# datamicroscopes/common

Measured on AMD Instinct MI355X. Metric: score_value evals/sec, higher is better.
Workload: dtype f32

## Files before the change

common_amd/csrc/abi.cpp:

```cpp
#include <algorithm>
#include <atomic>
#include <cmath>
#include <memory>
#include <mutex>
#include <new>

#include "launchers.hpp"

namespace msc {

static thread_local std::string g_last_error;

void set_error(const char *fmt, ...) {
  char buf[1024];
  va_list ap;
  va_start(ap, fmt);
  vsnprintf(buf, sizeof buf, fmt, ap);
  va_end(ap);
  g_last_error = buf;
}
int fail(int code, const char *fmt, ...) {
  char buf[1024];
  va_list ap;
  va_start(ap, fmt);
  vsnprintf(buf, sizeof buf, fmt, ap);
  va_end(ap);
  g_last_error = buf;
  return code;
}

size_t primitive_size(int t) {
  static const size_t sz[MSC_TYPE_NELEMS] = {1, 1, 1, 2, 2, 4, 4, 8, 8, 4, 8};
  return (t >= 0 && t < MSC_TYPE_NELEMS) ? sz[t] : 0;
}

static bool family_ok(int f) { return f >= MSC_BB && f <= MSC_DM; }

struct Switches {
  bool tail_forced = false, no_narrow_tail = false, no_bb_fuse = false, sweep_graph = false;
  uint64_t tail_min_rows = 0;
  int loo_lds = -1, sweep_nich1 = 0, alloc_candidates = 12;
  int marginal_tile = -1;

  float alloc_accept_gbps = 6650.f;
};
static Switches read_switches() {
  Switches sw;
  if (const char *e = std::getenv("MSC_TAIL_MIN_ROWS")) sw.tail_forced = true, sw.tail_min_rows = (uint64_t)std::atoll(e);
  sw.no_narrow_tail = std::getenv("MSC_NO_NARROW_TAIL") != nullptr, sw.no_bb_fuse = std::getenv("MSC_NO_BB_FUSE") != nullptr;
  if (const char *e = std::getenv("MSC_LOO_LDS")) sw.loo_lds = std::atoi(e);
  if (const char *e = std::getenv("MSC_SWEEP_NICH1")) sw.sweep_nich1 = std::atoi(e);
  if (const char *e = std::getenv("MSC_MARGINAL_TILE")) sw.marginal_tile = std::atoi(e);
  if (const char *g = std::getenv("MSC_SWEEP_GRAPH")) sw.sweep_graph = g[0] != '0' && g[0] != 0;
  if (const char *e = std::getenv("MSC_ALLOC_CANDIDATES")) sw.alloc_candidates = std::atoi(e);
  if (const char *e = std::getenv("MSC_ALLOC_ACCEPT_GBPS")) sw.alloc_accept_gbps = (float)std::atof(e);
  return sw;
}

template <typename T>
static int alloc_zeroed(DevBuf<T> &buf, size_t count) {
  MSC_HIP(buf.alloc(count, 1));
  MSC_HIP(hipMemset(buf, 0, std::max<size_t>(count, 1) * sizeof(T)));
  return MSC_OK;
}

}

using namespace msc;

extern "C" int msc_abi_version(void) { return MSC_ABI_VERSION; }
extern "C" const char *msc_last_kernel(int which) { return msc::last_kernel(which); }
extern "C" const char *msc_last_error(void) { return g_last_error.c_str(); }
extern "C" const char *msc_build_info(void) {
  return "microscopes_hip abi " "1" " gfx950 (CDNA4) hipcc " __VERSION__;
}

static int device_error_word(int device, volatile uint32_t **host_out) {
  static std::mutex mu;
  static uint32_t *words[64] = {};
  MSC_REQUIRE(device >= 0 && device < 64, "device %d: at most 64 devices", device);
  std::lock_guard<std::mutex> lock(mu);
  if (!words[device]) {
    uint32_t *h = nullptr;
    void *d = nullptr;
    MSC_HIP(hipHostMalloc(reinterpret_cast<void **>(&h), 64, hipHostMallocMapped));
    h[0] = h[1] = 0;
    MSC_HIP(hipHostGetDevicePointer(&d, h, 0));
    uint32_t *w = static_cast<uint32_t *>(d);
    if (bind_error_word_score(w) || bind_error_word_sweep(w) || bind_error_word_state(w) || bind_error_word_seq(w) ||
        bind_error_word_query(w))
      return fail(MSC_EHIP, "binding the device error word failed: %s", hipGetErrorString(hipGetLastError()));
    words[device] = h;
  }
  *host_out = words[device];
  return MSC_OK;
}
static int device_error_check(msc_context *ctx) {
  volatile uint32_t *w = ctx ? ctx->err_host : nullptr;
  if (!w || w[0] == 0) return MSC_OK;
  std::atomic_thread_fence(std::memory_order_acquire);
  const uint32_t code = w[0], detail = w[1];
  w[0] = 0;
  std::string what;
  auto add = [&](const char *t) { if (!what.empty()) what += "; "; what += t; };
  if (code & 1u) add("a wave-subset barrier of a tile kernel timed out (detail: workgroup): rows of that launch are wrong");
  if (code & 2u) add("msc_entity_op: leave from a group the row is not in / an empty group, or join of an assigned row (detail: group)");
  if (code & 4u) add("msc_relation_slice_scores: a block offset beyond the score row (detail: cell)");
  if (code & 8u) add("msc_sweep_sequential: an order entry >= nrows (visit skipped; detail: entry), or a leave from an empty group or counter (detail: group)");
  if (code & 16u) add("msc_zmatrix_add: a label outside [0, nlabels) (that sample was skipped; detail: row of z)");
  if (code & ~31u) add("unknown device-side error");
  return fail(MSC_EDEVICE, "reported by an earlier kernel on device %d: %s [detail of the first: %u]; rebuild the affected state's tables",
              ctx->device, what.c_str(), detail);
}

extern "C" int msc_context_create(int device, void *stream, msc_context **out) {
  MSC_REQUIRE(out != nullptr, "msc_context_create: out is null");
  *out = nullptr;
  int ndev = 0;
  hipError_t e = hipGetDeviceCount(&ndev);
  if (e != hipSuccess || ndev <= 0)
    return fail(MSC_ENODEVICE, "no HIP device visible (%s); this library has no CPU path",
                e == hipSuccess ? "device count is 0" : hipGetErrorString(e));
  MSC_REQUIRE(device >= 0 && device < ndev, "device %d out of range (have %d)", device, ndev);
  hipDeviceProp_t prop;
  MSC_HIP(hipGetDeviceProperties(&prop, device));
  if (std::strncmp(prop.gcnArchName, "gfx950", 6) != 0)
    return fail(MSC_ENODEVICE, "device %d is %s; kernels are built for gfx950 only", device,
                prop.gcnArchName);
  MSC_HIP(hipSetDevice(device));
  std::unique_ptr<msc_context> ctx(new (std::nothrow) msc_context());
  if (!ctx) return fail(MSC_ENOMEM, "out of host memory");
  ctx->device = device;
  ctx->stream = static_cast<hipStream_t>(stream);
  ctx->num_cus = prop.multiProcessorCount > 0 ? prop.multiProcessorCount : 256;
  MSC_HIP(ctx->mailbox_host.alloc(192 * 1024));
  MSC_HIP(hipHostGetDevicePointer(&ctx->mailbox_dev, ctx->mailbox_host, 0));
  if (ctx->sync_word_host.alloc(16) == hipSuccess) {
    *ctx->sync_word_host = 0;
    if (hipHostGetDevicePointer(&ctx->sync_word_dev, ctx->sync_word_host, 0) != hipSuccess) ctx->sync_word_ok = false;
  } else {
    (void)hipGetLastError();
  }
  MSC_TRY(device_error_word(device, &ctx->err_host));
  *out = ctx.release();
  return MSC_OK;
}

static void vmm_free(msc_context::VmmAlloc &a);

extern "C" int msc_context_destroy(msc_context *ctx) {
  if (!ctx) return MSC_OK;
  (void)hipSetDevice(ctx->device);
  for (auto &a : ctx->vmm) vmm_free(a);
  ctx->vmm.clear();
  if (ctx->record_stream) (void)hipStreamDestroy(ctx->record_stream);
  delete ctx;
  return MSC_OK;
}

extern "C" int msc_context_set_stream(msc_context *ctx, void *stream) {
  MSC_REQUIRE(ctx, "null context");
  ctx->stream = static_cast<hipStream_t>(stream);
  return MSC_OK;
}

extern "C" int msc_context_synchronize(msc_context *ctx) {
  MSC_REQUIRE(ctx, "null context");
  if (ctx->sync_word_host && ctx->sync_word_ok) {
    const uint32_t seq = ++ctx->sync_seq;
    if (hipStreamWriteValue32(ctx->stream, ctx->sync_word_dev, seq, 0) == hipSuccess) {
      volatile uint32_t *w = ctx->sync_word_host;
      for (int spin = 0; spin < 400000; spin++)
        if (*w == seq) {
          std::atomic_thread_fence(std::memory_order_acquire);
          return device_error_check(ctx);
        }
    } else {
      (void)hipGetLastError();
      ctx->sync_word_ok = false;
    }
  }
  MSC_HIP(hipStreamSynchronize(ctx->stream));
  return device_error_check(ctx);
}

static bool vmm_alloc(int device, size_t nbytes, msc_context::VmmAlloc *out) {
  const size_t chunk = 32u << 20;
  hipMemAllocationProp prop = {};
  prop.type = hipMemAllocationTypePinned;
  prop.location.type = hipMemLocationTypeDevice;
  prop.location.id = device;
  size_t gran = 0;
  if (hipMemGetAllocationGranularity(&gran, &prop, hipMemAllocationGranularityMinimum) != hipSuccess || gran == 0 || chunk % gran != 0) {
    (void)hipGetLastError();
    return false;
  }
  msc_context::VmmAlloc a;
  const size_t n = (std::max<size_t>(nbytes, 1) + chunk - 1) / chunk;
  a.size = n * chunk;
  a.va = nullptr;
  if (hipMemAddressReserve(&a.va, a.size, 2u << 20, nullptr, 0) != hipSuccess) {
    (void)hipGetLastError();
    return false;
  }
  bool ok = true;
  size_t mapped = 0;
// ... 737 lines not shown
    d.loo_tab = nullptr;
    tf.push_back(d);
    extra_f.push_back(0u);
  }
  for (uint32_t i = 0; i < n; i++)
    if (!taken[i]) {
      tf.push_back(t[i]);
      extra_f.push_back(extra[i]);
    }
  {
    std::vector<FeatDesc> &ta = st->desc_acc_host;
    ta.clear();
    std::vector<bool> covered(n, false);
    for (size_t q = 0; q < quads.size(); q++) {
      const Fused &fq = quads[q];
      if ((size_t)st->K * 8u * fq.m * 4u > 64u * 1024u) continue;
      const std::vector<uint32_t> &mem = members[fq.radix - 2];
      FeatDesc d = tf[q];
      for (uint32_t j = 0; j < 4; j++) d.fuse_acc[j] = nullptr;
      for (uint32_t j = 0; j < fq.m; j++) {
        const uint32_t src = t_src[mem[fq.first + j]];
        d.fuse_acc[j] = st->desc_host[src].acc_i64;
        covered[src] = true;
      }
      ta.push_back(d);
    }
    for (uint32_t i = 0; i < n; i++)
      if (!covered[i]) ta.push_back(st->desc_host[i]);
  }
  const std::vector<Fused> &fused = quads;
  st->fuse_any = !fused.empty();
  st->fuse_nfeat = (uint32_t)tf.size();
  st->fuse_split = split - (n - st->fuse_nfeat);
  for (uint32_t i = st->fuse_split; i < st->fuse_nfeat; i++) {
    tf[i].blk_first -= n - st->fuse_nfeat;
    tf[i].blk_end -= n - st->fuse_nfeat;
  }
  if (st->fuse_any) facts = plan_layout(tf, st->fuse_split, extra_f, sw);
  for (FeatDesc &d : tf) d.rn_pack = nullptr, d.rn_pos = nullptr, d.rn_x = nullptr, d.rn_n2 = d.rn_n2p = 0;
  for (FeatDesc &d : t) d.rn_pack = nullptr, d.rn_pos = nullptr, d.rn_x = nullptr, d.rn_n2 = d.rn_n2p = 0;
  if (stages_nich(facts.path) && bview == nullptr) facts.path = MSC_PATH_TILE;
  if (stages_nich(facts.path)) {
    const uint32_t s0 = st->fuse_split, n2 = st->fuse_nfeat - s0, n2p = (n2 + 3u) & ~3u;
    std::vector<NichPos> pos(n2p);
    std::vector<const void *> xcols(n2);
    for (uint32_t i = 0; i < n2p; i++) {
      NichPos &q = pos[i];
      q.xlim = INFINITY, q.blk_ok = 0u;
      if (i < n2) {
        const FeatDesc &d = tf[s0 + i];
        q.blk = (d.blk_first - s0) | (d.blk_end - d.blk_first) << 16, q.seg_end = d.grp_end - s0;
        xcols[i] = d.col;
      } else q.blk = i | 1u << 16, q.seg_end = n2p;
    }
    const float *xm = nullptr;
    if (nich_x_matrix(bview, xcols, &xm)) {
      MSC_HIP(hipMemcpyAsync(st->rn_pos, pos.data(), sizeof(NichPos) * n2p, hipMemcpyHostToDevice, st->ctx->stream));
      MSC_HIP(hipStreamSynchronize(st->ctx->stream));
      FeatDesc &h = tf[s0];
      h.rn_pack = st->rn_pack, h.rn_pos = st->rn_pos, h.rn_x = xm, h.rn_n2 = n2, h.rn_n2p = n2p;
    } else facts.path = MSC_PATH_TILE;
  }
  for (FeatDesc &d : tf) d.lk_idx = nullptr, d.lk_l4 = d.lk_goff = 0;
  for (FeatDesc &d : t) d.lk_idx = nullptr, d.lk_l4 = d.lk_goff = 0;
  if (bview == nullptr && facts.path == MSC_PATH_LOOKUPS) facts.path = MSC_PATH_TILE;
  if (facts.path == MSC_PATH_TILE_ROLES || facts.path == MSC_PATH_LOOKUPS) {
    const uint32_t *im = nullptr;
    uint32_t l4 = 0;
    if (look_idx_matrix(bview, tf, st->fuse_split, &im, &l4)) tf[0].lk_idx = im, tf[0].lk_l4 = l4;
    else facts.path = MSC_PATH_TILE;
  }
  st->tile_path = facts.path;
  {
    double lookups = 0, rows = 0, nich = (double)(st->fuse_nfeat - st->fuse_split);
    for (uint32_t i = 0; i < st->fuse_split; i++) {
      if (tf[i].family == MSC_NICH) nich += 1;
      else if (tf[i].family == MSC_DM) lookups += 2.0 * (tf[i].dim + 1), rows += tf[i].grp_rows;
      else lookups += 1, rows += tf[i].grp_rows;
    }
    PlanCost pc;
    const double first = 6.0 + 0.45 * lookups + 0.012 * rows;
    pc.tile_round_us = facts.path == MSC_PATH_NICH_PACK ? 6.0 + 1.3 * nich + 3.0 * lookups : facts.path == MSC_PATH_TILE_ROLES ? first + 0.75 * nich
                       : facts.path == MSC_PATH_LOOKUPS ? 0.75 * first : first + 1.5 * nich;
    pc.sweep_round_us = pc.tile_round_us + 2.5;
    pc.tail_fixed_us = 2.0;
    pc.tail_group_us = 0.5 + 0.03 * lookups + 0.057 * nich;
    st->plan_cost = pc;
  }
  st->tile_narrow_tail_ok = facts.tail_ok;
  st->tail_masked_nich = facts.tail_masked_nich;
  st->tail_dm = facts.tail_dm;
  st->tail_max_rows = facts.tail_max_rows;
  st->tail_pack_rows = facts.tail_pack_rows;
  return MSC_OK;
}

static int upload_desc(msc_state *st) {
  MSC_TRY(plan_groups(st));
  MSC_HIP(hipMemcpyAsync(st->desc_dev, st->desc_host.data(), sizeof(FeatDesc) * st->nfeat,
                         hipMemcpyHostToDevice, st->ctx->stream));
  MSC_HIP(hipMemcpyAsync(st->desc_tile_dev, st->desc_tile_host.data(), sizeof(FeatDesc) * st->nfeat,
                         hipMemcpyHostToDevice, st->ctx->stream));
  MSC_HIP(hipMemcpyAsync(st->desc_fuse_dev, st->desc_fuse_host.data(), sizeof(FeatDesc) * st->fuse_nfeat,
                         hipMemcpyHostToDevice, st->ctx->stream));
  MSC_HIP(hipMemcpyAsync(st->desc_acc_dev, st->desc_acc_host.data(), sizeof(FeatDesc) * st->desc_acc_host.size(),
                         hipMemcpyHostToDevice, st->ctx->stream));
  MSC_HIP(hipStreamSynchronize(st->ctx->stream));
  return MSC_OK;
}

extern "C" int msc_state_create(msc_context *ctx, const msc_feature_spec *features,
                                uint32_t nfeatures, uint32_t ngroups, msc_state **out) {
  MSC_REQUIRE(ctx && features && out, "null argument");
  MSC_REQUIRE(nfeatures > 0 && nfeatures <= 65535, "a state needs 1..65535 features (got %u)", nfeatures);
  MSC_REQUIRE(ngroups > 0 && ngroups <= (1u << 20), "ngroups %u out of range", ngroups);
  *out = nullptr;
  MSC_HIP(hipSetDevice(ctx->device));
  std::unique_ptr<msc_state> st(new (std::nothrow) msc_state());
  if (!st) return fail(MSC_ENOMEM, "out of host memory");
  st->ctx = ctx;
  st->nfeat = nfeatures;
  st->K = ngroups;
  st->kpad = round_up(ngroups, kGroupTile);
  const size_t kpad = st->kpad;
  st->feats.resize(nfeatures);
  st->desc_host.resize(nfeatures);
  size_t n_i64 = kpad, n_f64 = 0;
  for (uint32_t f = 0; f < nfeatures; f++) {
    msc_feature_host &h = st->feats[f];
    h.family = features[f].family;
    h.dim = features[f].dim;
    MSC_REQUIRE(family_ok(h.family), "feature %u: unknown family %d", f, h.family);
    if (h.family == MSC_DD && (h.dim == 0 || h.dim > kMaxDDDim))
      return fail(MSC_EUNSUPPORTED, "feature %u: dd dim %u outside 1..%u (DirichletDiscrete<128>)", f,
                  h.dim, kMaxDDDim);
    if (h.family == MSC_DM && (h.dim == 0 || h.dim > kMaxDDDim))
      return fail(MSC_EUNSUPPORTED, "feature %u: dm categories %u outside 1..%u", f, h.dim, kMaxDDDim);
    if (h.family == MSC_NIW && (h.dim == 0 || h.dim > kMaxNiwDim))
      return fail(MSC_EUNSUPPORTED, "feature %u: niw dim %u outside 1..%u", f, h.dim, kMaxNiwDim);
    h.i64_off = n_i64;
    h.i64_len = acc_i64_rows(h.family, h.dim) * kpad;
    n_i64 += h.i64_len;
    h.f64_off = n_f64;
    h.f64_len = h.family == MSC_NIW ? (size_t)ngroups * (h.dim + (size_t)h.dim * h.dim)
                                    : acc_f64_rows(h.family) * kpad;
    n_f64 += h.f64_len;
  }
  st->n_i64 = n_i64;
  st->n_f64 = n_f64;
  st->nich1 = nfeatures == 1 && st->feats[0].family == MSC_NICH;
  for (const msc_feature_host &h : st->feats) st->has_dm |= h.family == MSC_DM, st->n_niw += h.family == MSC_NIW;
  MSC_TRY(alloc_zeroed(st->red_i64, n_i64));
  MSC_TRY(alloc_zeroed(st->red_f64, n_f64));
  MSC_TRY(alloc_zeroed(st->cnt_u32, kpad));
  MSC_TRY(alloc_zeroed(st->logpc, crp_floats(st->kpad)));
  MSC_TRY(alloc_zeroed(st->desc_dev, nfeatures));
  MSC_TRY(alloc_zeroed(st->desc_tile_dev, nfeatures));
  MSC_TRY(alloc_zeroed(st->desc_fuse_dev, nfeatures));
  MSC_TRY(alloc_zeroed(st->nich_info, nfeatures));
  MSC_TRY(alloc_zeroed(st->rn_pos, (size_t)((nfeatures + 3u) & ~3u)));
  {
    size_t nnich = 0;
    for (uint32_t f = 0; f < nfeatures; f++) nnich += features[f].family == MSC_NICH;
    MSC_TRY(alloc_zeroed(st->rn_pack, (1 + kNichPackRows * nnich) * (size_t)kpad));
  }
  MSC_TRY(alloc_zeroed(st->desc_acc_dev, nfeatures));
  MSC_TRY(alloc_zeroed(st->rng_dev, 2));
  MSC_TRY(alloc_zeroed(st->colmax_dev, 1));
  for (uint32_t f = 0; f < nfeatures; f++) {
    msc_feature_host &h = st->feats[f];
    default_hp(h.family, h.dim, h.hp);
    MSC_TRY(alloc_zeroed(h.hp_dev, h.hp.size()));
    MSC_TRY(alloc_zeroed(h.tab, (size_t)(tab_rows(h.family, h.dim) + 4) * kpad));
    MSC_TRY(alloc_zeroed(h.raw_u32, (size_t)raw_u32_rows(h.family, h.dim) * kpad));
    const size_t nf32 = h.family == MSC_NIW ? (size_t)ngroups * (h.dim + (size_t)h.dim * h.dim)
                                            : (size_t)raw_f32_rows(h.family) * kpad;
    MSC_TRY(alloc_zeroed(h.raw_f32, nf32));
    if (loo_rows(h.family)) MSC_TRY(alloc_zeroed(h.loo64, (size_t)loo_rows(h.family) * kpad));
    if (loo_tab_rows(h.family, h.dim)) MSC_TRY(alloc_zeroed(h.loo_tab, (size_t)loo_tab_rows(h.family, h.dim) * kpad));
    if (h.family == MSC_DM) {
      MSC_TRY(alloc_zeroed(h.dm_meta_dev, 2 * ((size_t)h.dim + 1)));
      h.dm_meta.assign(2 * ((size_t)h.dim + 1), 0u);
    }
    if (h.family == MSC_NIW) {
      if (h.dim <= (uint32_t)kNiwPad) {
        MSC_TRY(alloc_zeroed(h.niw_w, (size_t)ngroups * kNiwPad * kNiwPad));
        MSC_TRY(alloc_zeroed(h.niw_b, (size_t)ngroups * 2 * kNiwPad));
      }
      MSC_TRY(alloc_zeroed(h.niw_w64, (size_t)ngroups * niw_w_stream(h.dim)));
      MSC_TRY(alloc_zeroed(h.niw_mu64, (size_t)ngroups * niw_b_stream(h.dim)));
      MSC_TRY(alloc_zeroed(h.niw_c64, (size_t)ngroups * 8));
    }
    if (!h.hp.empty()) {
      hipError_t e = hipMemcpy(h.hp_dev, h.hp.data(), h.hp.size() * sizeof(float), hipMemcpyHostToDevice);
      if (e != hipSuccess) return fail(MSC_EHIP, "hp upload failed: %s", hipGetErrorString(e));
    }
    h.raw_valid = true;
    h.additive_valid = true;
    h.derived_valid = false;
    FeatDesc &d = st->desc_host[f];
    std::memset(&d, 0, sizeof d);
    d.family = h.family;
    d.dim = h.dim;
    d.col_type = value_type_of(h.family);
    d.hp = h.hp_dev;
    d.tab = h.tab;
    d.raw_u32 = h.raw_u32;
    d.raw_f32 = h.raw_f32;
    d.acc_i64 = st->red_i64 + h.i64_off;
    d.acc_f64 = st->red_f64 + h.f64_off;
    d.niw_w = h.niw_w;
    d.niw_b = h.niw_b;
    d.niw_w64 = h.niw_w64;
    d.niw_mu64 = h.niw_mu64;
    d.niw_c64 = h.niw_c64;
    d.vcap = 32;
    d.dm_meta = nullptr;
    d.loo64 = h.loo64;
    d.loo_tab = h.loo_tab;
    d.aux = 0.0;
    for (float a : h.hp) d.aux += h.family == MSC_DD || h.family == MSC_DM ? (double)a : 0.0;
  }
  st->cnt_additive_valid = true;
  MSC_TRY(upload_desc(st.get()));
  hipError_t e = hipStreamSynchronize(ctx->stream);
  if (e != hipSuccess) return fail(MSC_EHIP, "state init failed: %s", hipGetErrorString(e));
  *out = st.release();
  return MSC_OK;
}

extern "C" int msc_state_destroy(msc_state *st) {
  if (!st) return MSC_OK;
  (void)hipSetDevice(st->ctx->device);
  (void)hipStreamSynchronize(st->ctx->stream);
  if (st->step_graph.exec) (void)hipGraphExecDestroy(st->step_graph.exec);
  if (st->pred_upload) (void)hipEventDestroy(st->pred_upload);
  delete st;
  return MSC_OK;
}

extern "C" int msc_state_shape(const msc_state *st, uint32_t *nfeatures, uint32_t *ngroups) {
  MSC_REQUIRE(st, "null state");
  if (nfeatures) *nfeatures = st->nfeat;
  if (ngroups) *ngroups = st->K;
  return MSC_OK;
}

extern "C" int msc_state_set_hp(msc_state *st, uint32_t feature, const float *host_hp, size_t nfloats) {
  MSC_REQUIRE(st && host_hp, "null argument");
  MSC_REQUIRE(feature < st->nfeat, "feature %u out of range", feature);
  msc_feature_host &h = st->feats[feature];
  MSC_REQUIRE(nfloats == h.hp.size(), "feature %u: hp block has %zu floats, expected %zu", feature,
              nfloats, h.hp.size());
  std::copy(host_hp, host_hp + nfloats, h.hp.begin());
  if (nfloats) {
    MSC_HIP(hipMemcpyAsync(h.hp_dev, h.hp.data(), nfloats * sizeof(float), hipMemcpyHostToDevice, st->ctx->stream));
    MSC_HIP(hipStreamSynchronize(st->ctx->stream));
  }
  h.derived_valid = false;
  if (h.family == MSC_DD || h.family == MSC_DM) {
    double asum = 0;
    for (float a : h.hp) asum += (double)a;
    st->desc_host[feature].aux = asum;
    MSC_TRY(upload_desc(st));
  }
  return MSC_OK;
}

extern "C" int msc_state_get_hp(const msc_state *st, uint32_t feature, float *host_hp, size_t nfloats) {
  MSC_REQUIRE(st && host_hp, "null argument");
  MSC_REQUIRE(feature < st->nfeat, "feature %u out of range", feature);
  const msc_feature_host &h = st->feats[feature];
  MSC_REQUIRE(nfloats == h.hp.size(), "feature %u: hp block has %zu floats, expected %zu", feature,
              nfloats, h.hp.size());
  std::copy(h.hp.begin(), h.hp.end(), host_hp);
  return MSC_OK;
}

static int launch_commit_all(msc_state *st) {
  if (launch_commit(st->ctx->stream, st->desc_dev, (int)st->nfeat, st->kpad, st->red_i64, st->cnt_u32))
    return fail(MSC_EHIP, "k_commit launch failed");
  for (uint32_t f = 0; f < st->nfeat; f++)
    if (st->feats[f].family == MSC_NIW &&
        launch_niw_commit(st->ctx->stream, st->desc_dev, f, st->feats[f].dim, st->K, st->kpad, 1))
      return fail(MSC_EHIP, "k_niw_commit launch failed");
  return MSC_OK;
}

static int ensure_raw(msc_state *st) {
  bool any = false;
  for (auto &h : st->feats) any |= !h.raw_valid;
  if (!any) return MSC_OK;
  MSC_TRY(launch_commit_all(st));
  for (auto &h : st->feats) { h.raw_valid = true; h.derived_valid = false; }
  st->crp_valid = false;
  return MSC_OK;
}

static void record_layout(int family, uint32_t dim, uint32_t &nu32, uint32_t &nf32) {
  nu32 = raw_u32_rows(family, dim);
  nf32 = raw_f32_rows(family);
}

extern "C" int msc_state_set_ss(msc_state *st, uint32_t feature, uint32_t first_group,
                                uint32_t ngroups, const void *host_records, size_t nbytes) {
  MSC_REQUIRE(st && host_records, "null argument");
// ... 486 lines not shown
  r.lanes = narrow_lanes(st, sw, &r.table_rows);
  r.path = st->nich1 ? MSC_PATH_NICH1 : st->has_dm ? MSC_PATH_TILE_DM : st->tile_path;
  if (r.lanes) return r;
  if (r.path == MSC_PATH_NICH1) {
    r.shape.nich1 = nich1_shape_for(st->ctx, out, nrows, st->K);
    return r;
  }
  const int cus = st->ctx->num_cus;
  const uint32_t ktiles = st->kpad / kGroupTile, last_groups = st->K - (ktiles - 1) * kGroupTile;
  const uint64_t round = (uint64_t)cus / ktiles;
  const bool small4 = r.path != MSC_PATH_TILE_DM && (nrows + 63) / 64 <= round, small2 = small4 && (nrows + 31) / 32 <= round;
  r.shape.wave_rows = small2 ? 2 : small4 ? 4 : 8;
  r.shape.pair = !small4 && pair_path(r.path, st->K);
  if (ktiles > 1 && r.path == MSC_PATH_TILE_ROLES && !small4 && last_groups > 64 && last_groups <= 128) r.shape.last = LastTile::pair;
  if (r.shape.last == LastTile::pair || !narrow_tail_fits(st)) return r;
  const PlanCost &pc = st->plan_cost;
  const uint64_t c128 = (nrows + 127) / 128;
  const double tile_us = (r.shape.pair ? kPairTileShare : 1.0) *
                         (tile_rounds_us(c128 * ktiles, cus, false, pc) - (ktiles > 1 ? tile_rounds_us(c128 * (ktiles - 1), cus, false, pc) : 0.0));
  const bool many_rows = sw.tail_forced ? nrows >= sw.tail_min_rows
                                        : nrows >= kTailMinRows && tail_rows_us(last_groups, true, nrows, cus, pc) < tile_us;
  if (many_rows) r.shape.last = LastTile::rows;
  return r;
}

static int run_score(msc_state *st, uint64_t row0, uint64_t nrows, const int32_t *z_dev, bool crp,
                     bool niw_f32, float *out_dev, uint64_t ld_out) {
  hipStream_t s = st->ctx->stream;
  const float *prior = crp ? st->logpc : nullptr;
  if (z_dev) MSC_TRY(run_loo_own(st, row0, nrows, z_dev, crp));
  const ScoreRoute r = route_score(st, nrows, out_dev);
  if (r.lanes) {
    return launch_narrow(s, st->ctx->num_cus, r.lanes, r.table_rows, false, st->desc_dev, (int)st->nfeat, st->K, st->kpad, row0, nrows,
                         z_dev, st->own, prior, out_dev, ld_out, 0, nullptr, nullptr, ZeroSpans());
  }
  bool written = false;
  if (st->n_niw < st->nfeat || crp) {
    const bool nich1 = r.path == MSC_PATH_NICH1;
    TailPlan tail;
    if (!nich1) {
      MSC_TRY(tail_plan(st, tail));
      MSC_TRY(refresh_fused_tables(st));
    }
    MSC_TRY(launch_score(s, st->ctx->num_cus, r.path, tail, r.shape, nich1 ? st->desc_dev : st->desc_fuse_dev, (int)st->fuse_nfeat,
                         (int)st->fuse_split, st->K, st->kpad, row0, nrows, z_dev, st->own, prior, out_dev, ld_out));
    written = true;
    for (uint32_t f = 0; f < st->nfeat; f++)
      if (gp_beyond_table(st, f) &&
          launch_gp_large_fix(s, st->ctx->num_cus, st->desc_dev, (int)f, st->K, st->kpad, row0, nrows, z_dev, out_dev, ld_out))
        return fail(MSC_EHIP, "k_gp_large_fix launch failed");
  }
  for (uint32_t f = 0; f < st->nfeat; f++) {
    if (st->feats[f].family != MSC_NIW) continue;
    if (z_dev) MSC_HIP(grow_retained(st->retired, st->niw_qown, nrows));
    if (launch_niw_score(s, st->ctx->num_cus, st->desc_dev, f, st->feats[f].dim, st->K, st->kpad, row0, nrows, z_dev, written,
                         niw_f32, st->niw_qown, out_dev, ld_out))
      return fail(MSC_EHIP, "k_score_niw launch failed: %s", hipGetErrorString(hipGetLastError()));
    written = true;
  }
  return MSC_OK;
}

extern "C" int msc_score_value(msc_state *st, const msc_dataview *view, const uint32_t *cols,
                               uint64_t row0, uint64_t nrows, const int32_t *z_dev, uint32_t flags,
                               float *out_dev, uint64_t ld_out) {
  MSC_REQUIRE(st && (out_dev || nrows == 0), "null argument");
  MSC_REQUIRE(ld_out >= st->K, "ld_out %llu < ngroups %u", (unsigned long long)ld_out, st->K);
  MSC_REQUIRE((flags & ~(MSC_SCORE_CRP_PRIOR | MSC_SCORE_NIW_F32)) == 0, "unknown flags 0x%x", flags);
  MSC_HIP(hipSetDevice(st->ctx->device));
  MSC_TRY(device_error_check(st->ctx));
  MSC_TRY(bind_view(st, view, cols, row0, nrows));
  if (nrows == 0) return MSC_OK;
  MSC_TRY(ensure_derived(st));
  const bool crp = (flags & MSC_SCORE_CRP_PRIOR) != 0;
  if (crp) MSC_TRY(ensure_crp(st));
  return run_score(st, row0, nrows, z_dev, crp, (flags & MSC_SCORE_NIW_F32) != 0, out_dev, ld_out);
}

extern "C" int msc_score_tune(msc_state *st, const msc_dataview *view, const uint32_t *cols, uint64_t row0,
                              uint64_t nrows, float *out_dev, uint64_t ld_out, int *shape_out, float *ms_out) {
  MSC_REQUIRE(st && view && out_dev, "null argument");
  MSC_REQUIRE(ld_out >= st->K, "ld_out %llu < ngroups %u", (unsigned long long)ld_out, st->K);
  if (shape_out) *shape_out = -1;
  if (ms_out) *ms_out = 0.f;
  MSC_HIP(hipSetDevice(st->ctx->device));
  MSC_TRY(bind_view(st, view, cols, row0, nrows));
  const ScoreRoute r = route_score(st, nrows, out_dev);
  if (r.lanes || r.path != MSC_PATH_NICH1 || nrows == 0) return MSC_OK;
  MSC_TRY(ensure_derived(st));
  hipStream_t s = st->ctx->stream;
  hipStreamCaptureStatus cap = hipStreamCaptureStatusNone;
  if (hipStreamIsCapturing(s, &cap) == hipSuccess && cap != hipStreamCaptureStatusNone)
    return fail(MSC_EINVAL, "msc_score_tune waits for the device: not on a capturing stream");
  auto launch = [&](int code) {
    return launch_score(s, st->ctx->num_cus, MSC_PATH_NICH1, TailPlan(), ScoreShape{8, false, LastTile::tiles, code}, st->desc_dev, 1, (int)st->tile_split, st->K, st->kpad, row0,
                        nrows, nullptr, nullptr, nullptr, out_dev, ld_out);
  };
  hipEvent_t e0, e1;
  MSC_HIP(hipEventCreate(&e0));
  MSC_HIP(hipEventCreate(&e1));
  float best = 0.f;
  int shape = -1, rc = MSC_OK;
  for (int cand = 0; cand < kNich1NumShapes && rc == MSC_OK; cand++) {
    if ((rc = launch(cand)) != MSC_OK) break;
    hipError_t e = hipEventRecord(e0, s);
    for (int r = 0; r < 6 && e == hipSuccess; r++) (void)launch(cand);
    if (e == hipSuccess) e = hipEventRecord(e1, s);
    if (e == hipSuccess) e = hipEventSynchronize(e1);
    float ms = 0.f;
    if (e == hipSuccess) e = hipEventElapsedTime(&ms, e0, e1);
    if (e != hipSuccess) { rc = fail(MSC_EHIP, "timing failed: %s", hipGetErrorString(e)); break; }
    if (shape < 0 || ms < best) {
      best = ms;
      shape = cand;
    }
  }
  int plain_stores = 0;
  if (rc == MSC_OK && shape >= 0) {
    float ms_kind[2] = {0.f, 0.f};
    for (int kind = 0; kind < 2 && rc == MSC_OK; kind++) {
      const int code = shape | (kind ? 0x100 : 0);
      if ((rc = launch(code)) != MSC_OK) break;
      hipError_t e = hipEventRecord(e0, s);
      for (int r = 0; r < 6 && e == hipSuccess; r++) (void)launch(code);
      if (e == hipSuccess) e = hipEventRecord(e1, s);
      if (e == hipSuccess) e = hipEventSynchronize(e1);
      if (e == hipSuccess) e = hipEventElapsedTime(&ms_kind[kind], e0, e1);
      if (e != hipSuccess) rc = fail(MSC_EHIP, "timing failed: %s", hipGetErrorString(e));
    }
    plain_stores = ms_kind[1] < ms_kind[0] ? 1 : 0;
    best = ms_kind[plain_stores];
  }
  (void)hipEventDestroy(e0);
  (void)hipEventDestroy(e1);
  MSC_TRY(rc);
  auto &memo = st->ctx->nich1_shapes;
  for (size_t i = 0; i < memo.size();)
    if (memo[i].out == out_dev && memo[i].nrows == nrows && memo[i].K == st->K) memo.erase(memo.begin() + i);
    else i++;
  memo.insert(memo.begin(), msc_context::ShapeEntry{out_dev, nrows, st->K, shape, plain_stores});
  if (memo.size() > 16) memo.pop_back();
  if (shape_out) *shape_out = shape;
  if (ms_out) *ms_out = best / 6.f;
  return MSC_OK;
}

static int commit(msc_state *st) {
  MSC_TRY(launch_commit_all(st));
  for (auto &h : st->feats) { h.raw_valid = true; h.derived_valid = false; }
  st->crp_valid = false;
  return MSC_OK;
}

enum : uint32_t { kAccZeroed = 0x100, kAccThenPrepare = 0x200 };

static int commit_and_prepare(msc_state *st, bool bump_rng = true) {
  hipStream_t s = st->ctx->stream;
  if (launch_commit_prepare(s, st->desc_dev, (int)st->nfeat, st->K, st->kpad, st->red_i64, st->cnt_u32, st->alpha,
                            st->logpc, bump_rng ? st->rng_dev : nullptr, prepare_value_slices(st)))
    return fail(MSC_EHIP, "k_commit_prepare launch failed");
  for (uint32_t f = 0; f < st->nfeat; f++) {
    const msc_feature_host &h = st->feats[f];
    if (h.family == MSC_NIW && (launch_niw_commit(s, st->desc_dev, f, h.dim, st->K, st->kpad, 1) ||
                                launch_niw_prepare(s, st->desc_dev, f, h.dim, st->K, st->kpad)))
      return fail(MSC_EHIP, "niw commit / prepare launch failed");
    if (h.family == MSC_DM && st->desc_host[f].dm_meta != nullptr &&
        launch_dm_prepare(s, st->desc_dev, (int)f, h.dim, st->kpad, dm_value_slices(h)))
      return fail(MSC_EHIP, "k_dm_prepare launch failed");
  }
  for (auto &h : st->feats) { h.raw_valid = true; h.derived_valid = true; }
  st->crp_valid = true;
  return MSC_OK;
}

static int accumulate_impl(msc_state *st, const msc_dataview *view, const uint32_t *cols, uint64_t row0,
                           uint64_t nrows, const int32_t *z_dev, uint32_t flags) {
  MSC_TRY(bind_view(st, view, cols, row0, nrows));
  hipStream_t s = st->ctx->stream;
  if (flags & MSC_ACC_RESET) {
    if (!(flags & kAccZeroed) && launch_zero64(s, st->red_i64, st->n_i64, st->red_f64, st->n_f64))
      return fail(MSC_EHIP, "k_zero64 launch failed");
  } else {
    MSC_TRY(ensure_raw(st));
    for (uint32_t f = 0; f < st->nfeat; f++)
      if (!st->feats[f].additive_valid) {
        const int rc = st->feats[f].family == MSC_NIW
                           ? launch_niw_commit(s, st->desc_dev, f, st->feats[f].dim, st->K, st->kpad, 0)
                           : launch_lift(s, st->desc_dev + f, 1, st->kpad, st->red_i64, st->cnt_u32, 0);
        if (rc) return fail(MSC_EHIP, "k_lift launch failed");
      }
    if (!st->cnt_additive_valid)
      if (launch_lift(s, st->desc_dev, 0, st->kpad, st->red_i64, st->cnt_u32, 1))
        return fail(MSC_EHIP, "k_lift launch failed");
  }
  for (auto &h : st->feats) h.additive_valid = true;
  st->cnt_additive_valid = true;
  if (nrows > 0) {
    const int rc = launch_accumulate(s, st->ctx->num_cus, st->desc_acc_dev, st->desc_acc_host.data(), (int)st->desc_acc_host.size(),
                                     st->K, st->kpad, row0, nrows, z_dev,
                                     (flags & MSC_ACC_SUBTRACT) ? -1 : 1, st->red_i64);
    if (rc == -2) return fail(MSC_EUNSUPPORTED, "accumulate tables for %u groups exceed LDS", st->K);
    if (rc) return fail(MSC_EHIP, "k_accumulate launch failed: %s", hipGetErrorString(hipGetLastError()));
    for (uint32_t f = 0; f < st->nfeat; f++) {
      if (st->feats[f].family != MSC_NIW) continue;
      MSC_REQUIRE(nrows < (1ull << 32), "niw accumulate takes at most 2^32 - 1 rows per call");
      MSC_HIP(grow_retained(st->retired, st->niw_scratch, 2 * (size_t)st->K + 1 + (size_t)nrows));
      if (launch_niw_accumulate(s, st->ctx->num_cus, st->desc_dev, f, st->K, row0, nrows, z_dev,
                                (flags & MSC_ACC_SUBTRACT) ? -1 : 1, st->niw_scratch, st->feats[f].dim))
        return fail(MSC_EHIP, "niw accumulate launch failed");
    }
  }
  for (auto &h : st->feats) h.raw_valid = false;
  if (flags & kAccThenPrepare) return commit_and_prepare(st);
  if (!(flags & MSC_ACC_NO_COMMIT)) MSC_TRY(commit(st));
  return MSC_OK;
}

extern "C" int msc_accumulate(msc_state *st, const msc_dataview *view, const uint32_t *cols,
                              uint64_t row0, uint64_t nrows, const int32_t *z_dev, uint32_t flags) {
  MSC_REQUIRE(st && (z_dev || nrows == 0), "null argument");
  MSC_REQUIRE((flags & ~(MSC_ACC_RESET | MSC_ACC_SUBTRACT | MSC_ACC_NO_COMMIT)) == 0, "unknown flags 0x%x", flags);
  MSC_HIP(hipSetDevice(st->ctx->device));
  MSC_TRY(device_error_check(st->ctx));
  return accumulate_impl(st, view, cols, row0, nrows, z_dev, flags);
}

extern "C" int msc_entity_op(msc_state *st, const msc_dataview *view, const uint32_t *cols, uint64_t row, uint32_t group,
                             int sign, int32_t *z_dev) {
  MSC_REQUIRE(st && view, "null argument");
  MSC_REQUIRE(sign != 0, "sign must be +1 (join) or -1 (leave)");
  MSC_REQUIRE(group < st->K, "group %u outside [0,%u)", group, st->K);
  MSC_REQUIRE(!st->rng_bump_pending, "msc_entity_op between msc_sweep_step_begin and msc_state_commit_reduce: the additive "
                                     "tables hold uncommitted sums");
  MSC_TRY(device_error_check(st->ctx));
  MSC_HIP(hipSetDevice(st->ctx->device));
  MSC_TRY(bind_view(st, view, cols, row, 1));
  hipStream_t s = st->ctx->stream;
  bool scalar_only = true;
  for (const auto &h : st->feats) scalar_only &= h.family != MSC_NIW && h.family != MSC_DM;
  if (!scalar_only) {
    if (!st->one_z) MSC_TRY(alloc_zeroed(st->one_z, 1));
    if (launch_set_i32(s, st->one_z, (int32_t)group)) return fail(MSC_EHIP, "k_set_i32 launch failed");
    MSC_TRY(accumulate_impl(st, view, cols, row, 1, st->one_z, sign < 0 ? (uint32_t)MSC_ACC_SUBTRACT : 0u));
    if (z_dev && launch_set_i32(s, z_dev + row, sign > 0 ? (int32_t)group : -1)) return fail(MSC_EHIP, "k_set_i32 launch failed");
    return MSC_OK;
  }
  MSC_TRY(ensure_raw(st));
  for (uint32_t f = 0; f < st->nfeat; f++)
    if (!st->feats[f].additive_valid && launch_lift(s, st->desc_dev + f, 1, st->kpad, st->red_i64, st->cnt_u32, 0))
      return fail(MSC_EHIP, "k_lift launch failed");
  if (!st->cnt_additive_valid && launch_lift(s, st->desc_dev, 0, st->kpad, st->red_i64, st->cnt_u32, 1))
    return fail(MSC_EHIP, "k_lift launch failed");
  for (auto &h : st->feats) h.additive_valid = true;
  st->cnt_additive_valid = true;
  MSC_TRY(ensure_derived(st));
  MSC_TRY(ensure_crp(st));
  if (launch_entity_op(s, st->desc_dev, (int)st->nfeat, st->K, st->kpad, row, group, sign > 0 ? 1 : -1, st->red_i64, st->cnt_u32,
                       st->alpha, st->logpc, z_dev ? z_dev + row : nullptr))
    return fail(MSC_EHIP, "k_entity_op launch failed");
  return MSC_OK;
}

extern "C" int msc_score_data(msc_state *st, float *out_dev) {
  MSC_REQUIRE(st && out_dev, "null argument");
  MSC_HIP(hipSetDevice(st->ctx->device));
  MSC_TRY(ensure_raw(st));
  if (launch_score_data(st->ctx->stream, st->desc_dev, (int)st->nfeat, st->K, st->kpad, out_dev))
    return fail(MSC_EHIP, "k_score_data launch failed");
  if (st->n_niw) {
    MSC_TRY(ensure_derived(st));
    for (uint32_t f = 0; f < st->nfeat; f++)
      if (st->feats[f].family == MSC_NIW &&
          launch_niw_score_data(st->ctx->stream, st->desc_dev, f, st->K, st->kpad, out_dev))
        return fail(MSC_EHIP, "k_niw_score_data launch failed");
  }
  return MSC_OK;
}

static bool sweep_is_niw1(const msc_state *st) {
  return st->nfeat == 1 && st->feats[0].family == MSC_NIW && (int)st->K <= sweep_niw1_max_groups(st->feats[0].dim);
}

static bool sweep_pair_mode(const msc_state *st) {
  return view_rows(st) >= kTailMinRows && pair_path(st->tile_path, st->K);
}
static bool sweep_rows_pays(const msc_state *st, const Switches &sw, uint32_t groups) {
  const uint64_t rows = view_rows(st);
  if (sw.tail_forced) return rows >= sw.tail_min_rows;
  if (rows < kTailMinRows) return false;
  const int cus = st->ctx->num_cus;
  const uint64_t c128 = (rows + 127) / 128;
  const bool tail = groups < st->K;
  const double sample_us = [&](uint64_t floats_per_row) { return 30.0 + (double)rows * floats_per_row * 4.0 / 2.0e6; }(tail ? st->K : 128);
  double rows_us = tail_rows_us(groups, false, rows, cus, st->plan_cost), tile_us;
  if (tail) {
    rows_us *= 1.15;
    tile_us = tile_rounds_us(c128, cus, false, st->plan_cost) + sample_us;
  } else {
    if (groups > 64) rows_us += sample_us;
    PlanCost pc = st->plan_cost;
    pc.sweep_round_us = pc.tile_round_us * (sweep_pair_mode(st) ? kPairTileShare : 1.0) + 2.5;
    tile_us = tile_rounds_us(c128, cus, true, pc);
  }
  return rows_us < tile_us;
}

static bool sweep_plain(const msc_state *st) {
  for (uint32_t f = 0; f < st->nfeat; f++) if (gp_beyond_table(st, f)) return false;
  return st->n_niw == 0;
}

static bool sweep_is_fused(const msc_state *st) {
  if (sweep_is_niw1(st)) return true;
  if (!sweep_plain(st)) return false;
  return st->nich1 ? st->K <= sweep_nich1_rows_max_groups() : st->K <= 256;
}

enum class SweepKind { niw1, nich1, nich1_rows, narrow, rows, rows_sampler, mixed, roles_tail, generic };
struct SweepRoute {
  SweepKind kind = SweepKind::generic;
  int lanes = 0; uint32_t table_rows = 0;
  bool transposed = false;
  ScoreShape shape;
  uint64_t tail_ld = 0;
  bool tail_pair = false;
};
static SweepRoute route_sweep(const msc_state *st, uint64_t nrows) {
  const Switches sw = read_switches();
  const uint64_t cus = (uint64_t)st->ctx->num_cus;
  SweepRoute r;
  if (sweep_is_niw1(st)) {
    r.kind = SweepKind::niw1;
  } else if (sweep_is_fused(st)) {
    if (st->nich1) {
      r.kind = st->K > 1024 ? SweepKind::nich1_rows : SweepKind::nich1;
      r.transposed = sw.sweep_nich1 == 2 || (sw.sweep_nich1 != 1 && view_rows(st) >= cus * 64);
    } else if ((r.lanes = narrow_lanes(st, sw, &r.table_rows)) != 0) {
      r.kind = SweepKind::narrow;
    } else if (narrow_tail_fits(st) && st->K <= kTailMaxGroups && sweep_rows_pays(st, sw, st->K)) {
      r.kind = st->K <= 64 ? SweepKind::rows : SweepKind::rows_sampler;
    } else {
      r.kind = SweepKind::mixed;
      r.shape.pair = sweep_pair_mode(st);
      const bool small = (nrows + 63) / 64 <= cus, view_small = (view_rows(st) + 63) / 64 <= cus;
      const int R = small ? ((nrows + 31) / 32 > cus ? 4 : 2) : view_small ? 4 : 8;
      if (!st->has_dm && (view_small || st->tile_path == MSC_PATH_TILE)) r.shape.wave_rows = R;
    }
  } else if (!st->nich1 && !st->has_dm && st->tile_path != MSC_PATH_TILE && st->tile_narrow_tail_ok && st->K > 256 &&
             st->K <= (uint32_t)kGroupTile + kTailMaxGroups && sweep_rows_pays(st, sw, st->K - kGroupTile) && sweep_plain(st)) {
    r.tail_ld = st->K <= (uint32_t)kGroupTile + 64 ? 64 : 128;
    r.tail_pair = st->tile_path == MSC_PATH_TILE_ROLES && r.tail_ld == 128;
    if (r.tail_pair || narrow_tail_fits(st)) r.kind = SweepKind::roles_tail;
  }
  return r;
}

static int sweep_assign_impl(msc_state *st, const msc_dataview *view, const uint32_t *cols, uint64_t row0,
                             uint64_t nrows, uint64_t row_id0, int32_t *z_dev, uint64_t seed, uint64_t sweep,
                             bool *zeroed = nullptr) {
  MSC_TRY(bind_view(st, view, cols, row0, nrows));
  if (nrows == 0) return MSC_OK;
  if (!st->rng_valid || st->rng_seed != seed || st->rng_sweep != sweep) {
    if (launch_rng_set(st->ctx->stream, st->rng_dev, seed, sweep)) return fail(MSC_EHIP, "k_rng_set launch failed");
    st->rng_valid = true;
    st->rng_seed = seed;
    st->rng_sweep = sweep;
  }
  MSC_TRY(ensure_derived(st));
  MSC_TRY(ensure_crp(st));
  hipStream_t s = st->ctx->stream;
  const int cus = st->ctx->num_cus;
  ZeroSpans zero;
  if (zeroed) {
    zero.a = reinterpret_cast<unsigned long long *>(st->red_i64.get()); zero.na = st->n_i64;
    zero.b = reinterpret_cast<unsigned long long *>(st->red_f64.get()); zero.nb = st->n_f64;
  }
  const SweepRoute r = route_sweep(st, nrows);
  bool zeroes = true;
  switch (r.kind) {
    case SweepKind::niw1:
      MSC_TRY(launch_sweep_niw1(s, cus, st->feats[0].dim, st->desc_dev, st->K, st->kpad, row0, nrows, row_id0, z_dev, st->logpc, st->rng_dev, zero));
      break;
    case SweepKind::nich1_rows:
      MSC_HIP(grow_retained(st->retired, st->rows_table, sweep_nich1_rows_table_floats(st->kpad)));
      MSC_TRY(launch_sweep_nich1_rows(s, cus, st->desc_dev, st->K, st->kpad, row0, nrows, row_id0, z_dev, st->logpc, st->rng_dev, zero, st->rows_table));
      break;
    case SweepKind::nich1:
      MSC_TRY(launch_sweep_nich1(s, cus, r.transposed, st->desc_dev, st->K, st->kpad, row0, nrows, row_id0, z_dev, st->own, st->logpc, st->rng_dev, zero));
      break;
    case SweepKind::narrow:
      MSC_TRY(run_loo_own(st, row0, nrows, z_dev, true));
      MSC_TRY(launch_narrow(s, cus, r.lanes, r.table_rows, true, st->desc_dev, (int)st->nfeat, st->K, st->kpad, row0, nrows, z_dev,
                            st->own, st->logpc, nullptr, 0, row_id0, z_dev, st->rng_dev, zero));
      break;
    case SweepKind::mixed:
      MSC_TRY(run_loo_own(st, row0, nrows, z_dev, true));
      MSC_TRY(refresh_fused_tables(st));
      MSC_TRY(launch_sweep_mixed(s, cus, st->has_dm, st->tile_path, r.shape, st->desc_fuse_dev, (int)st->fuse_nfeat, (int)st->fuse_split, st->K, st->kpad, row0, nrows, row_id0, z_dev, st->own, st->logpc, st->rng_dev, zero));
      break;
    case SweepKind::rows:
    case SweepKind::rows_sampler: {
      MSC_TRY(run_loo_own(st, row0, nrows, z_dev, true));
      MSC_TRY(refresh_fused_tables(st));
      TailPlan tail;
      MSC_TRY(tail_plan(st, tail, false));
      if (r.kind == SweepKind::rows) {
        MSC_TRY(launch_sweep_rows(s, cus, tail, st->desc_fuse_dev, (int)st->fuse_nfeat, (int)st->fuse_split, st->K, st->kpad, row0, nrows, row_id0,
                                  z_dev, st->own, st->logpc, st->rng_dev, zero));
        break;
      }
      MSC_HIP(grow_retained(st->retired, st->tail_scores, ((size_t)nrows + 16) * 128));
      MSC_TRY(launch_score_tail(s, cus, tail, st->desc_fuse_dev, (int)st->fuse_nfeat, (int)st->fuse_split, st->K, st->kpad, 0, row0, nrows,
                                z_dev, st->own, st->logpc, st->tail_scores, 128));
      if (launch_sample_rows(s, cus, st->tail_scores, 128, st->K, nrows, row_id0, z_dev, st->rng_dev)) return fail(MSC_EHIP, "k_sample_rows launch failed");
      zeroes = false;
      break;
    }
    case SweepKind::roles_tail: {
      MSC_TRY(refresh_fused_tables(st));
      MSC_TRY(run_loo_own(st, row0, nrows, z_dev, true));
      MSC_HIP(grow_retained(st->retired, st->tail_scores, ((size_t)nrows + 16) * r.tail_ld));
      TailPlan tail;
      MSC_TRY(tail_plan(st, tail, false));
      MSC_TRY(r.tail_pair ? launch_score_pair_tail(s, cus, st->desc_fuse_dev, (int)st->fuse_nfeat, (int)st->fuse_split, st->K, st->kpad, row0, nrows,
                                                   z_dev, st->own, st->logpc, st->tail_scores, r.tail_ld)
                          : launch_score_tail(s, cus, tail, st->desc_fuse_dev, (int)st->fuse_nfeat, (int)st->fuse_split, st->K, st->kpad,
                                              kGroupTile, row0, nrows, z_dev, st->own, st->logpc, st->tail_scores - kGroupTile, r.tail_ld));
      MSC_TRY(launch_sweep_roles_tail(s, cus, st->tile_path, st->desc_fuse_dev, (int)st->fuse_nfeat, (int)st->fuse_split, st->K, st->kpad, row0, nrows,
                                      row_id0, z_dev, st->own, st->logpc, st->rng_dev, zero, st->tail_scores));
      break;
    }
    case SweepKind::generic: {
      const uint64_t ld = std::min<uint64_t>(st->kpad, ((uint64_t)st->K + 63) & ~63ull);
      const uint64_t chunk = std::max<uint64_t>(1, std::min<uint64_t>((4096ull << 20) / (ld * sizeof(float)), nrows));
      MSC_HIP(grow_retained(st->retired, st->scratch, chunk * ld));
      for (uint64_t at = 0; at < nrows; at += chunk) {
        const uint64_t n = std::min<uint64_t>(chunk, nrows - at);
        MSC_TRY(run_score(st, row0 + at, n, z_dev + at, true, false, st->scratch, ld));
        if (launch_sample_rows(s, cus, st->scratch, ld, st->K, n, row_id0 + at, z_dev + at, st->rng_dev))
          return fail(MSC_EHIP, "k_sample_rows launch failed");
      }
      zeroes = false;
      break;
    }
  }
  if (zeroed) {
    *zeroed = zeroes;
    return MSC_OK;
  }
  if (launch_rng_bump(s, st->rng_dev)) return fail(MSC_EHIP, "k_rng_bump launch failed");
  st->rng_sweep = sweep + 1;
  return MSC_OK;
}

extern "C" int msc_sweep_assign(msc_state *st, const msc_dataview *view, const uint32_t *cols,
                                uint64_t row0, uint64_t nrows, uint64_t row_id0, int32_t *z_dev,
                                uint64_t seed, uint64_t sweep) {
  MSC_REQUIRE(st && (z_dev || nrows == 0), "null argument");
  MSC_HIP(hipSetDevice(st->ctx->device));
  MSC_TRY(device_error_check(st->ctx));
  return sweep_assign_impl(st, view, cols, row0, nrows, row_id0, z_dev, seed, sweep);
}

static int accumulate_impl(msc_state *st, const msc_dataview *view, const uint32_t *cols, uint64_t row0,
                           uint64_t nrows, const int32_t *z_dev, uint32_t flags);

typedef std::vector<uint8_t> StepFlags;
static StepFlags save_flags(const msc_state *st) {
  StepFlags f;
  for (auto &h : st->feats) f.push_back((uint8_t)(h.raw_valid | (h.additive_valid << 1) | (h.derived_valid << 2)));
  f.push_back((uint8_t)(st->cnt_additive_valid | (st->crp_valid << 1) | (st->rng_valid << 2)));
  return f;
}
static void restore_flags(msc_state *st, const StepFlags &f) {
  for (size_t i = 0; i < st->feats.size(); i++) {
    st->feats[i].raw_valid = f[i] & 1;
    st->feats[i].additive_valid = (f[i] >> 1) & 1;
    st->feats[i].derived_valid = (f[i] >> 2) & 1;
  }
  st->cnt_additive_valid = f.back() & 1;
  st->crp_valid = (f.back() >> 1) & 1;
  st->rng_valid = (f.back() >> 2) & 1;
}

extern "C" int msc_sweep_step(msc_state *st, const msc_dataview *view, const uint32_t *cols, uint64_t row0,
                              uint64_t nrows, uint64_t row_id0, int32_t *z_dev, uint64_t seed, uint64_t sweep) {
  MSC_REQUIRE(st && view && (z_dev || nrows == 0), "null argument");
  MSC_HIP(hipSetDevice(st->ctx->device));
  MSC_TRY(device_error_check(st->ctx));
  hipStream_t s = st->ctx->stream;
  auto eager = [&]() -> int {
    st->step_graph.n_eager++;
    bool zeroed = false;
    MSC_TRY(sweep_assign_impl(st, view, cols, row0, nrows, row_id0, z_dev, seed, sweep, &zeroed));
    st->rng_valid = false;
    MSC_TRY(accumulate_impl(st, view, cols, row0, nrows, z_dev,
                            MSC_ACC_RESET | kAccThenPrepare | (zeroed ? (uint32_t)kAccZeroed : 0u)));
    st->rng_valid = true;
    st->rng_sweep = sweep + 1;
    return MSC_OK;
  };
  MSC_TRY(bind_view(st, view, cols, row0, nrows));
  msc_state::StepGraph &g = st->step_graph;
  const bool no_graph = !read_switches().sweep_graph;
  if (nrows == 0) return accumulate_impl(st, view, cols, row0, 0, z_dev, MSC_ACC_RESET);
  if (no_graph || g.disabled) return eager();
  std::vector<uint32_t> colv(st->nfeat);
  for (uint32_t f = 0; f < st->nfeat; f++) colv[f] = cols ? cols[f] : f;
  const bool same_key = g.view == view && g.view_serial == view->serial && g.row0 == row0 && g.nrows == nrows &&
                        g.row_id0 == row_id0 && g.z == z_dev && g.alpha == st->alpha && g.cols == colv;
  if (!same_key) {
    if (g.exec) { (void)hipGraphExecDestroy(g.exec); g.exec = nullptr; }
    g.view = view; g.view_serial = view->serial; g.row0 = row0; g.nrows = nrows; g.row_id0 = row_id0; g.z = z_dev;
    g.alpha = st->alpha; g.cols = colv;
    g.seen = 0;
  }
  const bool next_sweep = st->rng_valid && st->rng_seed == seed && st->rng_sweep == sweep;
  const StepFlags entry = save_flags(st);
  if (g.exec) {
    if (!next_sweep || entry != g.flags) return eager();
    MSC_HIP(hipGraphLaunch(g.exec, s));
    g.n_replayed++;
    st->rng_sweep = sweep + 1;
    return MSC_OK;
  }
  if (g.seen < 2 || !next_sweep || !sweep_is_fused(st)) {
    g.seen++;
    return eager();
  }
  msc_context *ctx = st->ctx;
  if (!ctx->record_stream && hipStreamCreateWithFlags(&ctx->record_stream, hipStreamNonBlocking) != hipSuccess)
    ctx->record_stream = nullptr;
  if (!ctx->record_stream || hipStreamBeginCapture(ctx->record_stream, hipStreamCaptureModeThreadLocal) != hipSuccess) {
    (void)hipGetLastError();
    g.disabled = true;
    return eager();
  }
  const uint64_t sweep_before = st->rng_sweep;
  ctx->stream = ctx->record_stream;
  const int rc = eager();
  ctx->stream = s;
  g.n_eager--;
  hipGraph_t graph = nullptr;
  const hipError_t ec = hipStreamEndCapture(ctx->record_stream, &graph);
  bool ok = rc == MSC_OK && ec == hipSuccess && graph != nullptr && save_flags(st) == entry;
  if (ok && hipGraphInstantiate(&g.exec, graph, nullptr, nullptr, 0) != hipSuccess) {
    g.exec = nullptr;
    ok = false;
  }
  if (graph) (void)hipGraphDestroy(graph);
  if (!ok) {
    (void)hipGetLastError();
    if (g.exec) { (void)hipGraphExecDestroy(g.exec); g.exec = nullptr; }
    g.disabled = true;
    restore_flags(st, entry);
    st->rng_sweep = sweep_before;
    return eager();
  }
  g.flags = entry;
  MSC_HIP(hipGraphLaunch(g.exec, s));
  g.n_replayed++;
  return MSC_OK;
}

extern "C" int msc_sweep_step_begin(msc_state *st, const msc_dataview *view, const uint32_t *cols, uint64_t row0,
                                    uint64_t nrows, uint64_t row_id0, int32_t *z_dev, uint64_t seed, uint64_t sweep) {
  MSC_REQUIRE(st && view && (z_dev || nrows == 0), "null argument");
  MSC_HIP(hipSetDevice(st->ctx->device));
  MSC_TRY(device_error_check(st->ctx));
  if (nrows == 0) return accumulate_impl(st, view, cols, row0, 0, z_dev, MSC_ACC_RESET | MSC_ACC_NO_COMMIT);
  bool zeroed = false;
  MSC_TRY(sweep_assign_impl(st, view, cols, row0, nrows, row_id0, z_dev, seed, sweep, &zeroed));
  st->rng_valid = false;
  st->rng_bump_pending = true;
  st->rng_next_sweep = sweep + 1;
  return accumulate_impl(st, view, cols, row0, nrows, z_dev,
                         MSC_ACC_RESET | MSC_ACC_NO_COMMIT | (zeroed ? (uint32_t)kAccZeroed : 0u));
}

extern "C" int msc_sweep_step_stats(const msc_state *st, uint64_t *eager_steps, uint64_t *graph_steps) {
  MSC_REQUIRE(st, "null argument");
  if (eager_steps) *eager_steps = st->step_graph.n_eager;
  if (graph_steps) *graph_steps = st->step_graph.n_replayed;
  return MSC_OK;
}

constexpr double kSeqLaunchUs = 20000.0;
constexpr uint64_t kSeqMaxVisitsPerLaunch = 10000;

static double seq_visit_us(const msc_state *st) {
  double rows = 0.0;
  for (uint32_t f = 0; f < st->nfeat; f++) {
    switch (st->feats[f].family) {
      case MSC_BB: rows += 4; break;
      case MSC_GP:
      case MSC_BNB: rows += 2.0 * st->desc_host[f].vcap + 4; break;
      case MSC_DD: rows += 2.0 * st->feats[f].dim + 2; break;
      case MSC_NICH: rows += 14; break;
      default: break;
    }
  }
  return 16.0 + 0.02 * 2.0 * rows + 0.007 * (double)st->K * (double)st->nfeat;
}

struct SeqRoute { int rc = MSC_OK; const char *why = ""; };
static SeqRoute route_sequential(const msc_state *st) {
  SeqRoute r;
  for (const auto &h : st->feats) {
    if (h.family == MSC_NIW || h.family == MSC_DM || h.family == MSC_BBNC) {
      r.rc = MSC_EUNSUPPORTED;
      r.why = "the sequential sweep takes bb, gp, bnb, dd, nich and noop features (the state holds niw, dm or bbnc)";
      return r;
    }
  }
  if (st->nfeat > (uint32_t)kSeqMaxFeat) {
    r.rc = MSC_EUNSUPPORTED;
    r.why = "the sequential sweep takes at most 256 features";
  } else if (st->K > kSeqMaxGroups) {
    r.rc = MSC_EUNSUPPORTED;
    r.why = "the sequential sweep takes at most 8192 groups";
  }
  return r;
}

extern "C" int msc_sweep_sequential(msc_state *st, const msc_dataview *view, const uint32_t *cols, uint64_t row0,
                                    uint64_t nrows, uint64_t row_id0, int32_t *z_dev, const uint32_t *order_dev,
                                    uint32_t nsweeps, uint64_t seed, uint64_t sweep, int32_t *trace_dev) {
  MSC_REQUIRE(st && view && (z_dev || nrows == 0), "null argument");
  MSC_REQUIRE(nrows < (1ull << 32), "the sequential sweep takes at most 2^32 - 1 rows per call");
  MSC_REQUIRE(!st->rng_bump_pending, "msc_sweep_sequential between msc_sweep_step_begin and msc_state_commit_reduce: the "
                                     "additive tables hold uncommitted sums");
  MSC_HIP(hipSetDevice(st->ctx->device));
  MSC_TRY(device_error_check(st->ctx));
  const SeqRoute route = route_sequential(st);
  if (route.rc != MSC_OK) return fail(route.rc, "%s", route.why);
  MSC_TRY(bind_view(st, view, cols, row0, nrows));
  if (nrows == 0 || nsweeps == 0) return MSC_OK;
  hipStream_t s = st->ctx->stream;
  MSC_TRY(ensure_raw(st));
  for (uint32_t f = 0; f < st->nfeat; f++)
    if (!st->feats[f].additive_valid && launch_lift(s, st->desc_dev + f, 1, st->kpad, st->red_i64, st->cnt_u32, 0))
      return fail(MSC_EHIP, "k_lift launch failed");
  if (!st->cnt_additive_valid && launch_lift(s, st->desc_dev, 0, st->kpad, st->red_i64, st->cnt_u32, 1))
    return fail(MSC_EHIP, "k_lift launch failed");
  for (auto &h : st->feats) h.additive_valid = true;
  st->cnt_additive_valid = true;
  MSC_TRY(ensure_derived(st));
  MSC_TRY(ensure_crp(st));
  const uint64_t visits = (uint64_t)nsweeps * nrows;
  const uint64_t per_launch = (uint64_t)std::max(1.0, std::min((double)kSeqMaxVisitsPerLaunch, kSeqLaunchUs / seq_visit_us(st)));
  for (uint64_t v0 = 0; v0 < visits; v0 += per_launch) {
    const uint64_t v1 = std::min(visits, v0 + per_launch);
    const int rc = launch_sweep_seq(s, st->desc_dev, (int)st->nfeat, st->K, st->kpad, row0, nrows, row_id0, z_dev, order_dev,
                                    v0, v1, seed, sweep, st->red_i64, st->cnt_u32, st->alpha, st->logpc, trace_dev);
    if (rc == -2) return fail(MSC_EUNSUPPORTED, "k_sweep_seq does not take this shape");
    if (rc) return fail(MSC_EHIP, "k_sweep_seq launch failed: %s", hipGetErrorString(hipGetLastError()));
  }
  for (auto &h : st->feats) { h.raw_valid = true; h.additive_valid = true; h.derived_valid = true; }
  st->cnt_additive_valid = true;
  st->crp_valid = true;
  return MSC_OK;
}

extern "C" int msc_state_reduce_buffers(msc_state *st, void **dev_i64, size_t *n_i64, void **dev_f64,
                                        size_t *n_f64) {
  MSC_REQUIRE(st, "null state");
  if (dev_i64) *dev_i64 = st->red_i64;
  if (n_i64) *n_i64 = st->n_i64;
  if (dev_f64) *dev_f64 = st->red_f64;
  if (n_f64) *n_f64 = st->n_f64;
  return MSC_OK;
}

extern "C" int msc_state_reduce_pack(msc_state *st, void **pack_dev, size_t *n_f64) {
  MSC_REQUIRE(st && pack_dev, "null argument");
  MSC_HIP(hipSetDevice(st->ctx->device));
  if (!st->red_pack) MSC_TRY(alloc_zeroed(st->red_pack, st->n_i64 + st->n_f64));
  if (launch_pack64(st->ctx->stream, false, st->red_i64, st->n_i64, st->red_f64, st->n_f64, st->red_pack))
    return fail(MSC_EHIP, "k_pack64 launch failed");
  *pack_dev = st->red_pack;
  if (n_f64) *n_f64 = st->n_i64 + st->n_f64;
  return MSC_OK;
}
extern "C" int msc_state_reduce_unpack(msc_state *st) {
  MSC_REQUIRE(st, "null state");
  MSC_REQUIRE(st->red_pack, "msc_state_reduce_unpack before msc_state_reduce_pack");
  MSC_HIP(hipSetDevice(st->ctx->device));
  if (launch_pack64(st->ctx->stream, true, st->red_i64, st->n_i64, st->red_f64, st->n_f64, st->red_pack))
    return fail(MSC_EHIP, "k_unpack64 launch failed");
  return MSC_OK;
}

extern "C" int msc_state_set_sweep_rows(msc_state *st, uint64_t global_rows) {
  MSC_REQUIRE(st, "null state");
  if (st->sweep_rows_hint != global_rows && st->step_graph.exec) {
    (void)hipGraphExecDestroy(st->step_graph.exec);
    st->step_graph.exec = nullptr;
    st->step_graph.seen = 0;
  }
  st->sweep_rows_hint = global_rows;
  return MSC_OK;
}

extern "C" int msc_state_col_bounds(msc_state *st, const msc_dataview *view, const uint32_t *cols, uint32_t *out, size_t n) {
  MSC_REQUIRE(st && view, "null argument");
  const size_t want = col_bounds_size(st);
  MSC_REQUIRE(n == want, "the state's features take %zu column bounds (got %zu)", want, n);
  MSC_REQUIRE(out || n == 0, "null argument");
  MSC_HIP(hipSetDevice(st->ctx->device));
  MSC_TRY(device_error_check(st->ctx));
  MSC_TRY(bind_view(st, view, cols, 0, 0));
  size_t k = 0;
  for (uint32_t f = 0; f < st->nfeat; f++) {
    const uint32_t c = st->bound_cols[f];
    if (is_count_family(st->feats[f].family)) out[k++] = (uint32_t)std::max(view->col_max[c], 0ll);
    else if (st->feats[f].family == MSC_DM)
      for (uint32_t i = 0; i <= st->feats[f].dim; i++) out[k++] = view->dm_max[c][i];
  }
  return MSC_OK;
}

extern "C" int msc_state_set_col_bounds(msc_state *st, const uint32_t *bounds, size_t n) {
  MSC_REQUIRE(st, "null state");
  const size_t want = col_bounds_size(st);
  MSC_REQUIRE(n == 0 || n == want, "the state's features take %zu column bounds (got %zu)", want, n);
  MSC_REQUIRE(bounds || n == 0, "null bounds");
  std::vector<std::vector<uint32_t>> nb;
  if (n != 0) {
    nb.resize(st->nfeat);
    for (uint32_t f = 0, k = 0; f < st->nfeat; f++) {
// ... 788 lines not shown
```

common_amd/csrc/kernels_sweep.hip:

```cpp
#include "family_math.hpp"
#include "launchers.hpp"
#include "score_block.hpp"

namespace msc {

template <int CTRL, int ROW_MASK>
MSC_DEV float dpp_f32(float identity, float v) {
  return __int_as_float(__builtin_amdgcn_update_dpp(__float_as_int(identity), __float_as_int(v), CTRL, ROW_MASK, 0xf, false));
}
#define MSC_DPP_REDUCE(op, v)                                                     \
  asm volatile("s_nop 1\n\t" op " %0, %0, %0 row_shr:1 row_mask:0xf bank_mask:0xf\n\t"      \
               "s_nop 1\n\t" op " %0, %0, %0 row_shr:2 row_mask:0xf bank_mask:0xf\n\t"      \
               "s_nop 1\n\t" op " %0, %0, %0 row_shr:4 row_mask:0xf bank_mask:0xf\n\t"      \
               "s_nop 1\n\t" op " %0, %0, %0 row_shr:8 row_mask:0xf bank_mask:0xf\n\t"      \
               "s_nop 1\n\t" op " %0, %0, %0 row_bcast:15 row_mask:0xa bank_mask:0xf\n\t"   \
               "s_nop 1\n\t" op " %0, %0, %0 row_bcast:31 row_mask:0xc bank_mask:0xf\n\t"   \
               "s_nop 1"                                                          \
               : "+v"(v))
MSC_DEV float wave_max(float v) {
  MSC_DPP_REDUCE("v_max_f32_dpp", v);
  return lane_bcast(v, 63);
}
MSC_DEV float wave_incl_scan(float v, int) {
  MSC_DPP_REDUCE("v_add_f32_dpp", v);
  return v;
}

template <int G, bool LOG2 = false, bool BOUND = false, bool SHIFTED = false>
MSC_DEV int sample_from_scores(const float (&s)[G], float u01, int lane, uint32_t K, float bound = 0.f) {
  float p[G], sum = 0.f, incl = 0.f, total = 0.f;
  bool done = false;
  if (BOUND) {
    sum = 0.f;
#pragma unroll
    for (int j = 0; j < G; j++) {
      p[j] = __builtin_amdgcn_exp2f(SHIFTED ? s[j] : LOG2 ? s[j] - bound : (s[j] - bound) * 1.44269504088896340736f);
      sum += p[j];
    }
    incl = wave_incl_scan(sum, lane);
    total = lane_bcast(incl, 63);
    done = total > 0x1p-60f && total < 0x1p100f;
  }
  if (!done) {
    float m = s[0];
#pragma unroll
    for (int j = 1; j < G; j++) m = fmaxf(m, s[j]);
    m = wave_max(m);
    sum = 0.f;
#pragma unroll
    for (int j = 0; j < G; j++) {
      p[j] = __builtin_amdgcn_exp2f(LOG2 ? s[j] - m : (s[j] - m) * 1.44269504088896340736f);
      sum += p[j];
    }
    incl = wave_incl_scan(sum, lane);
    total = lane_bcast(incl, 63);
  }
  const float dart = u01 * total;
  float c = incl - sum;
  int nmiss = 0;
  if constexpr (G <= 4) {
#pragma unroll
    for (int j = 0; j < G; j++) {
      c += p[j];
      nmiss += c < dart ? 1 : 0;
    }
  } else {
    float q[G / 4];
#pragma unroll
    for (int b = 0; b < G / 4; b++) q[b] = ((p[4 * b] + p[4 * b + 1]) + p[4 * b + 2]) + p[4 * b + 3];
    int blk = 0;
#pragma unroll
    for (int b = 0; b < G / 4; b++) {
      const float cq = c + q[b];
      const bool miss = (blk == b) && cq < dart;
      c = miss ? cq : c;
      blk += miss ? 1 : 0;
    }
    nmiss = 4 * blk;
    if (blk < G / 4) {
      float e0 = p[0], e1 = p[1], e2 = p[2];
#pragma unroll
      for (int b = 1; b < G / 4; b++) {
        e0 = blk == b ? p[4 * b] : e0;
        e1 = blk == b ? p[4 * b + 1] : e1;
        e2 = blk == b ? p[4 * b + 2] : e2;
      }
      c += e0;
      const bool m0 = c < dart;
      c += e1;
      const bool m1 = m0 && c < dart;
      c += e2;
      const bool m2 = m1 && c < dart;
      nmiss += (m0 ? 1 : 0) + (m1 ? 1 : 0) + (m2 ? 1 : 0);
    }
  }
  const unsigned long long hit = __builtin_amdgcn_ballot_w64(nmiss < G);
  if (hit == 0ull) return (int)K - 1;
  const int l = (int)__builtin_ctzll(hit);
  const int k = G * l + lane_bcast(nmiss, l);
  return k < (int)K ? k : (int)K - 1;
}

template <int TAILP>
MSC_DEV int sample_tile_and_tail(const float (&sm)[4], const float (&st)[4], float u01, int lane, uint32_t K) {
  float m = fmaxf(fmaxf(fmaxf(sm[0], sm[1]), fmaxf(sm[2], sm[3])), fmaxf(fmaxf(st[0], st[1]), fmaxf(st[2], st[3])));
  m = wave_max(m);
  float pm[4], pt[4], summ = 0.f, sumt = 0.f;
#pragma unroll
  for (int j = 0; j < 4; j++) {
    pm[j] = __builtin_amdgcn_exp2f((sm[j] - m) * 1.44269504088896340736f);
    pt[j] = __builtin_amdgcn_exp2f((st[j] - m) * 1.44269504088896340736f);
    summ += pm[j];
    sumt += pt[j];
  }
  const float inclm = wave_incl_scan(summ, lane), totm = lane_bcast(inclm, 63);
  const float inclt = wave_incl_scan(sumt, lane), tott = lane_bcast(inclt, 63);
  const float dart = u01 * (totm + tott);
  float c = inclm - summ;
  int nmiss = 0;
#pragma unroll
  for (int j = 0; j < 4; j++) {
    c += pm[j];
    nmiss += c < dart ? 1 : 0;
  }
  unsigned long long hit = __builtin_amdgcn_ballot_w64(nmiss < 4);
  if (hit != 0ull) {
    const int l = (int)__builtin_ctzll(hit);
    return 4 * l + lane_bcast(nmiss, l);
  }
  c = totm + (inclt - sumt);
  nmiss = 0;
#pragma unroll
  for (int j = 0; j < 4; j++) {
    c += pt[j];
    nmiss += c < dart ? 1 : 0;
  }
  hit = __builtin_amdgcn_ballot_w64(nmiss < 4 && lane < 16 * TAILP);
  if (hit == 0ull) return (int)K - 1;
  const int l = (int)__builtin_ctzll(hit);
  const int k = kGroupTile + 4 * l + lane_bcast(nmiss, l);
  return k < (int)K ? k : (int)K - 1;
}


template <int G>
__global__ __launch_bounds__(256, G == 16 ? 3 : 1) void k_sweep_nich1(const FeatDesc *__restrict__ feats, uint32_t K,
                                                      uint32_t kpad, uint64_t row0, uint64_t nrows,
                                                      uint64_t row_id0, int32_t *__restrict__ z,
                                                      const float *__restrict__ own,
                                                      const float *__restrict__ crp,
                                                      const uint64_t *__restrict__ rng, int chunk_rows,
                                                      ZeroSpans zero) {
  const uint64_t seed = rng[0], sweep = rng[1];
  zero_spans(zero);
  const FeatDesc fd = feats[0];
  const int lane = threadIdx.x & 63;
  const uint32_t kb = (uint32_t)(G * lane);
  float mh[G], ml[G], c0[G], c1[G], c2[G];
  bool empty[G];
#pragma unroll
  for (int j = 0; j < G; j++) {
    const uint32_t k = kb + j;
    const size_t kc = k < kpad ? k : 0;
    mh[j] = fd.tab[(size_t)NICH_MU_HI * kpad + kc];
    ml[j] = fd.tab[(size_t)NICH_MU_LO * kpad + kc];
    c0[j] = fd.tab[(size_t)NICH_C0 * kpad + kc];
    c1[j] = fd.tab[(size_t)NICH_C1 * kpad + kc];
    c2[j] = fd.tab[(size_t)NICH_C2 * kpad + kc];
    const float lcj = crp[kc];
    empty[j] = __builtin_isinf(lcj);
    c0[j] += empty[j] ? 0.f : lcj;
  }
  const float le0 = crp[2 * (size_t)kpad], le1 = crp[2 * (size_t)kpad + 1];
  constexpr float kLog2e = 1.44269504088896340736f;
  const bool any_empty = !__builtin_isinf(le0);
  const float dle = any_empty ? (le1 - le0) * kLog2e : 0.f;
  float c0s[G];
  unsigned emask = 0u;
  float bound = -INFINITY;
#pragma unroll
  for (int j = 0; j < G; j++) {
    if (empty[j] && kb + j < K) emask |= 1u << j;
    c0s[j] = (kb + j >= K) ? -INFINITY : (c0[j] + (empty[j] ? le0 : 0.f)) * kLog2e;
    if (kb + j < K) bound = fmaxf(bound, c0s[j]);
  }
  bound = wave_max(bound) + 16.f;
#pragma unroll
  for (int j = 0; j < G; j++) c0s[j] -= bound;
  const float *xcol = reinterpret_cast<const float *>(fd.col) + row0;
  const uint64_t nchunks = (nrows + chunk_rows - 1) / chunk_rows;
  const uint64_t wave_id = (uint64_t)blockIdx.x * 4 + (threadIdx.x >> 6);
  const uint64_t nwaves = (uint64_t)gridDim.x * 4;
  for (uint64_t chunk = wave_id; chunk < nchunks; chunk += nwaves) {
    const uint64_t rb = chunk * chunk_rows;
    const int nr = (int)((nrows - rb) < (uint64_t)chunk_rows ? (nrows - rb) : (uint64_t)chunk_rows);
    const bool has_row = lane < nr;
    const float xv = has_row ? xcol[rb + lane] : 0.0f;
    int gz = has_row ? z[rb + lane] : -1;
    if ((uint32_t)gz >= K) gz = -1;
    const float u01 = philox_uniform01(seed, sweep, row_id0 + rb + lane);
    const unsigned long long mbits =
        __builtin_amdgcn_ballot_w64(fd.mask != nullptr && has_row && fd.mask[row0 + rb + lane] != 0);
    float sloo = 0.f;
    bool single = false;
    if (gz >= 0) {
      const float lm1 = crp[kpad + gz];
      single = __builtin_isinf(lm1);
      double s = single ? (double)le1 + (double)crp[2 * (size_t)kpad + 3] : (double)lm1 + (double)crp[crp_lo_cntm1(kpad) + gz];
      if (!((mbits >> lane) & 1ull))
        s += nich_loo_tab(fd.hp, fd.loo64 + (size_t)gz * kNlooStride, 1, xv);
      sloo = (float)s * kLog2e - bound;
    }
    const unsigned long long singles = any_empty ? __builtin_amdgcn_ballot_w64(single) : 0ull;
    const unsigned long long odd = mbits | singles;
    int znew = gz;
    for (int r = 0; r < nr; r++) {
      const float x = lane_bcast(xv, r), sl = lane_bcast(sloo, r);
      const int g = lane_bcast(gz, r);
      float s[G];
#pragma unroll
      for (int j = 0; j < G; j++) s[j] = nich_eval_log2(x, mh[j], ml[j], c0s[j], c1[j], c2[j]);
      if ((odd >> r) & 1ull) {
        if ((mbits >> r) & 1ull) {
          const float e_raw = ((singles >> r) & 1ull) ? le1 : le0;
#pragma unroll
          for (int j = 0; j < G; j++) {
            const float lcj = crp[kb + j < kpad ? kb + j : 0];
            s[j] = (kb + j >= K) ? -INFINITY : (__builtin_isinf(lcj) ? e_raw : lcj) * kLog2e - bound;
          }
        } else {
#pragma unroll
          for (int j = 0; j < G; j++) s[j] += ((emask >> j) & 1u) ? dle : 0.f;
        }
      }
      if (g >= 0 && lane == g / G) {
#pragma unroll
        for (int j = 0; j < G; j++)
          if (j == g % G) s[j] = sl;
      }
      const int pick = sample_from_scores<G, true, true, true>(s, lane_bcast(u01, r), lane, K);
      if (lane == r) znew = pick;
    }
    if (has_row) z[rb + lane] = znew;
  }
}

constexpr int kTRows = 32;
constexpr int kTPad = 65;

template <int G>
struct NichConsts {
  float mh[G], ml[G], c0s[G], c1[G], c2[G];
  unsigned emask;
};
struct NichRowCtx {
  const float *tab, *crp;
  uint32_t K, kpad;
  float le0, le1, dle, bound, x;
  bool masked, single;
};
MSC_DEV float nich_entry_log2(const NichRowCtx &c, uint32_t k) {
  constexpr float kLog2e = 1.44269504088896340736f;
  const size_t kc = k < c.kpad ? k : 0;
  const float lc = c.crp[kc];
  const bool empty = __builtin_isinf(lc);
  float s;
  if (c.masked) {
    s = (empty ? (c.single ? c.le1 : c.le0) : lc) * kLog2e - c.bound;
  } else {
    const float c0s = (c.tab[(size_t)NICH_C0 * c.kpad + kc] + (empty ? c.le0 : lc)) * kLog2e - c.bound;
    s = nich_eval_log2(c.x, c.tab[(size_t)NICH_MU_HI * c.kpad + kc], c.tab[(size_t)NICH_MU_LO * c.kpad + kc], c0s,
                       c.tab[(size_t)NICH_C1 * c.kpad + kc], c.tab[(size_t)NICH_C2 * c.kpad + kc]);
    s += (c.single && empty) ? c.dle : 0.f;
  }
  return k < c.K ? s : -INFINITY;
}
template <int G>
MSC_DEV void nich_row_scores(float (&s)[G], const NichConsts<G> &c, float x, bool masked, bool single, float dle, int own,
                             float sl, const float *__restrict__ crp, uint32_t K, uint32_t kpad, uint32_t l, float le0,
                             float le1, float bound) {
  constexpr float kLog2e = 1.44269504088896340736f;
#pragma unroll
  for (int j = 0; j < G; j++) s[j] = nich_eval_log2(x, c.mh[j], c.ml[j], c.c0s[j], c.c1[j], c.c2[j]);
  if (masked) {
#pragma unroll
    for (int j = 0; j < G; j++) {
      const uint32_t k = (uint32_t)G * l + j;
      const float lc = crp[k < kpad ? k : 0];
      s[j] = (k >= K) ? -INFINITY : (__builtin_isinf(lc) ? (single ? le1 : le0) : lc) * kLog2e - bound;
    }
  } else if (single) {
#pragma unroll
    for (int j = 0; j < G; j++) s[j] += ((c.emask >> j) & 1u) ? dle : 0.f;
  }
#pragma unroll
  for (int j = 0; j < G; j++)
    if (j == own) s[j] = sl;
}

constexpr int kTCst = 5;
enum { TC_MH = 0, TC_ML, TC_C0, TC_C1, TC_C2 };

template <int G>
__global__ __launch_bounds__(256) void k_sweep_nich1_t(const FeatDesc *__restrict__ feats, uint32_t K, uint32_t kpad,
                                                        uint64_t row0, uint64_t nrows, uint64_t row_id0,
                                                        int32_t *z, const float *__restrict__ crp,
                                                        const uint64_t *__restrict__ rng, ZeroSpans zero) {
  constexpr int TR = kTRows;
  __shared__ float lsum[4][TR * kTPad];
  __shared__ float cst[64 * G * kTCst];
  const uint64_t seed = rng[0], sweep = rng[1];
  zero_spans(zero);
  const FeatDesc fd = feats[0];
  const int lane = threadIdx.x & 63, wave = __builtin_amdgcn_readfirstlane(threadIdx.x >> 6);
  float *mysum = lsum[wave];
  constexpr float kLog2e = 1.44269504088896340736f;
  const float le0 = crp[2 * (size_t)kpad], le1 = crp[2 * (size_t)kpad + 1];
  const bool any_empty = !__builtin_isinf(le0);
  const float dle = any_empty ? (le1 - le0) * kLog2e : 0.f;
  for (uint32_t k = threadIdx.x; k < 64u * G; k += 256u) {
    const uint32_t kc = k < kpad ? k : 0u;
    const float lc = crp[kc];
    float *c = cst + k * kTCst;
    c[TC_MH] = fd.tab[NICH_MU_HI * kpad + kc];
    c[TC_ML] = fd.tab[NICH_MU_LO * kpad + kc];
    c[TC_C0] = k < K ? (fd.tab[NICH_C0 * kpad + kc] + (__builtin_isinf(lc) ? le0 : lc)) * kLog2e : -INFINITY;
    c[TC_C1] = fd.tab[NICH_C1 * kpad + kc];
    c[TC_C2] = fd.tab[NICH_C2 * kpad + kc];
  }
  __syncthreads();
  NichConsts<G> mine;
  mine.emask = 0u;
  float bound = -INFINITY;
#pragma unroll
  for (int j = 0; j < G; j++) {
    const uint32_t k = (uint32_t)(G * lane + j);
    const float *c = cst + k * kTCst;
    mine.mh[j] = c[TC_MH], mine.ml[j] = c[TC_ML], mine.c0s[j] = c[TC_C0], mine.c1[j] = c[TC_C1], mine.c2[j] = c[TC_C2];
    if (k < K && __builtin_isinf(crp[k])) mine.emask |= 1u << j;
    bound = fmaxf(bound, mine.c0s[j]);
  }
  bound = wave_max(bound) + 16.f;
#pragma unroll
  for (int j = 0; j < G; j++) mine.c0s[j] -= bound;
  const float *xcol = reinterpret_cast<const float *>(fd.col) + row0;
  const uint64_t wave_id = (uint64_t)blockIdx.x * 4 + wave, nwaves = (uint64_t)gridDim.x * 4;
  const uint64_t per = nrows / nwaves, extra = nrows % nwaves;
  const uint64_t rbeg = wave_id * per + (wave_id < extra ? wave_id : extra), rend = rbeg + per + (wave_id < extra ? 1 : 0);
  for (uint64_t rb = rbeg; rb < rend; rb += 64) {
    const int nr = __builtin_amdgcn_readfirstlane((int)((rend - rb) < 64u ? (rend - rb) : 64u));
    const bool has_row = lane < nr;
    const float xv = has_row ? xcol[rb + lane] : 0.0f;
    int gz = has_row ? z[rb + lane] : -1;
    if ((uint32_t)gz >= K) gz = -1;
    const float u01 = philox_uniform01(seed, sweep, row_id0 + rb + lane);
    const bool my_mask = fd.mask != nullptr && has_row && fd.mask[row0 + rb + lane] != 0;
    const unsigned long long mbits = __builtin_amdgcn_ballot_w64(my_mask);
    float sloo = 0.f;
    bool single = false;
    if (gz >= 0) {
      const float lm1 = crp[kpad + gz];
      single = __builtin_isinf(lm1);
      float s = single ? le1 : lm1;
      if (!my_mask) s += nich_loo_tab_sweep(fd.hp, fd.loo64 + (size_t)gz * kNlooStride, 1, xv);
      sloo = s * kLog2e - bound;
    }
    const bool my_single = single && any_empty;
    const unsigned long long singles = __builtin_amdgcn_ballot_w64(my_single);
    const unsigned long long odd = mbits | singles;
    const bool plain = !(my_mask || my_single);
    const NichRowCtx rc = {fd.tab, crp, K, kpad, le0, le1, dle, bound, xv, my_mask, my_single};
    auto entry = [&](int k) -> float {
      const float *c = cst + k * kTCst;
      float s = nich_eval_log2_est(xv, c[TC_MH], c[TC_ML], c[TC_C0] - bound, c[TC_C1], c[TC_C2]);
      if (!plain) s = nich_entry_log2(rc, (uint32_t)k);
      return __builtin_amdgcn_exp2f(k == gz ? sloo : s);
    };
    const int own_lane = gz >= 0 ? gz / G : -1;
    float own_sum = 0.f;
    if (own_lane >= 0) {
      own_sum = entry(G * own_lane);
#pragma unroll
      for (int j = 1; j < G; j++) own_sum += entry(G * own_lane + j);
    }
    int pick = gz;
    bool redo = false;
    for (int h0 = 0; h0 < nr; h0 += TR) {
      const int h1 = h0 + TR < nr ? h0 + TR : nr;
      __builtin_amdgcn_s_waitcnt(0);
      for (int r = h0; r < h1; r++) {
        const float x = lane_bcast(xv, r);
        float s[G];
        if ((odd >> r) & 1ull) {
          nich_row_scores<G>(s, mine, x, ((mbits >> r) & 1ull) != 0, ((singles >> r) & 1ull) != 0, dle, -1, 0.f, crp, K, kpad,
                             (uint32_t)lane, le0, le1, bound);
        } else {
#pragma unroll
          for (int j = 0; j < G; j++) s[j] = nich_eval_log2_est(x, mine.mh[j], mine.ml[j], mine.c0s[j], mine.c1[j], mine.c2[j]);
        }
        float sum = __builtin_amdgcn_exp2f(s[0]);
#pragma unroll
        for (int j = 1; j < G; j++) sum += __builtin_amdgcn_exp2f(s[j]);
        mysum[(r - h0) * kTPad + lane] = sum;
      }
      __builtin_amdgcn_wave_barrier();
      if (lane >= h0 && lane < h1) {
        float *row = mysum + (lane - h0) * kTPad;
        if (own_lane >= 0) row[own_lane] = own_sum;
        float blk[8], total = 0.f;
#pragma unroll
        for (int b = 0; b < 8; b++) {
          float t = row[8 * b];
#pragma unroll
          for (int i = 1; i < 8; i++) t += row[8 * b + i];
          blk[b] = t;
          total = b == 0 ? t : total + t;
        }
        if (total > 0x1p-60f && total < 0x1p100f) {
          const float dart = u01 * total;
          float c0 = 0.f;
          int b0 = 0;
#pragma unroll
          for (int b = 0; b < 7; b++) {
            const bool miss = b0 == b && c0 + blk[b] < dart;
            c0 = miss ? c0 + blk[b] : c0;
            b0 += miss ? 1 : 0;
          }
          int hl = 8 * b0;
#pragma unroll
          for (int i = 0; i < 7; i++) {
            const float v = row[8 * b0 + i];
            const bool miss = hl == 8 * b0 + i && c0 + v < dart;
            c0 = miss ? c0 + v : c0;
            hl += miss ? 1 : 0;
          }
          int j0 = 0;
#pragma unroll
          for (int j = 0; j < G - 1; j++) {
            const float v = entry(G * hl + j);
            const bool miss = j0 == j && c0 + v < dart;
            c0 = miss ? c0 + v : c0;
            j0 += miss ? 1 : 0;
          }
          const int k = G * hl + j0;
          pick = k < (int)K ? k : (int)K - 1;
        } else {
          redo = true;
        }
      }
      __builtin_amdgcn_wave_barrier();
    }
    unsigned long long todo = __builtin_amdgcn_ballot_w64(redo);
    while (todo != 0ull) {
      const int r = (int)__builtin_ctzll(todo);
      todo &= todo - 1ull;
      const float x = lane_bcast(xv, r);
      const int g = lane_bcast(gz, r);
      float s[G];
      nich_row_scores<G>(s, mine, x, ((mbits >> r) & 1ull) != 0, ((singles >> r) & 1ull) != 0, dle,
                         (g >= 0 && lane == g / G) ? g % G : -1, lane_bcast(sloo, r), crp, K, kpad, (uint32_t)lane, le0, le1, bound);
      const int p = sample_from_scores<G, true, false>(s, lane_bcast(u01, r), lane, K);
      if (lane == r) pick = p;
    }
    if (has_row) z[rb + lane] = pick;
  }
}

#ifndef MSC_DBG_ALWAYS_REDO
#define MSC_DBG_ALWAYS_REDO 0
#endif
constexpr int kRowsNb = 16;
constexpr uint32_t kRowsMaxK = 32768;
struct RowsGeom {
  uint32_t B, nb;
};
inline RowsGeom rows_geom(uint32_t kpad) {
  RowsGeom g;
  g.B = ((kpad + kRowsNb - 1) / kRowsNb + 63) / 64 * 64;
  g.nb = (kpad + g.B - 1) / g.B;
  return g;
}
enum { RT_MH = 0, RT_ML, RT_C0, RT_C1, RT_C2, RT_PRIOR, RT_DLE, RT_PAD, RT_WORDS };

__global__ __launch_bounds__(1024) void k_nich_rows_table(const FeatDesc *__restrict__ feats, uint32_t K, uint32_t kpad,
                                                           const float *__restrict__ crp, float *__restrict__ tab, uint32_t nent) {
  __shared__ float red[16];
  const FeatDesc fd = feats[0];
  constexpr float kLog2e = 1.44269504088896340736f;
  const float le0 = crp[2 * (size_t)kpad], le1 = crp[2 * (size_t)kpad + 1];
  const bool any_empty = !__builtin_isinf(le0);
  const float dle = any_empty ? (le1 - le0) * kLog2e : 0.f;
  float mx = -INFINITY;
  for (uint32_t k = threadIdx.x; k < K; k += 1024) {
    const float lc = crp[k];
    mx = fmaxf(mx, (fd.tab[(size_t)NICH_C0 * kpad + k] + (__builtin_isinf(lc) ? le0 : lc)) * kLog2e);
  }
  mx = wave_max(mx);
  if ((threadIdx.x & 63) == 0) red[threadIdx.x >> 6] = mx;
  __syncthreads();
  float bound = red[0];
  for (int w = 1; w < 16; w++) bound = fmaxf(bound, red[w]);
  bound += 16.f;
  for (uint32_t k = threadIdx.x; k < nent; k += 1024) {
    float *e = tab + (size_t)k * RT_WORDS;
    const bool in = k < K;
    const uint32_t kc = in ? k : 0u;
    const float lc = crp[kc];
    const bool empty = __builtin_isinf(lc);
    const float pr = empty ? le0 : lc;
    e[RT_MH] = in ? fd.tab[(size_t)NICH_MU_HI * kpad + kc] : 0.f;
    e[RT_ML] = in ? fd.tab[(size_t)NICH_MU_LO * kpad + kc] : 0.f;
    e[RT_C0] = in ? (fd.tab[(size_t)NICH_C0 * kpad + kc] + pr) * kLog2e - bound : -INFINITY;
    e[RT_C1] = in ? fd.tab[(size_t)NICH_C1 * kpad + kc] : 0.f;
    e[RT_C2] = in ? fd.tab[(size_t)NICH_C2 * kpad + kc] : 0.f;
    e[RT_PRIOR] = in ? pr * kLog2e - bound : -INFINITY;
    e[RT_DLE] = in && empty ? dle : 0.f;
    e[RT_PAD] = 0.f;
  }
  if (threadIdx.x < 8 * RT_WORDS) tab[(size_t)nent * RT_WORDS + threadIdx.x] = 0.f;
  if (threadIdx.x == 0) tab[((size_t)nent + 8) * RT_WORDS] = bound;
}

typedef float f32x2 __attribute__((ext_vector_type(2)));
typedef uint32_t u32x2 __attribute__((ext_vector_type(2)));
MSC_DEV f32x2 rows_eval2(f32x2 x, f32x4 e0, float c2) {
#pragma clang fp contract(off)
  const f32x2 mh = {e0.x, e0.x}, ml = {e0.y, e0.y}, c0 = {e0.z, e0.z}, nc1 = {-e0.w, -e0.w}, sc = {c2, c2};
  const f32x2 one = {1.0f, 1.0f};
  const f32x2 a = __builtin_elementwise_fma(x, sc, -mh) - ml;
  const f32x2 u = __builtin_elementwise_fma(a, a, one);
  const u32x2 magic = {kLog2eOverU, kLog2eOverU};
  const f32x2 ru = __builtin_bit_cast(f32x2, magic - __builtin_bit_cast(u32x2, u));
  const f32x2 lg = {hw_log2(u.x), hw_log2(u.y)};
  const f32x2 s = __builtin_elementwise_fma(nc1, __builtin_elementwise_fma(__builtin_elementwise_fma(a, a, -(u - one)), ru, lg), c0);
  return f32x2{__builtin_amdgcn_exp2f(s.x), __builtin_amdgcn_exp2f(s.y)};
}
MSC_DEV float rows_entry(float x, f32x4 e0, f32x4 e1, bool masked, bool single) {
  float s = nich_eval_log2_est(x, e0.x, e0.y, e0.z, e0.w, e1.x);
  s += single ? e1.z : 0.f;
  return masked ? e1.y + (single ? e1.z : 0.f) : s;
}

__global__ __launch_bounds__(128) void k_sweep_nich1_rows(const FeatDesc *__restrict__ feats, uint32_t K, uint32_t kpad,
                                                           uint64_t row0, uint64_t nrows, uint64_t row_id0,
                                                           int32_t *__restrict__ z, const float *__restrict__ crp,
                                                           const uint64_t *__restrict__ rng, ZeroSpans zero,
                                                           const float *__restrict__ tab, uint32_t B, uint32_t nb) {
  __shared__ float blk_all[2][kRowsNb * 2 * 64];
  typedef const __attribute__((address_space(4))) f32x4 *scalar_f4;
  const uint64_t seed = rng[0], sweep = rng[1];
  zero_spans(zero);
  const FeatDesc fd = feats[0];
  const int lane = threadIdx.x & 63, wave = __builtin_amdgcn_readfirstlane(threadIdx.x >> 6);
  float *blk = blk_all[wave];
  constexpr float kLog2e = 1.44269504088896340736f;
  const uint32_t nent = nb * B;
  const float bound = tab[((size_t)nent + 8) * RT_WORDS];
  const float le1 = crp[2 * (size_t)kpad + 1];
  const bool any_empty = !__builtin_isinf(crp[2 * (size_t)kpad]);
  const float *xcol = reinterpret_cast<const float *>(fd.col) + row0;
  const scalar_f4 stab = (scalar_f4)tab;
  const f32x4 *gtab = reinterpret_cast<const f32x4 *>(tab);
  const uint64_t wave_id = (uint64_t)blockIdx.x * 2 + wave, nwaves = (uint64_t)gridDim.x * 2;
  const uint64_t per = nrows / nwaves, extra = nrows % nwaves;
  const uint64_t rbeg = wave_id * per + (wave_id < extra ? wave_id : extra), rend = rbeg + per + (wave_id < extra ? 1 : 0);
  for (uint64_t rb = rbeg; rb < rend; rb += 128) {
    float x[2], u01[2], sloo[2];
    int gz[2], pick[2];
    bool has[2], masked[2], single[2];
#pragma unroll
    for (int i = 0; i < 2; i++) {
      const uint64_t n = rb + 64 * i + lane;
      has[i] = n < rend;
      x[i] = has[i] ? xcol[n] : 0.f;
      gz[i] = has[i] ? z[n] : -1;
      if ((uint32_t)gz[i] >= K) gz[i] = -1;
      u01[i] = philox_uniform01(seed, sweep, row_id0 + n);
      masked[i] = fd.mask != nullptr && has[i] && fd.mask[row0 + n] != 0;
      sloo[i] = 0.f;
      single[i] = false;
      if (gz[i] >= 0) {
        const float lm1 = crp[kpad + gz[i]];
        const bool only = __builtin_isinf(lm1);
        float s = only ? le1 : lm1;
        if (!masked[i]) s += nich_loo_tab_sweep(fd.hp, fd.loo64 + (size_t)gz[i] * kNlooStride, 1, x[i]);
        sloo[i] = s * kLog2e - bound;
        single[i] = only && any_empty;
      }
      pick[i] = gz[i];
    }
    const bool odd = __builtin_amdgcn_ballot_w64(masked[0] || masked[1] || single[0] || single[1]) != 0ull;
    for (uint32_t b = 0; b < nb; b++) {
      float run0 = 0.f, run1 = 0.f;
      if (!odd) {
        f32x2 run = {0.f, 0.f};
        const f32x2 xx = {x[0], x[1]};
        typedef const __attribute__((address_space(4))) float *scalar_f;
        const scalar_f sflt = (scalar_f)tab;
        scalar_f4 t4 = stab + 2 * (size_t)(b * B);
        scalar_f tf = sflt + (size_t)RT_WORDS * (b * B);
        f32x4 ca[4], cb[4];
        float sa[4], sb[4];
#pragma unroll
        for (int q = 0; q < 4; q++) ca[q] = t4[2 * q], sa[q] = tf[RT_WORDS * q + RT_C2];
        for (uint32_t j = 0; j < B; j += 8, t4 += 16, tf += 8 * RT_WORDS) {
#pragma unroll
          for (int q = 0; q < 4; q++) cb[q] = t4[2 * (4 + q)], sb[q] = tf[RT_WORDS * (4 + q) + RT_C2];
          __builtin_amdgcn_sched_barrier(0);
#pragma unroll
          for (int q = 0; q < 4; q++) run += rows_eval2(xx, ca[q], sa[q]);
          __builtin_amdgcn_sched_barrier(0);
#pragma unroll
          for (int q = 0; q < 4; q++) ca[q] = t4[2 * (8 + q)], sa[q] = tf[RT_WORDS * (8 + q) + RT_C2];
          __builtin_amdgcn_sched_barrier(0);
#pragma unroll
          for (int q = 0; q < 4; q++) run += rows_eval2(xx, cb[q], sb[q]);
          __builtin_amdgcn_sched_barrier(0);
        }
// ... 848 lines not shown
                               int32_t *__restrict__ z, uint64_t seed, uint64_t sweep, bool vec_ok) {
  const int lane = threadIdx.x & 63;
  const uint64_t wave_id = (uint64_t)blockIdx.x * 4 + (threadIdx.x >> 6);
  const uint64_t nwaves = (uint64_t)gridDim.x * 4;
  constexpr float kLog2e = 1.44269504088896340736f;
  float4 cur[NT], nxt[NT];
  auto fetch = [&](uint64_t row, float4 (&v)[NT]) {
    const float *s = scores + (row < nrows ? row : nrows - 1) * ld;
#pragma unroll
    for (int t = 0; t < NT; t++) v[t] = load_score4(s, (uint32_t)t * kGroupTile + 4 * lane, K, vec_ok);
  };
  if (wave_id < nrows) fetch(wave_id, cur);
  for (uint64_t row = wave_id; row < nrows; row += nwaves) {
    fetch(row + nwaves, nxt);
    if (NT == 1) {
      const float sc[4] = {cur[0].x, cur[0].y, cur[0].z, cur[0].w};
      const int pick1 = sample_from_scores<4>(sc, philox_uniform01(seed, sweep, row_id0 + row), lane, K);
      if (lane == 0) z[row] = pick1;
    } else {
      float m = -INFINITY;
#pragma unroll
      for (int t = 0; t < NT; t++) m = fmaxf(fmaxf(m, fmaxf(cur[t].x, cur[t].y)), fmaxf(cur[t].z, cur[t].w));
      m = wave_max(m);
      float p[NT][4], sum[NT], incl[NT];
      float total = 0.f;
#pragma unroll
      for (int t = 0; t < NT; t++) {
        p[t][0] = __builtin_amdgcn_exp2f((cur[t].x - m) * kLog2e);
        p[t][1] = __builtin_amdgcn_exp2f((cur[t].y - m) * kLog2e);
        p[t][2] = __builtin_amdgcn_exp2f((cur[t].z - m) * kLog2e);
        p[t][3] = __builtin_amdgcn_exp2f((cur[t].w - m) * kLog2e);
        sum[t] = ((p[t][0] + p[t][1]) + p[t][2]) + p[t][3];
        incl[t] = wave_incl_scan(sum[t], lane);
        total += lane_bcast(incl[t], 63);
      }
      const float dart = philox_uniform01(seed, sweep, row_id0 + row) * total;
      float before = 0.f;
      int pick = (int)K - 1;
      bool found = false;
#pragma unroll
      for (int t = 0; t < NT; t++) {
        const float tile_total = lane_bcast(incl[t], 63);
        if (!found && before + tile_total >= dart) {
          float c = before + (incl[t] - sum[t]);
          int nmiss = 0;
          c += p[t][0]; nmiss += c < dart ? 1 : 0;
          c += p[t][1]; nmiss += c < dart ? 1 : 0;
          c += p[t][2]; nmiss += c < dart ? 1 : 0;
          c += p[t][3]; nmiss += c < dart ? 1 : 0;
          const unsigned long long hit = __builtin_amdgcn_ballot_w64(nmiss < 4);
          if (hit != 0ull) {
            const int l = (int)__builtin_ctzll(hit);
            const int k = t * kGroupTile + 4 * l + lane_bcast(nmiss, l);
            pick = k < (int)K ? k : (int)K - 1;
            found = true;
          }
        }
        before += tile_total;
      }
      if (lane == 0) z[row] = pick;
    }
#pragma unroll
    for (int t = 0; t < NT; t++) cur[t] = nxt[t];
  }
}

__global__ __launch_bounds__(256) void k_sample_rows(const float *__restrict__ scores, uint64_t ld,
                                                      uint32_t K, uint64_t nrows, uint64_t row_id0,
                                                      int32_t *__restrict__ z,
                                                      const uint64_t *__restrict__ rng) {
  const uint64_t seed = rng[0], sweep = rng[1];
  const int lane = threadIdx.x & 63;
  const uint64_t wave_id = (uint64_t)blockIdx.x * 4 + (threadIdx.x >> 6);
  const uint64_t nwaves = (uint64_t)gridDim.x * 4;
  const uint32_t ntiles = (K + kGroupTile - 1) / kGroupTile;
  const bool vec_ok = ((ld & 3) == 0) && ((reinterpret_cast<uintptr_t>(scores) & 15) == 0);
  constexpr float kLog2e = 1.44269504088896340736f;
  if (ntiles == 1) return sample_rows_tiles<1>(scores, ld, K, nrows, row_id0, z, seed, sweep, vec_ok);
  if (ntiles == 2) return sample_rows_tiles<2>(scores, ld, K, nrows, row_id0, z, seed, sweep, vec_ok);
  if (ntiles == 3) return sample_rows_tiles<3>(scores, ld, K, nrows, row_id0, z, seed, sweep, vec_ok);
  if (ntiles == 4) return sample_rows_tiles<4>(scores, ld, K, nrows, row_id0, z, seed, sweep, vec_ok);
  for (uint64_t row = wave_id; row < nrows; row += nwaves) {
    const float *s = scores + row * ld;
    float m = -INFINITY;
    for (uint32_t t = 0; t < ntiles; t++) {
      const float4 v = load_score4(s, t * kGroupTile + 4 * lane, K, vec_ok);
      m = fmaxf(fmaxf(m, fmaxf(v.x, v.y)), fmaxf(v.z, v.w));
    }
    m = wave_max(m);
    float total = 0.f;
    for (uint32_t t = 0; t < ntiles; t++) {
      const float4 v = load_score4(s, t * kGroupTile + 4 * lane, K, vec_ok);
      const float sum = ((__builtin_amdgcn_exp2f((v.x - m) * kLog2e) + __builtin_amdgcn_exp2f((v.y - m) * kLog2e)) +
                         __builtin_amdgcn_exp2f((v.z - m) * kLog2e)) + __builtin_amdgcn_exp2f((v.w - m) * kLog2e);
      total += lane_bcast(wave_incl_scan(sum, lane), 63);
    }
    const float dart = philox_uniform01(seed, sweep, row_id0 + row) * total;
    float before = 0.f;
    int pick = (int)K - 1;
    for (uint32_t t = 0; t < ntiles; t++) {
      const float4 v = load_score4(s, t * kGroupTile + 4 * lane, K, vec_ok);
      const float p0 = __builtin_amdgcn_exp2f((v.x - m) * kLog2e), p1 = __builtin_amdgcn_exp2f((v.y - m) * kLog2e),
                  p2 = __builtin_amdgcn_exp2f((v.z - m) * kLog2e), p3 = __builtin_amdgcn_exp2f((v.w - m) * kLog2e);
      const float sum = ((p0 + p1) + p2) + p3;
      const float incl = wave_incl_scan(sum, lane);
      const float tile_total = lane_bcast(incl, 63);
      if (before + tile_total >= dart) {
        float c = before + (incl - sum);
        int nmiss = 0;
        c += p0; nmiss += c < dart ? 1 : 0;
        c += p1; nmiss += c < dart ? 1 : 0;
        c += p2; nmiss += c < dart ? 1 : 0;
        c += p3; nmiss += c < dart ? 1 : 0;
        const unsigned long long hit = __builtin_amdgcn_ballot_w64(nmiss < 4);
        if (hit != 0ull) {
          const int l = (int)__builtin_ctzll(hit);
          const int k = (int)(t * kGroupTile) + 4 * l + lane_bcast(nmiss, l);
          pick = k < (int)K ? k : (int)K - 1;
          break;
        }
      }
      before += tile_total;
    }
    if (lane == 0) z[row] = pick;
  }
}

static uint64_t grid_for(uint64_t work_items_per_wave_chunk, int num_cus, int waves_per_cu_cap) {
  uint64_t gx = (work_items_per_wave_chunk + 3) / 4;
  const uint64_t cap = (uint64_t)num_cus * waves_per_cu_cap / 4;
  if (gx > cap) gx = cap;
  return gx ? gx : 1;
}

size_t sweep_nich1_rows_table_floats(uint32_t kpad) {
  const RowsGeom g = rows_geom(kpad);
  return ((size_t)g.nb * g.B + 8) * RT_WORDS + 16;
}
uint32_t sweep_nich1_rows_max_groups() { return kRowsMaxK; }
int launch_sweep_nich1_rows(hipStream_t stream, int num_cus, const FeatDesc *feats_dev, uint32_t K, uint32_t kpad,
                            uint64_t row0, uint64_t nrows, uint64_t row_id0, int32_t *z, const float *crp,
                            const uint64_t *rng, ZeroSpans zero, float *table) {
  const RowsGeom g = rows_geom(kpad);
  hipLaunchKernelGGL(k_nich_rows_table, dim3(1), dim3(1024), 0, stream, feats_dev, K, kpad, crp, table, g.nb * g.B);
  uint64_t gx = (nrows + 255) / 256;
  const uint64_t cap = (uint64_t)num_cus * 10;
  if (gx > cap) gx = cap;
  if (gx == 0) gx = 1;
  hipLaunchKernelGGL(k_sweep_nich1_rows, dim3((unsigned)gx), dim3(128), 0, stream, feats_dev, K, kpad, row0, nrows, row_id0,
                     z, crp, rng, zero, table, g.B, g.nb);
  return launch_status("k_sweep_nich1_rows");
}

int launch_sweep_nich1(hipStream_t stream, int num_cus, bool transposed, const FeatDesc *feats_dev, uint32_t K,
                       uint32_t kpad, uint64_t row0, uint64_t nrows, uint64_t row_id0, int32_t *z,
                       const float *own, const float *crp, const uint64_t *rng, ZeroSpans zero) {
  if (K > 1024) return fail(MSC_EHIP, "launch_sweep_nich1: K = %u was routed here", K);
  if (transposed) {
    const uint64_t gxt = grid_for((nrows + kTRows - 1) / kTRows, num_cus, K <= 256 ? 16 : K <= 512 ? 12 : 8);
    const dim3 gridt((unsigned)gxt), blockt(256);
    if (K <= 64)
      hipLaunchKernelGGL(k_sweep_nich1_t<1>, (note_kernel(1, "k_sweep_nich1_t<1>"), gridt), blockt, 0, stream, feats_dev, K, kpad, row0, nrows, row_id0, z, crp, rng, zero);
    else if (K <= 128)
      hipLaunchKernelGGL(k_sweep_nich1_t<2>, (note_kernel(1, "k_sweep_nich1_t<2>"), gridt), blockt, 0, stream, feats_dev, K, kpad, row0, nrows, row_id0, z, crp, rng, zero);
    else if (K <= 256)
      hipLaunchKernelGGL(k_sweep_nich1_t<4>, (note_kernel(1, "k_sweep_nich1_t<4>"), gridt), blockt, 0, stream, feats_dev, K, kpad, row0, nrows, row_id0, z, crp, rng, zero);
    else if (K <= 512)
      hipLaunchKernelGGL(k_sweep_nich1_t<8>, (note_kernel(1, "k_sweep_nich1_t<8>"), gridt), blockt, 0, stream, feats_dev, K, kpad, row0, nrows, row_id0, z, crp, rng, zero);
    else
      hipLaunchKernelGGL(k_sweep_nich1_t<16>, (note_kernel(1, "k_sweep_nich1_t<16>"), gridt), blockt, 0, stream, feats_dev, K, kpad, row0, nrows, row_id0, z, crp, rng, zero);
    return launch_status("k_sweep_nich1_t");
  }
  int chunk_rows = 64;
  while (chunk_rows > 4 && (nrows + chunk_rows - 1) / chunk_rows < (uint64_t)num_cus * 32) chunk_rows >>= 1;
  const uint64_t gx = grid_for((nrows + chunk_rows - 1) / chunk_rows, num_cus, 16);
  const dim3 grid((unsigned)gx), block(256);
  if (K <= 64)
    hipLaunchKernelGGL(k_sweep_nich1<1>, (note_kernel(1, "k_sweep_nich1<1>"), grid), block, 0, stream, feats_dev, K, kpad, row0, nrows, row_id0, z, own, crp, rng, chunk_rows, zero);
  else if (K <= 128)
    hipLaunchKernelGGL(k_sweep_nich1<2>, (note_kernel(1, "k_sweep_nich1<2>"), grid), block, 0, stream, feats_dev, K, kpad, row0, nrows, row_id0, z, own, crp, rng, chunk_rows, zero);
  else if (K <= 256)
    hipLaunchKernelGGL(k_sweep_nich1<4>, (note_kernel(1, "k_sweep_nich1<4>"), grid), block, 0, stream, feats_dev, K, kpad, row0, nrows, row_id0, z, own, crp, rng, chunk_rows, zero);
  else if (K <= 512)
    hipLaunchKernelGGL(k_sweep_nich1<8>, (note_kernel(1, "k_sweep_nich1<8>"), grid), block, 0, stream, feats_dev, K, kpad, row0, nrows, row_id0, z, own, crp, rng, chunk_rows, zero);
  else
    hipLaunchKernelGGL(k_sweep_nich1<16>, (note_kernel(1, "k_sweep_nich1<16>"), grid), block, 0, stream, feats_dev, K, kpad, row0, nrows, row_id0, z, own, crp, rng, chunk_rows, zero);
  return launch_status("k_sweep_nich1");
}

static dim3 rows_grid(uint64_t nrows, uint64_t rows_per_wg, uint64_t cap) {
  return dim3((unsigned)std::max<uint64_t>(1, std::min<uint64_t>((nrows + rows_per_wg - 1) / rows_per_wg, cap)));
}

int launch_sweep_mixed(hipStream_t stream, int num_cus, bool has_dm, ScorePath path, const ScoreShape &shape, const FeatDesc *feats_dev, int nfeat, int nsplit,
                       uint32_t K, uint32_t kpad, uint64_t row0, uint64_t nrows, uint64_t row_id0, int32_t *z,
                       const float *own, const float *crp, const uint64_t *rng, ZeroSpans zero) {
  if (K > 256 || (shape.pair && K > 128)) return fail(MSC_EHIP, "launch_sweep_mixed: K = %u was routed here", K);
  const bool pair = shape.pair, small = shape.wave_rows < 8, small4 = shape.wave_rows == 4;
  const uint64_t cap = (uint64_t)num_cus * 4;
  const dim3 grid = rows_grid(nrows, has_dm ? 64 : small4 ? 64 : small ? 32 : 128, cap);
  if (has_dm)
    hipLaunchKernelGGL((k_sweep_tile<8, 8, true>), (note_kernel(1, "k_sweep_tile<8, 8, true>"), grid), dim3(512), 0, stream, feats_dev, nfeat, nsplit, K, kpad, row0, nrows,
                       row_id0, z, own, crp, rng, zero);
  else if (path == MSC_PATH_LOOKUPS && pair)
    hipLaunchKernelGGL((k_sweep_lookups<true>), (note_kernel(1, "k_sweep_lookups<true, 0>"), rows_grid(nrows, 512, cap)), dim3(1024), 0, stream,
                       feats_dev, nfeat, K, kpad, row0, nrows, row_id0, z, own, crp, rng, zero);
  else if (path == MSC_PATH_LOOKUPS && !small && !pair)
    hipLaunchKernelGGL((k_sweep_lookups<false>), (note_kernel(1, "k_sweep_lookups<false, 0>"), rows_grid(nrows, 256, cap)), dim3(1024), 0, stream,
                       feats_dev, nfeat, K, kpad, row0, nrows, row_id0, z, own, crp, rng, zero);
  else if (path == MSC_PATH_NICH_PACK && pair)
  {
    const dim3 g = rows_grid(nrows, 32 * kNichPackWaves, cap * (16 / kNichPackWaves));
    if (nsplit > 0)
      hipLaunchKernelGGL((k_sweep_nich_pack<true, true>), (note_kernel(1, "k_sweep_nich_pack<true, true, 0>"), g), dim3(kNichPackWaves * 64), 0, stream, feats_dev, nsplit, K, kpad, row0, nrows, row_id0, z, own, crp, rng, zero);
    else
      hipLaunchKernelGGL((k_sweep_nich_pack<true, false>), (note_kernel(1, "k_sweep_nich_pack<true, false, 0>"), g), dim3(kNichPackWaves * 64), 0, stream, feats_dev, nsplit, K, kpad, row0, nrows, row_id0, z, own, crp, rng, zero);
  }
  else if (path == MSC_PATH_NICH_PACK && !small && !pair)
  {
    const dim3 g = rows_grid(nrows, 16 * kNichPackWaves, cap * (16 / kNichPackWaves));
    if (nsplit > 0)
      hipLaunchKernelGGL((k_sweep_nich_pack<false, true>), (note_kernel(1, "k_sweep_nich_pack<false, true, 0>"), g), dim3(kNichPackWaves * 64), 0, stream, feats_dev, nsplit, K, kpad, row0, nrows, row_id0, z, own, crp, rng, zero);
    else
      hipLaunchKernelGGL((k_sweep_nich_pack<false, false>), (note_kernel(1, "k_sweep_nich_pack<false, false, 0>"), g), dim3(kNichPackWaves * 64), 0, stream, feats_dev, nsplit, K, kpad, row0, nrows, row_id0, z, own, crp, rng, zero);
  }
  else if (pair && path == MSC_PATH_TILE_ROLES)
    hipLaunchKernelGGL((k_sweep_tile_roles<0, true>), (note_kernel(1, "k_sweep_tile_roles<0, true>"), rows_grid(nrows, 256, cap)), dim3(1024), 0,
                       stream, feats_dev, nfeat, nsplit, K, kpad, row0, nrows, row_id0, z, own, crp, rng, zero, static_cast<const float *>(nullptr));
  else if (small4)
    hipLaunchKernelGGL((k_sweep_tile<4, 16, false>), (note_kernel(1, "k_sweep_tile<4, 16, false>"), grid), dim3(1024), 0, stream, feats_dev, nfeat, nsplit, K, kpad, row0, nrows,
                       row_id0, z, own, crp, rng, zero);
  else if (small)
    hipLaunchKernelGGL((k_sweep_tile<2, 16, false>), (note_kernel(1, "k_sweep_tile<2, 16, false>"), grid), dim3(1024), 0, stream, feats_dev, nfeat, nsplit, K, kpad, row0, nrows,
                       row_id0, z, own, crp, rng, zero);
  else if (path == MSC_PATH_TILE_ROLES)
    hipLaunchKernelGGL(k_sweep_tile_roles<0>, (note_kernel(1, "k_sweep_tile_roles<0, false>"), grid), dim3(1024), 0, stream, feats_dev, nfeat, nsplit, K, kpad, row0, nrows,
                       row_id0, z, own, crp, rng, zero, static_cast<const float *>(nullptr));
  else
    hipLaunchKernelGGL((k_sweep_tile<8, 16, false>), (note_kernel(1, "k_sweep_tile<8, 16, false>"), grid), dim3(1024), 0, stream, feats_dev, nfeat, nsplit, K, kpad, row0, nrows,
                       row_id0, z, own, crp, rng, zero);
  return launch_status("sweep kernel");
}

int launch_sweep_roles_tail(hipStream_t stream, int num_cus, ScorePath path, const FeatDesc *feats_dev, int nfeat, int nsplit, uint32_t K,
                            uint32_t kpad, uint64_t row0, uint64_t nrows, uint64_t row_id0, int32_t *z, const float *own,
                            const float *crp, const uint64_t *rng, ZeroSpans zero, const float *tail) {
  const uint64_t cap = (uint64_t)num_cus * 4;
  const bool wide = K > (uint32_t)kGroupTile + 64;
  if (path == MSC_PATH_LOOKUPS) {
    const dim3 g = rows_grid(nrows, 256, cap);
    if (!wide) hipLaunchKernelGGL((k_sweep_lookups<false, 1>), (note_kernel(1, "k_sweep_lookups<false, 1>"), g), dim3(1024), 0, stream, feats_dev, nfeat, K, kpad, row0, nrows, row_id0, z, own, crp, rng, zero, tail);
    else hipLaunchKernelGGL((k_sweep_lookups<false, 2>), (note_kernel(1, "k_sweep_lookups<false, 2>"), g), dim3(1024), 0, stream, feats_dev, nfeat, K, kpad, row0, nrows, row_id0, z, own, crp, rng, zero, tail);
    return launch_status("sweep kernel");
  }
  if (path == MSC_PATH_NICH_PACK) {
    const dim3 g = rows_grid(nrows, 16 * kNichPackWaves, cap * (16 / kNichPackWaves));
    const dim3 b(kNichPackWaves * 64);
    if (nsplit > 0) {
      if (!wide) hipLaunchKernelGGL((k_sweep_nich_pack<false, true, 1>), (note_kernel(1, "k_sweep_nich_pack<false, true, 1>"), g), b, 0, stream, feats_dev, nsplit, K, kpad, row0, nrows, row_id0, z, own, crp, rng, zero, tail);
      else hipLaunchKernelGGL((k_sweep_nich_pack<false, true, 2>), (note_kernel(1, "k_sweep_nich_pack<false, true, 2>"), g), b, 0, stream, feats_dev, nsplit, K, kpad, row0, nrows, row_id0, z, own, crp, rng, zero, tail);
    } else {
      if (!wide) hipLaunchKernelGGL((k_sweep_nich_pack<false, false, 1>), (note_kernel(1, "k_sweep_nich_pack<false, false, 1>"), g), b, 0, stream, feats_dev, nsplit, K, kpad, row0, nrows, row_id0, z, own, crp, rng, zero, tail);
      else hipLaunchKernelGGL((k_sweep_nich_pack<false, false, 2>), (note_kernel(1, "k_sweep_nich_pack<false, false, 2>"), g), b, 0, stream, feats_dev, nsplit, K, kpad, row0, nrows, row_id0, z, own, crp, rng, zero, tail);
    }
    return launch_status("sweep kernel");
  }
  if (!wide)
    hipLaunchKernelGGL(k_sweep_tile_roles<1>, (note_kernel(1, "k_sweep_tile_roles<1, false>"), rows_grid(nrows, 128, cap)), dim3(1024), 0, stream, feats_dev, nfeat, nsplit, K, kpad,
                       row0, nrows, row_id0, z, own, crp, rng, zero, tail);
  else
    hipLaunchKernelGGL(k_sweep_tile_roles<2>, (note_kernel(1, "k_sweep_tile_roles<2, false>"), rows_grid(nrows, 128, cap)), dim3(1024), 0, stream, feats_dev, nfeat, nsplit, K, kpad,
                       row0, nrows, row_id0, z, own, crp, rng, zero, tail);
  return launch_status("sweep kernel");
}

int launch_sample_rows(hipStream_t stream, int num_cus, const float *scores, uint64_t ld, uint32_t K,
                       uint64_t nrows, uint64_t row_id0, int32_t *z, const uint64_t *rng) {
  const uint64_t gx = grid_for(nrows, num_cus, 32);
  hipLaunchKernelGGL(k_sample_rows, dim3((unsigned)gx), dim3(256), 0, stream, scores, ld, K, nrows, row_id0,
                     z, rng);
  return hipGetLastError() == hipSuccess ? 0 : -1;
}

__global__ void k_rng_set(uint64_t *rng, uint64_t seed, uint64_t sweep) {
  rng[0] = seed;
  rng[1] = sweep;
}
__global__ void k_rng_bump(uint64_t *rng) { rng[1] += 1; }
int launch_rng_set(hipStream_t stream, uint64_t *rng, uint64_t seed, uint64_t sweep) {
  hipLaunchKernelGGL(k_rng_set, dim3(1), dim3(1), 0, stream, rng, seed, sweep);
  return hipGetLastError() == hipSuccess ? 0 : -1;
}
int launch_rng_bump(hipStream_t stream, uint64_t *rng) {
  hipLaunchKernelGGL(k_rng_bump, dim3(1), dim3(1), 0, stream, rng);
  return hipGetLastError() == hipSuccess ? 0 : -1;
}

}
```

common_amd/csrc/launchers.hpp:

```cpp
#pragma once
#include <algorithm>

#include "msc_internal.hpp"

namespace msc {

inline bool first_use_on_device(unsigned long long &seen) {
  int dev = 0;
  if (hipGetDevice(&dev) != hipSuccess || dev < 0 || dev > 63) return true;
  const unsigned long long bit = 1ull << dev;
  if (seen & bit) return false;
  seen |= bit;
  return true;
}

struct UnpackFeat {
  void *dst;
  uint8_t *dst_mask;
  uint32_t offset;
  uint32_t mask_offset;
  int32_t src_type, dst_type;
  uint32_t count;
  uint32_t pad;
};

struct MailboxHeader {
  int32_t family, dim, op, status;
  float score;
  uint32_t hp_off, ss_off, value_off;
};
int launch_value_op(hipStream_t stream, void *mailbox_dev, uint32_t dim, int family);

int bind_error_word_score(uint32_t *word_dev);
int bind_error_word_sweep(uint32_t *word_dev);
int bind_error_word_state(uint32_t *word_dev);
int bind_error_word_seq(uint32_t *word_dev);
int bind_error_word_query(uint32_t *word_dev);

int launch_prepare(hipStream_t stream, const FeatDesc *feats_dev, uint32_t nfeat, uint32_t kpad, uint32_t value_slices);
int launch_dm_prepare(hipStream_t stream, const FeatDesc *feats_dev, int f, uint32_t dim, uint32_t kpad, uint32_t value_slices);
int launch_crp_prepare(hipStream_t stream, const uint32_t *cnt, uint32_t K, uint32_t kpad, float alpha,
                       float *crp);
int launch_entity_op(hipStream_t stream, const FeatDesc *feats_dev, int nfeat, uint32_t K, uint32_t kpad, uint64_t row,
                     uint32_t group, int sign, long long *cnt_acc, uint32_t *cnt_u32, float alpha, float *crp, int32_t *z_slot);
int launch_set_i32(hipStream_t stream, int32_t *dst, int32_t value);
constexpr int kLooRows = 4, kLooThreads = 1024;
int launch_loo_own(hipStream_t stream, bool heavy, bool staged, const FeatDesc *feats_dev, int nfeat, uint32_t K, uint32_t kpad, uint64_t row0,
                   uint64_t nrows, const int32_t *z, const float *crp, float *own);
int launch_gp_large_fix(hipStream_t stream, int num_cus, const FeatDesc *feats_dev, int f, uint32_t K,
                        uint32_t kpad, uint64_t row0, uint64_t nrows, const int32_t *z, float *out, uint64_t ld);
struct Nich1Shape { int q, visits; };
constexpr int kNich1NumShapes = 8;
extern const Nich1Shape kNich1Shapes[kNich1NumShapes];
constexpr uint32_t kTailMaxGroups = 128;
constexpr uint64_t kNarrowMaxRows = 65536;
constexpr uint64_t kTailMinRows = 16384;
constexpr uint32_t kTailStride = 65;
inline double tile_rounds_us(uint64_t workgroups, int num_cus, bool sweep, const PlanCost &pc = PlanCost()) {
  return (sweep ? pc.sweep_round_us : pc.tile_round_us) * (double)((workgroups + (uint64_t)num_cus - 1) / (uint64_t)num_cus);
}
inline double tail_rows_us(uint32_t groups, bool exact, uint64_t nrows, int num_cus, const PlanCost &pc = PlanCost()) {
  const uint32_t widest = exact ? 32u : 64u, nblk = (groups + widest - 1) / widest;
  const uint32_t per = ((groups + nblk - 1) / nblk + 15u) / 16u * 16u;
  const double frac = (double)nrows / (1024.0 * num_cus);
  const double rounds = frac >= 1.0 ? frac : std::max(0.6, 0.4 + 0.6 * frac);
  return (double)nblk * (pc.tail_fixed_us + pc.tail_group_us * per) * rounds;
}
struct TailPlan {
  bool ok = false;
  bool exact = true;
  bool masked_nich = false;
  bool dm = false;
  uint32_t max_rows = 0;
  uint32_t pack_rows = 0;
  float *pack = nullptr;
};
int launch_score_tail(hipStream_t stream, int num_cus, const TailPlan &tp, const FeatDesc *feats_dev, int nfeat, int nsplit, uint32_t K,
                      uint32_t kpad, uint32_t k0, uint64_t row0, uint64_t nrows, const int32_t *z, const float *own, const float *crp,
                      float *out, uint64_t ld);
struct ZeroSpans {
  unsigned long long *a = nullptr;
  size_t na = 0;
  unsigned long long *b = nullptr;
  size_t nb = 0;
};
int launch_sweep_rows(hipStream_t stream, int num_cus, const TailPlan &tp, const FeatDesc *feats_dev, int nfeat, int nsplit, uint32_t K,
                      uint32_t kpad, uint64_t row0, uint64_t nrows, uint64_t row_id0, int32_t *z, const float *own, const float *crp,
                      const uint64_t *rng, ZeroSpans zero);
int launch_score_pair_tail(hipStream_t stream, int num_cus, const FeatDesc *feats_dev, int nfeat, int nsplit, uint32_t K, uint32_t kpad,
                           uint64_t row0, uint64_t nrows, const int32_t *z, const float *own, const float *crp, float *tail, uint64_t ld);
enum class LastTile { tiles, rows, pair };
struct ScoreShape { int wave_rows = 8; bool pair = false; LastTile last = LastTile::tiles; int nich1 = 0; };
int launch_score(hipStream_t stream, int num_cus, ScorePath path, const TailPlan &narrow_tail, const ScoreShape &shape, const FeatDesc *feats_dev, int nfeat, int nsplit,
                 uint32_t K, uint32_t kpad, uint64_t row0, uint64_t nrows, const int32_t *z,
                 const float *own, const float *crp, float *out, uint64_t ld);

void note_kernel(int slot, const char *fmt, ...) __attribute__((format(printf, 2, 3)));
const char *last_kernel(int slot);
inline const char *tf(bool b) { return b ? "true" : "false"; }
inline int launch_status(const char *what) {
  const hipError_t e = hipGetLastError();
  return e == hipSuccess ? 0 : fail(MSC_EHIP, "%s launch failed: %s", what, hipGetErrorString(e));
}

int launch_sweep_nich1(hipStream_t stream, int num_cus, bool transposed, const FeatDesc *feats_dev, uint32_t K,
                       uint32_t kpad, uint64_t row0, uint64_t nrows, uint64_t row_id0, int32_t *z,
                       const float *own, const float *crp, const uint64_t *rng_dev, ZeroSpans zero);
#ifndef MSC_NICH_PACK_WAVES
#define MSC_NICH_PACK_WAVES 8
#endif
constexpr int kNichPackWaves = MSC_NICH_PACK_WAVES;
#ifndef MSC_NICH_PACK_NC
#define MSC_NICH_PACK_NC 4
#endif
constexpr int kPackMaxLookups = 4;
constexpr int kNichPackNC = MSC_NICH_PACK_NC;
constexpr double kPairTileShare = 0.62;
int launch_sweep_mixed(hipStream_t stream, int num_cus, bool has_dm, ScorePath path, const ScoreShape &shape, const FeatDesc *feats_dev, int nfeat, int nsplit,
                       uint32_t K, uint32_t kpad, uint64_t row0, uint64_t nrows, uint64_t row_id0, int32_t *z,
                       const float *own, const float *crp, const uint64_t *rng, ZeroSpans zero);
int launch_sweep_roles_tail(hipStream_t stream, int num_cus, ScorePath path, const FeatDesc *feats_dev, int nfeat, int nsplit, uint32_t K,
                            uint32_t kpad, uint64_t row0, uint64_t nrows, uint64_t row_id0, int32_t *z, const float *own,
                            const float *crp, const uint64_t *rng, ZeroSpans zero, const float *tail);
int sweep_niw1_max_groups(uint32_t dim);
size_t sweep_nich1_rows_table_floats(uint32_t kpad);
uint32_t sweep_nich1_rows_max_groups();
int launch_sweep_nich1_rows(hipStream_t stream, int num_cus, const FeatDesc *feats_dev, uint32_t K, uint32_t kpad,
                            uint64_t row0, uint64_t nrows, uint64_t row_id0, int32_t *z, const float *crp,
                            const uint64_t *rng, ZeroSpans zero, float *table);
int launch_sweep_niw1(hipStream_t stream, int num_cus, uint32_t dim, const FeatDesc *feats_dev, uint32_t K, uint32_t kpad,
                      uint64_t row0, uint64_t nrows, uint64_t row_id0, int32_t *z, const float *crp, const uint64_t *rng,
                      ZeroSpans zero);
int launch_narrow(hipStream_t stream, int num_cus, int lanes_per_row, uint32_t table_rows, bool sweep, const FeatDesc *feats_dev,
                  int nfeat, uint32_t K, uint32_t kpad, uint64_t row0, uint64_t nrows, const int32_t *z, const float *own,
                  const float *crp, float *out, uint64_t ld, uint64_t row_id0, int32_t *z_out, const uint64_t *rng,
                  ZeroSpans zero);
int launch_sample_rows(hipStream_t stream, int num_cus, const float *scores, uint64_t ld, uint32_t K,
                       uint64_t nrows, uint64_t row_id0, int32_t *z, const uint64_t *rng_dev);
int launch_rng_set(hipStream_t stream, uint64_t *rng_dev, uint64_t seed, uint64_t sweep);
int launch_rng_bump(hipStream_t stream, uint64_t *rng_dev);

constexpr int kSeqThreads = 256;
constexpr uint32_t kSeqMaxGroups = 8192;
constexpr int kSeqMaxFeat = 256;
int launch_sweep_seq(hipStream_t stream, const FeatDesc *feats_dev, int nfeat, uint32_t K, uint32_t kpad, uint64_t row0,
                     uint64_t nrows, uint64_t row_id0, int32_t *z, const uint32_t *order, uint64_t v0, uint64_t v1,
                     uint64_t seed, uint64_t sweep, long long *cnt_acc, uint32_t *cnt_u32, float alpha, float *crp,
                     int32_t *trace);

int launch_niw_prepare(hipStream_t stream, const FeatDesc *feats_dev, uint32_t f, uint32_t dim, uint32_t K,
                       uint32_t kpad);
int launch_niw_score_data(hipStream_t stream, const FeatDesc *feats_dev, uint32_t f, uint32_t K,
                          uint32_t kpad, float *out);
int launch_niw_score(hipStream_t stream, int num_cus, const FeatDesc *feats_dev, uint32_t f, uint32_t dim, uint32_t K,
                     uint32_t kpad, uint64_t row0, uint64_t nrows, const int32_t *z, bool accum, bool f32_fast,
                     double *qown , float *out, uint64_t ld);
int launch_niw_accumulate(hipStream_t stream, int num_cus, const FeatDesc *feats_dev, uint32_t f, uint32_t K,
                          uint64_t row0, uint64_t nrows, const int32_t *z, int sign, uint32_t *scratch_dev, uint32_t dim);
int launch_niw_commit(hipStream_t stream, const FeatDesc *feats_dev, uint32_t f, uint32_t dim, uint32_t K,
                      uint32_t kpad, int to_raw);

int launch_accumulate(hipStream_t stream, int num_cus, const FeatDesc *feats_dev,
                      const FeatDesc *feats_host, int nfeat, uint32_t K, uint32_t kpad, uint64_t row0,
                      uint64_t nrows, const int32_t *z, int sign, long long *cnt_acc);
int launch_commit(hipStream_t stream, const FeatDesc *feats_dev, int nfeat, uint32_t kpad,
                  const long long *cnt_acc, uint32_t *cnt_u32);
int launch_commit_prepare(hipStream_t stream, const FeatDesc *feats_dev, int nfeat, uint32_t K, uint32_t kpad,
                          const long long *cnt_acc, uint32_t *cnt_u32, float alpha, float *crp, uint64_t *rng_bump,
                          uint32_t value_slices);
int launch_pack64(hipStream_t stream, bool unpack, long long *i64, size_t ni, double *f64, size_t nf, double *pack);
int launch_zero64(hipStream_t stream, void *a, size_t na, void *b, size_t nb);
int launch_stream_fill(hipStream_t stream, int num_cus, void *buf, size_t nbytes);
int launch_lift(hipStream_t stream, const FeatDesc *feats_dev, int nfeat, uint32_t kpad,
                long long *cnt_acc, const uint32_t *cnt_u32, int lift_cnt);
int launch_score_data(hipStream_t stream, const FeatDesc *feats_dev, int nfeat, uint32_t K,
                      uint32_t kpad, float *out);
int launch_relation_blocks(hipStream_t stream, uint32_t ndim, const uint64_t *shape, const int32_t *const *z_dev,
                           const uint32_t *ngroups, const uint32_t *positions_dev, uint64_t ncells, int32_t *out_dev);
int launch_relation_slice_scores(hipStream_t stream, const float *scores, uint64_t ld, uint32_t ndim, const uint64_t *shape,
                                 uint32_t dim, const uint32_t *seg_dev, const uint32_t *ids_dev, const int32_t *off_dev,
                                 uint32_t ncand, uint32_t cand_stride, uint64_t nent, float *out_dev, uint64_t ld_out);
int launch_dm_stats(hipStream_t stream, const uint32_t *col, uint64_t n, uint32_t dim, uint32_t *colmax_dev,
                    uint32_t *rowtot_dev);
int launch_col_max_u32(hipStream_t stream, const uint32_t *col, uint64_t n, uint32_t *out_dev);
int launch_mask_sentinel(hipStream_t stream, const void *col, const uint8_t *mask, uint64_t n, bool bytes, uint32_t sentinel, void *out);
int launch_pack_bits(hipStream_t stream, const void *const *cols, int m, uint32_t radix, uint64_t n, void *out);
int launch_pack_nich_x(hipStream_t stream, const float *const *cols_dev, uint32_t n2, uint32_t n2p, uint64_t n, float *out);
int launch_pack_look_idx(hipStream_t stream, const LookIdxSrc *src_dev, uint32_t nsrc, uint32_t l4, uint64_t n, uint32_t *out);
int launch_fuse_tables(hipStream_t stream, const FeatDesc *feats_dev, int nsplit, int nblocks, uint32_t kpad);
int launch_hp_grid_score(hipStream_t stream, const HpJob *jobs_dev, uint32_t njobs, uint32_t max_points, uint32_t K,
                         uint32_t kpad, const uint32_t *cnt, const uint8_t *slots, uint32_t nblk, double *part,
                         double *out);
int launch_crp_grid_score(hipStream_t stream, const HpJob *job_dev, uint32_t npoints, const uint32_t *cnt, uint32_t K,
                          double *out);
int launch_hp_grid_draw(hipStream_t stream, const HpJob *jobs_dev, uint32_t njobs, const double *scores, uint64_t seed,
                        uint64_t sweep, uint32_t *chosen);
int launch_hp_slice(hipStream_t stream, const SliceTarget *targets_dev, uint32_t ntargets, const SliceCoord *coords_dev,
                    uint32_t K, uint32_t kpad, const uint32_t *cnt, const uint8_t *slots, uint64_t key, uint64_t sweep,
                    float *values, uint32_t *evals, uint32_t *status);
inline uint32_t theta_slice_blocks(uint32_t K) { return (K + 255) / 256; }
int launch_theta_slice(hipStream_t stream, const ThetaJob *jobs_dev, uint32_t njobs, uint32_t K, uint32_t kpad,
                       const uint32_t *cnt, const uint8_t *slots, uint64_t key, uint64_t sweep,
                       unsigned long long *evals_part, uint32_t *bad_part);
int launch_unpack(hipStream_t stream, const uint8_t *records, const uint8_t *mask, uint64_t nrows,
                  uint32_t rowsize, uint32_t maskrowsize, const void *feats_dev, uint32_t nfeat);

int launch_pred_prepare(hipStream_t stream, const PredFeat *pfs_dev, const std::vector<PredFeat> &pfs, uint32_t K,
                        uint32_t kpad);
int launch_pred_sample(hipStream_t stream, const PredFeat *pfs_dev, const std::vector<PredFeat> &pfs, uint32_t K,
                       uint64_t row0, uint64_t nrows, uint64_t row_id0, const int32_t *z, int32_t *z_out,
                       bool masked_only, uint64_t seed, uint64_t sweep);

int launch_marginal_norm(hipStream_t stream, const uint32_t *cnt, uint32_t K, float alpha, double *norm);
int launch_marginal_nich1(hipStream_t stream, int num_cus, const FeatDesc *feats_dev, uint32_t K, uint32_t kpad, uint64_t row0,
                          uint64_t nrows, const int32_t *z, const float *crp, const double *norm, float *logp, int32_t *map,
                          float *logresp);
int launch_marginal_tile(hipStream_t stream, int num_cus, const FeatDesc *feats_dev, int nfeat, int nsplit, uint32_t K,
                         uint32_t kpad, uint64_t row0, uint64_t nrows, const int32_t *z, const float *own, const float *crp,
                         const double *norm, float *logp, int32_t *map, float *logresp);
int launch_row_lse(hipStream_t stream, int num_cus, const float *scores, uint64_t ld, uint32_t K, uint64_t nrows,
                   const int32_t *z, const double *norm, float *logp, int32_t *map, float *logresp);

constexpr uint32_t kZmTile = 64;
constexpr uint32_t kZmBatchWords = 256;
constexpr uint32_t kZmBatchMax = 4 * kZmBatchWords;
constexpr uint32_t kZmMaxRows = 1u << 18;
constexpr uint32_t kZmMaxLabels = 1u << 16;
inline uint32_t zm_batch_cap(bool wide) { return (wide ? 2u : 4u) * kZmBatchWords; }
int launch_zm_stage(hipStream_t stream, const int32_t *z, uint64_t ld, uint32_t nsamples, const uint32_t *rows,
                    uint32_t m, uint32_t nlabels, bool wide, uint32_t slot0, uint32_t *bad, uint32_t *batch);
int launch_zm_count(hipStream_t stream, const uint32_t *batch, uint32_t nt, bool wide, uint32_t staged,
                    const uint32_t *bad, uint32_t *counts);
int launch_zm_finish(hipStream_t stream, const uint32_t *counts, uint32_t nt, uint32_t m, const uint32_t *order,
                     bool norm, float S, void *out, uint64_t ld);

}
```

common_amd/csrc/msc_internal.hpp:

```cpp
#pragma once

#include <hip/hip_runtime.h>

#include <cstdarg>
#include <cstdint>
#include <cstdio>
#include <cstring>
#include <string>
#include <vector>

#include "../../include/microscopes_hip.h"
#include "dev_buf.hpp"

namespace msc {

constexpr int kWave = 64;
constexpr int kGroupTile = 256;
constexpr unsigned kMaxDDDim = 128;
constexpr int kGrpRows = 128;
constexpr unsigned kGpMaxTable = 1024;
constexpr float kNtFastGbps = 6650.f;

void set_error(const char *fmt, ...);
int fail(int code, const char *fmt, ...);
// ... 211 lines not shown
    case MSC_GP: return 1;
    case MSC_BBNC: return 1;
    case MSC_DM: return 1;
    case MSC_NICH: return 2;
    default: return 0;
  }
}
inline uint32_t acc_i64_rows(int family, uint32_t dim) {
  switch (family) {
    case MSC_BB: return 2;
    case MSC_BBNC: return 2;
    case MSC_GP: return 2;
    case MSC_BNB: return 2;
    case MSC_DM: return dim;
    case MSC_DD: return dim;
    case MSC_NICH: return 1;
    case MSC_NIW: return 1;
    default: return 0;
  }
}
inline uint32_t acc_f64_rows(int family) {
  switch (family) {
    case MSC_GP: return 1;
    case MSC_DM: return 1;
    case MSC_NICH: return 2;
    default: return 0;
  }
}
inline int value_type_of(int family) {
  switch (family) {
    case MSC_BB: return MSC_TYPE_B;
    case MSC_BBNC: return MSC_TYPE_B;
    case MSC_GP: return MSC_TYPE_U32;
    case MSC_BNB: return MSC_TYPE_U32;
    case MSC_DM: return MSC_TYPE_I32;
    case MSC_DD: return MSC_TYPE_I32;
    case MSC_NICH: return MSC_TYPE_F32;
    case MSC_NIW: return MSC_TYPE_F32;
    default: return MSC_TYPE_B;
  }
}
size_t primitive_size(int t);

enum { NIW_C0 = 0, NIW_C1 = 1, NIW_A_LOO = 2, NIW_B_LOO = 3, NIW_C_LOO = 4, NIW_LOGDET_HI = 5, NIW_LOGDET_LO = 6,
       NIW_ROWS = 7 };
constexpr int kNiwPad = 32;
constexpr unsigned kMaxNiwDim = 128;

__host__ __device__ inline uint32_t niw_blocks(uint32_t d) { return (d + 15u) / 16u; }
__host__ __device__ inline uint32_t niw_chunks(uint32_t d) { return niw_blocks(d) * (niw_blocks(d) + 1u) / 2u; }
__host__ __device__ inline size_t niw_w_stream(uint32_t d) { return (size_t)niw_chunks(d) * 256u; }
__host__ __device__ inline size_t niw_b_stream(uint32_t d) { return (size_t)niw_blocks(d) * 256u; }
__host__ __device__ inline size_t niw_w_index(uint32_t i, uint32_t j) {
  const uint32_t b = i >> 4, s4 = j >> 4;
  return (size_t)(b * (b + 1u) / 2u + s4) * 256u + (size_t)((i & 15u) + 16u * (j & 3u)) * 4u + ((j & 15u) >> 2);
}
__host__ __device__ inline size_t niw_b_index(uint32_t i) {
  return (size_t)(i >> 4) * 256u + (size_t)(16u * (i & 3u)) * 4u + ((i & 15u) >> 2);
}

}

struct msc_context {
  int device = 0;
  hipStream_t stream = nullptr;
  int num_cus = 256;
  struct ShapeEntry { const void *out; uint64_t nrows; uint32_t K; int shape; int plain_stores; };
  std::vector<ShapeEntry> nich1_shapes;
  struct Placed { const void *base; size_t size; bool nt_fast; };
  std::vector<Placed> placed;
  hipStream_t record_stream = nullptr;
  struct VmmAlloc { void *va; size_t size; std::vector<hipMemGenericAllocationHandle_t> handles; };
  std::vector<VmmAlloc> vmm;
  std::vector<float> last_alloc_rates;
  uint32_t last_alloc_chosen = 0;
  msc::MappedBuf<unsigned char> mailbox_host;
  void *mailbox_dev = nullptr;
  msc::MappedBuf<uint32_t> sync_word_host;
  void *sync_word_dev = nullptr;
  uint32_t sync_seq = 0;
  bool sync_word_ok = true;
  volatile uint32_t *err_host = nullptr;
};

struct msc_dataview {
  msc_context *ctx = nullptr;
  uint64_t serial = 0;
  uint64_t nrows = 0;
  std::vector<msc_runtime_type> types;
  std::vector<void *> cols;
  std::vector<void *> masks;
  std::vector<msc::DevBuf<uint8_t>> owned;
  mutable std::vector<long long> col_max;
  mutable std::vector<std::vector<uint32_t>> dm_max;
  enum CopyKind : uint32_t {
    kConverted,
    kSentinel,
    kPackedBits,
    kNichX,
    kLookIdx,
    kDmTot,
    kDmMax,
  };
  struct Copy {
    CopyKind kind;
    std::vector<uint64_t> key;
    msc::DevBuf<uint8_t> buf;
  };
  mutable std::vector<Copy> copies;
};

struct msc_feature_host {
  int family = 0;
  uint32_t dim = 0;
  std::vector<float> hp;
  msc::DevBuf<float> hp_dev;
  msc::DevBuf<float> tab;
  msc::DevBuf<uint32_t> raw_u32;
  msc::DevBuf<float> raw_f32;
  msc::DevBuf<double> loo64;
  msc::DevBuf<float> loo_tab;
  msc::DevBuf<float> niw_w, niw_b;
  msc::DevBuf<double> niw_w64, niw_mu64, niw_c64;
  size_t i64_off = 0, i64_len = 0;
  size_t f64_off = 0, f64_len = 0;
  msc::DevBuf<uint32_t> dm_meta_dev;
  std::vector<uint32_t> dm_meta;
  bool raw_valid = true;
  bool additive_valid = false;
  bool derived_valid = false;
};

struct msc_state;
struct msc_hp_grid {
  msc_state *st = nullptr;
  uint32_t feature = 0;
  std::vector<float> blocks;
  msc::DevBuf<float> grid_dev;
  msc::DevBuf<double> logprior_dev;
  msc::HpJob job;
  msc::DevBuf<msc::HpJob> job_dev;
};

struct msc_state {
  msc_context *ctx = nullptr;
  uint32_t nfeat = 0, K = 0, kpad = 0;
  float alpha = 1.f;
  std::vector<msc_feature_host> feats;
  bool nich1 = false, has_dm = false;
  uint32_t n_niw = 0;
  msc::DevBuf<long long> red_i64;
  msc::DevBuf<double> red_f64;
  size_t n_i64 = 0, n_f64 = 0;
  msc::DevBuf<double> red_pack;
  uint64_t sweep_rows_hint = 0;
  std::vector<std::vector<uint32_t>> col_bounds;
  bool rebind = false;
  msc::DevBuf<uint32_t> cnt_u32;
  msc::DevBuf<float> logpc;
  bool cnt_additive_valid = false;
  bool crp_valid = false;
  msc::DevBuf<msc::FeatDesc> desc_dev;
  std::vector<msc::FeatDesc> desc_host;
  msc::DevBuf<msc::FeatDesc> desc_tile_dev;
  std::vector<msc::FeatDesc> desc_tile_host;
  uint32_t tile_split = 0;
  msc::DevBuf<msc::FeatDesc> desc_fuse_dev;
  std::vector<msc::FeatDesc> desc_fuse_host;
  uint32_t fuse_nfeat = 0, fuse_split = 0;
  bool fuse_any = false;
  msc::DevBuf<float> fuse_tab;
  msc::DevBuf<msc::FeatDesc> desc_acc_dev;
  std::vector<msc::FeatDesc> desc_acc_host;
  msc::DevBuf<msc::NichPlanInfo> nich_info;
  msc::DevBuf<float> rn_pack;
  msc::DevBuf<msc::NichPos> rn_pos;
  bool nich_blocks_any = false;
  const msc_dataview *bound_view = nullptr;
  uint64_t bound_serial = 0;
  std::vector<uint32_t> bound_cols;
  msc::Retired retired;
  msc::DevBuf<float> scratch;
  msc::DevBuf<float> tail_scores;
  msc::DevBuf<float> own;
  msc::ScorePath tile_path = msc::MSC_PATH_TILE;
  msc::PlanCost plan_cost;
  bool tile_narrow_tail_ok = false;
  uint32_t tail_max_rows = 0, tail_pack_rows = 0;
  bool tail_masked_nich = false;
  bool tail_dm = false;
  msc::DevBuf<float> tail_pack;
  uint32_t loo_staged = 0;
  msc::DevBuf<double> marg_norm;
  msc::DevBuf<float> rows_table;
  msc::DevBuf<uint32_t> colmax_dev;
  msc::DevBuf<uint64_t> rng_dev;
  uint64_t rng_seed = 0, rng_sweep = 0;
  bool rng_valid = false;
  bool rng_bump_pending = false;
  uint64_t rng_next_sweep = 0;
  struct StepGraph {
    hipGraphExec_t exec = nullptr;
    const void *view = nullptr, *z = nullptr;
    uint64_t view_serial = 0, row0 = 0, nrows = 0, row_id0 = 0;
    float alpha = 0.f;
    std::vector<uint32_t> cols;
    std::vector<uint8_t> flags;
    int seen = 0;
    bool disabled = false;
    uint64_t n_eager = 0, n_replayed = 0;
  } step_graph;
  msc::DevBuf<double> niw_qown;
  msc::DevBuf<int32_t> one_z;
  msc::DevBuf<uint32_t> niw_scratch;
  std::vector<std::unique_ptr<msc_hp_grid>> hp_grids;
  msc::DevBuf<double> hp_part;
  msc::DevBuf<double> hp_out;
  msc::DevBuf<msc::HpJob> hp_jobs_dev;
  msc::DevBuf<uint32_t> hp_chosen_dev;
  std::vector<msc::HpJob> hp_jobs_host;
  msc::DevBuf<unsigned char> slice_buf;
  msc::DevBuf<msc::PredFeat> pred_feats_dev;
  msc::DevBuf<double> pred_par;
  msc::DevBuf<int32_t> pred_z;
  std::vector<msc::PredFeat> pred_feats_host;
  msc::PinnedBuf<msc::PredFeat> pred_stage;
  hipEvent_t pred_upload = nullptr;
  bool pred_upload_pending = false;
};

struct msc_zmatrix {
  msc_context *ctx = nullptr;
  uint64_t n = 0;
  uint32_t m = 0, nlabels = 0, nt = 0;
  bool wide = false;
  msc::DevBuf<uint32_t> rows_dev;
  msc::DevBuf<uint32_t> order_dev;
  msc::DevBuf<uint32_t> batch;
  msc::DevBuf<uint32_t> bad;
  msc::DevBuf<uint32_t> counts;
  uint32_t staged = 0;
  uint64_t nsamples = 0;
};
```

Before: 1744 billion.

## Fuse sufficient-statistic accumulation into the nich1 sweep kernel

For single-NICH-feature states, the sweep kernel now builds per-block LDS histograms of group size, sum x and sum x² for the new assignments. It flushes them atomically into a staging buffer, and the last block (found with a ticket counter) copies the staged totals into the reduction table. The separate zero and accumulate launches after the sweep are then skipped. This removes a pass over z and the data column plus extra kernel launches, at the cost of LDS and global atomics, dynamic shared memory and a last-block epilogue in the sweep kernel.

```diff
diff --git a/common_amd/csrc/abi.cpp b/common_amd/csrc/abi.cpp
--- a/common_amd/csrc/abi.cpp
+++ b/common_amd/csrc/abi.cpp
@@ -38,6 +38,7 @@
 
 struct Switches {
   bool tail_forced = false, no_narrow_tail = false, no_bb_fuse = false, sweep_graph = false;
+  bool sweep_acc_fused = true;
   uint64_t tail_min_rows = 0;
   int loo_lds = -1, sweep_nich1 = 0, alloc_candidates = 12;
   int marginal_tile = -1;
@@ -52,6 +53,7 @@
   if (const char *e = std::getenv("MSC_SWEEP_NICH1")) sw.sweep_nich1 = std::atoi(e);
   if (const char *e = std::getenv("MSC_MARGINAL_TILE")) sw.marginal_tile = std::atoi(e);
   if (const char *g = std::getenv("MSC_SWEEP_GRAPH")) sw.sweep_graph = g[0] != '0' && g[0] != 0;
+  if (const char *e = std::getenv("MSC_SWEEP_ACC_FUSED")) sw.sweep_acc_fused = e[0] != '0' && e[0] != 0;
   if (const char *e = std::getenv("MSC_ALLOC_CANDIDATES")) sw.alloc_candidates = std::atoi(e);
   if (const char *e = std::getenv("MSC_ALLOC_ACCEPT_GBPS")) sw.alloc_accept_gbps = (float)std::atof(e);
   return sw;
@@ -1095,6 +1097,11 @@
   for (const msc_feature_host &h : st->feats) st->has_dm |= h.family == MSC_DM, st->n_niw += h.family == MSC_NIW;
   MSC_TRY(alloc_zeroed(st->red_i64, n_i64));
   MSC_TRY(alloc_zeroed(st->red_f64, n_f64));
+  if (st->nich1) {
+    MSC_TRY(alloc_zeroed(st->stage_i64, n_i64));
+    MSC_TRY(alloc_zeroed(st->stage_f64, n_f64));
+    MSC_TRY(alloc_zeroed(st->stage_ticket, 1));
+  }
   MSC_TRY(alloc_zeroed(st->cnt_u32, kpad));
   MSC_TRY(alloc_zeroed(st->logpc, crp_floats(st->kpad)));
   MSC_TRY(alloc_zeroed(st->desc_dev, nfeatures));
@@ -1887,7 +1894,7 @@
   return MSC_OK;
 }
 
-enum : uint32_t { kAccZeroed = 0x100, kAccThenPrepare = 0x200 };
+enum : uint32_t { kAccZeroed = 0x100, kAccThenPrepare = 0x200, kAccInPlace = 0x400 };
 
 static int commit_and_prepare(msc_state *st, bool bump_rng = true) {
   hipStream_t s = st->ctx->stream;
@@ -1912,7 +1919,8 @@
                            uint64_t nrows, const int32_t *z_dev, uint32_t flags) {
   MSC_TRY(bind_view(st, view, cols, row0, nrows));
   hipStream_t s = st->ctx->stream;
-  if (flags & MSC_ACC_RESET) {
+  if (flags & kAccInPlace) {
+  } else if (flags & MSC_ACC_RESET) {
     if (!(flags & kAccZeroed) && launch_zero64(s, st->red_i64, st->n_i64, st->red_f64, st->n_f64))
       return fail(MSC_EHIP, "k_zero64 launch failed");
   } else {
@@ -1930,7 +1938,7 @@
   }
   for (auto &h : st->feats) h.additive_valid = true;
   st->cnt_additive_valid = true;
-  if (nrows > 0) {
+  if (nrows > 0 && !(flags & kAccInPlace)) {
     const int rc = launch_accumulate(s, st->ctx->num_cus, st->desc_acc_dev, st->desc_acc_host.data(), (int)st->desc_acc_host.size(),
                                      st->K, st->kpad, row0, nrows, z_dev,
                                      (flags & MSC_ACC_SUBTRACT) ? -1 : 1, st->red_i64);
@@ -2056,11 +2064,12 @@
   SweepKind kind = SweepKind::generic;
   int lanes = 0; uint32_t table_rows = 0;
   bool transposed = false;
+  bool accumulates = false;
   ScoreShape shape;
   uint64_t tail_ld = 0;
   bool tail_pair = false;
 };
-static SweepRoute route_sweep(const msc_state *st, uint64_t nrows) {
+static SweepRoute route_sweep(const msc_state *st, uint64_t nrows, bool in_step = false) {
   const Switches sw = read_switches();
   const uint64_t cus = (uint64_t)st->ctx->num_cus;
   SweepRoute r;
@@ -2070,6 +2079,7 @@
     if (st->nich1) {
       r.kind = st->K > 1024 ? SweepKind::nich1_rows : SweepKind::nich1;
       r.transposed = sw.sweep_nich1 == 2 || (sw.sweep_nich1 != 1 && view_rows(st) >= cus * 64);
+      r.accumulates = in_step && r.kind == SweepKind::nich1 && sw.sweep_acc_fused;
     } else if ((r.lanes = narrow_lanes(st, sw, &r.table_rows)) != 0) {
       r.kind = SweepKind::narrow;
     } else if (narrow_tail_fits(st) && st->K <= kTailMaxGroups && sweep_rows_pays(st, sw, st->K)) {
@@ -2092,7 +2102,8 @@
 
 static int sweep_assign_impl(msc_state *st, const msc_dataview *view, const uint32_t *cols, uint64_t row0,
                              uint64_t nrows, uint64_t row_id0, int32_t *z_dev, uint64_t seed, uint64_t sweep,
-                             bool *zeroed = nullptr) {
+                             bool *zeroed = nullptr, bool *accumulated = nullptr) {
+  if (accumulated) *accumulated = false;
   MSC_TRY(bind_view(st, view, cols, row0, nrows));
   if (nrows == 0) return MSC_OK;
   if (!st->rng_valid || st->rng_seed != seed || st->rng_sweep != sweep) {
@@ -2110,7 +2121,8 @@
     zero.a = reinterpret_cast<unsigned long long *>(st->red_i64.get()); zero.na = st->n_i64;
     zero.b = reinterpret_cast<unsigned long long *>(st->red_f64.get()); zero.nb = st->n_f64;
   }
-  const SweepRoute r = route_sweep(st, nrows);
+  const SweepRoute r = route_sweep(st, nrows, zeroed != nullptr);
+  if (accumulated) *accumulated = r.accumulates;
   bool zeroes = true;
   switch (r.kind) {
     case SweepKind::niw1:
@@ -2120,9 +2132,22 @@
       MSC_HIP(grow_retained(st->retired, st->rows_table, sweep_nich1_rows_table_floats(st->kpad)));
       MSC_TRY(launch_sweep_nich1_rows(s, cus, st->desc_dev, st->K, st->kpad, row0, nrows, row_id0, z_dev, st->logpc, st->rng_dev, zero, st->rows_table));
       break;
-    case SweepKind::nich1:
-      MSC_TRY(launch_sweep_nich1(s, cus, r.transposed, st->desc_dev, st->K, st->kpad, row0, nrows, row_id0, z_dev, st->own, st->logpc, st->rng_dev, zero));
+    case SweepKind::nich1: {
+      AccFuse acc;
+      if (r.accumulates) {
+        acc.table_i64 = reinterpret_cast<unsigned long long *>(st->red_i64.get());
+        acc.stage_i64 = reinterpret_cast<unsigned long long *>(st->stage_i64.get());
+        acc.n_i64 = st->n_i64;
+        acc.table_f64 = st->red_f64.get();
+        acc.stage_f64 = st->stage_f64.get();
+        acc.n_f64 = st->n_f64;
+        acc.ticket = st->stage_ticket.get();
+        acc.masked = st->desc_host[0].mask != nullptr;
+      }
+      MSC_TRY(launch_sweep_nich1(s, cus, r.transposed, st->desc_dev, st->K, st->kpad, row0, nrows, row_id0, z_dev, st->own, st->logpc, st->rng_dev, zero,
+                                 r.accumulates ? &acc : nullptr));
       break;
+    }
     case SweepKind::narrow:
       MSC_TRY(run_loo_own(st, row0, nrows, z_dev, true));
       MSC_TRY(launch_narrow(s, cus, r.lanes, r.table_rows, true, st->desc_dev, (int)st->nfeat, st->K, st->kpad, row0, nrows, z_dev,
@@ -2226,11 +2251,12 @@
   hipStream_t s = st->ctx->stream;
   auto eager = [&]() -> int {
     st->step_graph.n_eager++;
-    bool zeroed = false;
-    MSC_TRY(sweep_assign_impl(st, view, cols, row0, nrows, row_id0, z_dev, seed, sweep, &zeroed));
+    bool zeroed = false, in_place = false;
+    MSC_TRY(sweep_assign_impl(st, view, cols, row0, nrows, row_id0, z_dev, seed, sweep, &zeroed, &in_place));
     st->rng_valid = false;
     MSC_TRY(accumulate_impl(st, view, cols, row0, nrows, z_dev,
-                            MSC_ACC_RESET | kAccThenPrepare | (zeroed ? (uint32_t)kAccZeroed : 0u)));
+                            MSC_ACC_RESET | kAccThenPrepare | (zeroed ? (uint32_t)kAccZeroed : 0u) |
+                                (in_place ? (uint32_t)kAccInPlace : 0u)));
     st->rng_valid = true;
     st->rng_sweep = sweep + 1;
     return MSC_OK;
@@ -2304,13 +2330,14 @@
   MSC_HIP(hipSetDevice(st->ctx->device));
   MSC_TRY(device_error_check(st->ctx));
   if (nrows == 0) return accumulate_impl(st, view, cols, row0, 0, z_dev, MSC_ACC_RESET | MSC_ACC_NO_COMMIT);
-  bool zeroed = false;
-  MSC_TRY(sweep_assign_impl(st, view, cols, row0, nrows, row_id0, z_dev, seed, sweep, &zeroed));
+  bool zeroed = false, in_place = false;
+  MSC_TRY(sweep_assign_impl(st, view, cols, row0, nrows, row_id0, z_dev, seed, sweep, &zeroed, &in_place));
   st->rng_valid = false;
   st->rng_bump_pending = true;
   st->rng_next_sweep = sweep + 1;
   return accumulate_impl(st, view, cols, row0, nrows, z_dev,
-                         MSC_ACC_RESET | MSC_ACC_NO_COMMIT | (zeroed ? (uint32_t)kAccZeroed : 0u));
+                         MSC_ACC_RESET | MSC_ACC_NO_COMMIT | (zeroed ? (uint32_t)kAccZeroed : 0u) |
+                             (in_place ? (uint32_t)kAccInPlace : 0u));
 }
 
 extern "C" int msc_sweep_step_stats(const msc_state *st, uint64_t *eager_steps, uint64_t *graph_steps) {
diff --git a/common_amd/csrc/kernels_sweep.hip b/common_amd/csrc/kernels_sweep.hip
--- a/common_amd/csrc/kernels_sweep.hip
+++ b/common_amd/csrc/kernels_sweep.hip
@@ -143,6 +143,58 @@
 }
 
 
+struct AccHist {
+  double *sx, *sx2;
+  uint32_t *size, *count;
+};
+MSC_DEV AccHist acc_hist_zero(unsigned char *lds, uint32_t K, bool masked) {
+  AccHist h;
+  h.sx = reinterpret_cast<double *>(lds);
+  h.sx2 = h.sx + K;
+  h.size = reinterpret_cast<uint32_t *>(h.sx2 + K);
+  h.count = masked ? h.size + K : h.size;
+  for (uint32_t i = threadIdx.x; i < K; i += blockDim.x) {
+    h.sx[i] = 0.0;
+    h.sx2[i] = 0.0;
+    h.size[i] = 0u;
+    h.count[i] = 0u;
+  }
+  return h;
+}
+MSC_DEV void acc_hist_add(const AccHist &h, uint32_t K, bool separate_count, int pick, float xv, bool row_masked) {
+  if ((uint32_t)pick >= K) return;
+  atomicAdd(&h.size[pick], 1u);
+  if (row_masked) return;
+  if (separate_count) atomicAdd(&h.count[pick], 1u);
+  const double x = xv;
+  atomicAdd(&h.sx[pick], x);
+  atomicAdd(&h.sx2[pick], x * x);
+}
+MSC_DEV void acc_flush_and_close(const AccHist &h, const AccFuse &a, uint32_t K, uint32_t kpad) {
+  __syncthreads();
+  for (uint32_t i = threadIdx.x; i < K; i += blockDim.x) {
+    const uint32_t n = h.size[i], c = h.count[i];
+    if (n) atomicAdd(&a.stage_i64[i], (unsigned long long)n);
+    if (c) atomicAdd(&a.stage_i64[(size_t)kpad + i], (unsigned long long)c);
+    const double s1 = h.sx[i], s2 = h.sx2[i];
+    if (s1 != 0.0) atomicAdd(&a.stage_f64[i], s1);
+    if (s2 != 0.0) atomicAdd(&a.stage_f64[(size_t)kpad + i], s2);
+  }
+  asm volatile("s_waitcnt vmcnt(0)" ::: "memory");
+  __syncthreads();
+  if (threadIdx.x == 0) {
+    const unsigned t = __hip_atomic_fetch_add(a.ticket, 1u, __ATOMIC_RELAXED, __HIP_MEMORY_SCOPE_AGENT);
+    h.size[0] = t == gridDim.x - 1u ? 1u : 0u;
+  }
+  __syncthreads();
+  if (h.size[0] == 0u) return;
+  unsigned long long *si = a.stage_i64, *sf = reinterpret_cast<unsigned long long *>(a.stage_f64);
+  unsigned long long *ti = a.table_i64, *tf = reinterpret_cast<unsigned long long *>(a.table_f64);
+  for (size_t i = threadIdx.x; i < a.n_i64; i += blockDim.x) ti[i] = atomicExch(&si[i], 0ull);
+  for (size_t i = threadIdx.x; i < a.n_f64; i += blockDim.x) tf[i] = atomicExch(&sf[i], 0ull);
+  if (threadIdx.x == 0) __hip_atomic_store(a.ticket, 0u, __ATOMIC_RELAXED, __HIP_MEMORY_SCOPE_AGENT);
+}
+
 template <int G>
 __global__ __launch_bounds__(256, G == 16 ? 3 : 1) void k_sweep_nich1(const FeatDesc *__restrict__ feats, uint32_t K,
                                                       uint32_t kpad, uint64_t row0, uint64_t nrows,
@@ -151,98 +203,21 @@
                                                       const float *__restrict__ crp,
                                                       const uint64_t *__restrict__ rng, int chunk_rows,
                                                       ZeroSpans zero) {
-  const uint64_t seed = rng[0], sweep = rng[1];
-  zero_spans(zero);
-  const FeatDesc fd = feats[0];
-  const int lane = threadIdx.x & 63;
-  const uint32_t kb = (uint32_t)(G * lane);
-  float mh[G], ml[G], c0[G], c1[G], c2[G];
-  bool empty[G];
-#pragma unroll
-  for (int j = 0; j < G; j++) {
-    const uint32_t k = kb + j;
-    const size_t kc = k < kpad ? k : 0;
-    mh[j] = fd.tab[(size_t)NICH_MU_HI * kpad + kc];
-    ml[j] = fd.tab[(size_t)NICH_MU_LO * kpad + kc];
-    c0[j] = fd.tab[(size_t)NICH_C0 * kpad + kc];
-    c1[j] = fd.tab[(size_t)NICH_C1 * kpad + kc];
-    c2[j] = fd.tab[(size_t)NICH_C2 * kpad + kc];
-    const float lcj = crp[kc];
-    empty[j] = __builtin_isinf(lcj);
-    c0[j] += empty[j] ? 0.f : lcj;
-  }
-  const float le0 = crp[2 * (size_t)kpad], le1 = crp[2 * (size_t)kpad + 1];
-  constexpr float kLog2e = 1.44269504088896340736f;
-  const bool any_empty = !__builtin_isinf(le0);
-  const float dle = any_empty ? (le1 - le0) * kLog2e : 0.f;
-  float c0s[G];
-  unsigned emask = 0u;
-  float bound = -INFINITY;
-#pragma unroll
-  for (int j = 0; j < G; j++) {
-    if (empty[j] && kb + j < K) emask |= 1u << j;
-    c0s[j] = (kb + j >= K) ? -INFINITY : (c0[j] + (empty[j] ? le0 : 0.f)) * kLog2e;
-    if (kb + j < K) bound = fmaxf(bound, c0s[j]);
-  }
-  bound = wave_max(bound) + 16.f;
-#pragma unroll
-  for (int j = 0; j < G; j++) c0s[j] -= bound;
-  const float *xcol = reinterpret_cast<const float *>(fd.col) + row0;
-  const uint64_t nchunks = (nrows + chunk_rows - 1) / chunk_rows;
-  const uint64_t wave_id = (uint64_t)blockIdx.x * 4 + (threadIdx.x >> 6);
-  const uint64_t nwaves = (uint64_t)gridDim.x * 4;
-  for (uint64_t chunk = wave_id; chunk < nchunks; chunk += nwaves) {
-    const uint64_t rb = chunk * chunk_rows;
-    const int nr = (int)((nrows - rb) < (uint64_t)chunk_rows ? (nrows - rb) : (uint64_t)chunk_rows);
-    const bool has_row = lane < nr;
-    const float xv = has_row ? xcol[rb + lane] : 0.0f;
-    int gz = has_row ? z[rb + lane] : -1;
-    if ((uint32_t)gz >= K) gz = -1;
-    const float u01 = philox_uniform01(seed, sweep, row_id0 + rb + lane);
-    const unsigned long long mbits =
-        __builtin_amdgcn_ballot_w64(fd.mask != nullptr && has_row && fd.mask[row0 + rb + lane] != 0);
-    float sloo = 0.f;
-    bool single = false;
-    if (gz >= 0) {
-      const float lm1 = crp[kpad + gz];
-      single = __builtin_isinf(lm1);
-      double s = single ? (double)le1 + (double)crp[2 * (size_t)kpad + 3] : (double)lm1 + (double)crp[crp_lo_cntm1(kpad) + gz];
-      if (!((mbits >> lane) & 1ull))
-        s += nich_loo_tab(fd.hp, fd.loo64 + (size_t)gz * kNlooStride, 1, xv);
-      sloo = (float)s * kLog2e - bound;
-    }
-    const unsigned long long singles = any_empty ? __builtin_amdgcn_ballot_w64(single) : 0ull;
-    const unsigned long long odd = mbits | singles;
-    int znew = gz;
-    for (int r = 0; r < nr; r++) {
-      const float x = lane_bcast(xv, r), sl = lane_bcast(sloo, r);
-      const int g = lane_bcast(gz, r);
-      float s[G];
-#pragma unroll
-      for (int j = 0; j < G; j++) s[j] = nich_eval_log2(x, mh[j], ml[j], c0s[j], c1[j], c2[j]);
-      if ((odd >> r) & 1ull) {
-        if ((mbits >> r) & 1ull) {
-          const float e_raw = ((singles >> r) & 1ull) ? le1 : le0;
-#pragma unroll
-          for (int j = 0; j < G; j++) {
-            const float lcj = crp[kb + j < kpad ? kb + j : 0];
-            s[j] = (kb + j >= K) ? -INFINITY : (__builtin_isinf(lcj) ? e_raw : lcj) * kLog2e - bound;
-          }
-        } else {
-#pragma unroll
-          for (int j = 0; j < G; j++) s[j] += ((emask >> j) & 1u) ? dle : 0.f;
-        }
-      }
-      if (g >= 0 && lane == g / G) {
-#pragma unroll
-        for (int j = 0; j < G; j++)
-          if (j == g % G) s[j] = sl;
-      }
-      const int pick = sample_from_scores<G, true, true, true>(s, lane_bcast(u01, r), lane, K);
-      if (lane == r) znew = pick;
-    }
-    if (has_row) z[rb + lane] = znew;
-  }
+#define MSC_BODY_ACC 0
+#include "sweep_nich1_body.inc"
+#undef MSC_BODY_ACC
+}
+template <int G>
+__global__ __launch_bounds__(256, G == 16 ? 3 : 1) void k_sweep_nich1_acc(const FeatDesc *__restrict__ feats, uint32_t K,
+                                                      uint32_t kpad, uint64_t row0, uint64_t nrows,
+                                                      uint64_t row_id0, int32_t *__restrict__ z,
+                                                      const float *__restrict__ own,
+                                                      const float *__restrict__ crp,
+                                                      const uint64_t *__restrict__ rng, int chunk_rows,
+                                                      AccFuse acc) {
+#define MSC_BODY_ACC 1
+#include "sweep_nich1_body.inc"
+#undef MSC_BODY_ACC
 }
 
 constexpr int kTRows = 32;
@@ -306,164 +281,28 @@
                                                         uint64_t row0, uint64_t nrows, uint64_t row_id0,
                                                         int32_t *z, const float *__restrict__ crp,
                                                         const uint64_t *__restrict__ rng, ZeroSpans zero) {
-  constexpr int TR = kTRows;
-  __shared__ float lsum[4][TR * kTPad];
-  __shared__ float cst[64 * G * kTCst];
-  const uint64_t seed = rng[0], sweep = rng[1];
-  zero_spans(zero);
-  const FeatDesc fd = feats[0];
-  const int lane = threadIdx.x & 63, wave = __builtin_amdgcn_readfirstlane(threadIdx.x >> 6);
-  float *mysum = lsum[wave];
-  constexpr float kLog2e = 1.44269504088896340736f;
-  const float le0 = crp[2 * (size_t)kpad], le1 = crp[2 * (size_t)kpad + 1];
-  const bool any_empty = !__builtin_isinf(le0);
-  const float dle = any_empty ? (le1 - le0) * kLog2e : 0.f;
-  for (uint32_t k = threadIdx.x; k < 64u * G; k += 256u) {
-    const uint32_t kc = k < kpad ? k : 0u;
-    const float lc = crp[kc];
-    float *c = cst + k * kTCst;
-    c[TC_MH] = fd.tab[NICH_MU_HI * kpad + kc];
-    c[TC_ML] = fd.tab[NICH_MU_LO * kpad + kc];
-    c[TC_C0] = k < K ? (fd.tab[NICH_C0 * kpad + kc] + (__builtin_isinf(lc) ? le0 : lc)) * kLog2e : -INFINITY;
-    c[TC_C1] = fd.tab[NICH_C1 * kpad + kc];
-    c[TC_C2] = fd.tab[NICH_C2 * kpad + kc];
-  }
-  __syncthreads();
-  NichConsts<G> mine;
-  mine.emask = 0u;
-  float bound = -INFINITY;
-#pragma unroll
-  for (int j = 0; j < G; j++) {
-    const uint32_t k = (uint32_t)(G * lane + j);
-    const float *c = cst + k * kTCst;
-    mine.mh[j] = c[TC_MH], mine.ml[j] = c[TC_ML], mine.c0s[j] = c[TC_C0], mine.c1[j] = c[TC_C1], mine.c2[j] = c[TC_C2];
-    if (k < K && __builtin_isinf(crp[k])) mine.emask |= 1u << j;
-    bound = fmaxf(bound, mine.c0s[j]);
-  }
-  bound = wave_max(bound) + 16.f;
-#pragma unroll
-  for (int j = 0; j < G; j++) mine.c0s[j] -= bound;
-  const float *xcol = reinterpret_cast<const float *>(fd.col) + row0;
-  const uint64_t wave_id = (uint64_t)blockIdx.x * 4 + wave, nwaves = (uint64_t)gridDim.x * 4;
-  const uint64_t per = nrows / nwaves, extra = nrows % nwaves;
-  const uint64_t rbeg = wave_id * per + (wave_id < extra ? wave_id : extra), rend = rbeg + per + (wave_id < extra ? 1 : 0);
-  for (uint64_t rb = rbeg; rb < rend; rb += 64) {
-    const int nr = __builtin_amdgcn_readfirstlane((int)((rend - rb) < 64u ? (rend - rb) : 64u));
-    const bool has_row = lane < nr;
-    const float xv = has_row ? xcol[rb + lane] : 0.0f;
-    int gz = has_row ? z[rb + lane] : -1;
-    if ((uint32_t)gz >= K) gz = -1;
-    const float u01 = philox_uniform01(seed, sweep, row_id0 + rb + lane);
-    const bool my_mask = fd.mask != nullptr && has_row && fd.mask[row0 + rb + lane] != 0;
-    const unsigned long long mbits = __builtin_amdgcn_ballot_w64(my_mask);
-    float sloo = 0.f;
-    bool single = false;
-    if (gz >= 0) {
-      const float lm1 = crp[kpad + gz];
-      single = __builtin_isinf(lm1);
-      float s = single ? le1 : lm1;
-      if (!my_mask) s += nich_loo_tab_sweep(fd.hp, fd.loo64 + (size_t)gz * kNlooStride, 1, xv);
-      sloo = s * kLog2e - bound;
-    }
-    const bool my_single = single && any_empty;
-    const unsigned long long singles = __builtin_amdgcn_ballot_w64(my_single);
-    const unsigned long long odd = mbits | singles;
-    const bool plain = !(my_mask || my_single);
-    const NichRowCtx rc = {fd.tab, crp, K, kpad, le0, le1, dle, bound, xv, my_mask, my_single};
-    auto entry = [&](int k) -> float {
-      const float *c = cst + k * kTCst;
-      float s = nich_eval_log2_est(xv, c[TC_MH], c[TC_ML], c[TC_C0] - bound, c[TC_C1], c[TC_C2]);
-      if (!plain) s = nich_entry_log2(rc, (uint32_t)k);
-      return __builtin_amdgcn_exp2f(k == gz ? sloo : s);
-    };
-    const int own_lane = gz >= 0 ? gz / G : -1;
-    float own_sum = 0.f;
-    if (own_lane >= 0) {
-      own_sum = entry(G * own_lane);
-#pragma unroll
-      for (int j = 1; j < G; j++) own_sum += entry(G * own_lane + j);
-    }
-    int pick = gz;
-    bool redo = false;
-    for (int h0 = 0; h0 < nr; h0 += TR) {
-      const int h1 = h0 + TR < nr ? h0 + TR : nr;
-      __builtin_amdgcn_s_waitcnt(0);
-      for (int r = h0; r < h1; r++) {
-        const float x = lane_bcast(xv, r);
-        float s[G];
-        if ((odd >> r) & 1ull) {
-          nich_row_scores<G>(s, mine, x, ((mbits >> r) & 1ull) != 0, ((singles >> r) & 1ull) != 0, dle, -1, 0.f, crp, K, kpad,
-                             (uint32_t)lane, le0, le1, bound);
-        } else {
-#pragma unroll
-          for (int j = 0; j < G; j++) s[j] = nich_eval_log2_est(x, mine.mh[j], mine.ml[j], mine.c0s[j], mine.c1[j], mine.c2[j]);
-        }
-        float sum = __builtin_amdgcn_exp2f(s[0]);
-#pragma unroll
-        for (int j = 1; j < G; j++) sum += __builtin_amdgcn_exp2f(s[j]);
-        mysum[(r - h0) * kTPad + lane] = sum;
-      }
-      __builtin_amdgcn_wave_barrier();
-      if (lane >= h0 && lane < h1) {
-        float *row = mysum + (lane - h0) * kTPad;
-        if (own_lane >= 0) row[own_lane] = own_sum;
-        float blk[8], total = 0.f;
-#pragma unroll
-        for (int b = 0; b < 8; b++) {
-          float t = row[8 * b];
-#pragma unroll
-          for (int i = 1; i < 8; i++) t += row[8 * b + i];
-          blk[b] = t;
-          total = b == 0 ? t : total + t;
-        }
-        if (total > 0x1p-60f && total < 0x1p100f) {
-          const float dart = u01 * total;
-          float c0 = 0.f;
-          int b0 = 0;
-#pragma unroll
-          for (int b = 0; b < 7; b++) {
-            const bool miss = b0 == b && c0 + blk[b] < dart;
-            c0 = miss ? c0 + blk[b] : c0;
-            b0 += miss ? 1 : 0;
-          }
-          int hl = 8 * b0;
-#pragma unroll
-          for (int i = 0; i < 7; i++) {
-            const float v = row[8 * b0 + i];
-            const bool miss = hl == 8 * b0 + i && c0 + v < dart;
-            c0 = miss ? c0 + v : c0;
-            hl += miss ? 1 : 0;
-          }
-          int j0 = 0;
-#pragma unroll
-          for (int j = 0; j < G - 1; j++) {
-            const float v = entry(G * hl + j);
-            const bool miss = j0 == j && c0 + v < dart;
-            c0 = miss ? c0 + v : c0;
-            j0 += miss ? 1 : 0;
-          }
-          const int k = G * hl + j0;
-          pick = k < (int)K ? k : (int)K - 1;
-        } else {
-          redo = true;
-        }
-      }
-      __builtin_amdgcn_wave_barrier();
-    }
-    unsigned long long todo = __builtin_amdgcn_ballot_w64(redo);
-    while (todo != 0ull) {
-      const int r = (int)__builtin_ctzll(todo);
-      todo &= todo - 1ull;
-      const float x = lane_bcast(xv, r);
-      const int g = lane_bcast(gz, r);
-      float s[G];
-      nich_row_scores<G>(s, mine, x, ((mbits >> r) & 1ull) != 0, ((singles >> r) & 1ull) != 0, dle,
-                         (g >= 0 && lane == g / G) ? g % G : -1, lane_bcast(sloo, r), crp, K, kpad, (uint32_t)lane, le0, le1, bound);
-      const int p = sample_from_scores<G, true, false>(s, lane_bcast(u01, r), lane, K);
-      if (lane == r) pick = p;
-    }
-    if (has_row) z[rb + lane] = pick;
-  }
+#define MSC_BODY_ACC 0
+#define MSC_BODY_TR kTRows
+#include "sweep_nich1_t_body.inc"
+#undef MSC_BODY_TR
+#undef MSC_BODY_ACC
+}
+#ifndef MSC_ACC_TR4
+#define MSC_ACC_TR4 28
+#endif
+constexpr int kTRowsAcc4 = MSC_ACC_TR4;
+template <int G>
+constexpr int acc_trows() { return G == 4 ? kTRowsAcc4 : kTRows; }
+template <int G>
+__global__ __launch_bounds__(256) void k_sweep_nich1_t_acc(const FeatDesc *__restrict__ feats, uint32_t K, uint32_t kpad,
+                                                            uint64_t row0, uint64_t nrows, uint64_t row_id0,
+                                                            int32_t *z, const float *__restrict__ crp,
+                                                            const uint64_t *__restrict__ rng, AccFuse acc) {
+#define MSC_BODY_ACC 1
+#define MSC_BODY_TR acc_trows<G>()
+#include "sweep_nich1_t_body.inc"
+#undef MSC_BODY_TR
+#undef MSC_BODY_ACC
 }
 
 #ifndef MSC_DBG_ALWAYS_REDO
@@ -1618,40 +1457,61 @@
   return launch_status("k_sweep_nich1_rows");
 }
 
+template <typename Kern>
+static void allow_large_lds(Kern kern, unsigned long long &seen) {
+  if (!first_use_on_device(seen)) return;
+  if (hipFuncSetAttribute(reinterpret_cast<const void *>(kern), hipFuncAttributeMaxDynamicSharedMemorySize,
+                          (int)sweep_nich1_acc_lds_bytes(1024, true)) != hipSuccess)
+    (void)hipGetLastError();
+}
 int launch_sweep_nich1(hipStream_t stream, int num_cus, bool transposed, const FeatDesc *feats_dev, uint32_t K,
                        uint32_t kpad, uint64_t row0, uint64_t nrows, uint64_t row_id0, int32_t *z,
-                       const float *own, const float *crp, const uint64_t *rng, ZeroSpans zero) {
+                       const float *own, const float *crp, const uint64_t *rng, ZeroSpans zero, const AccFuse *acc) {
   if (K > 1024) return fail(MSC_EHIP, "launch_sweep_nich1: K = %u was routed here", K);
+  const size_t hist = acc ? sweep_nich1_acc_lds_bytes(K, acc->masked) : 0;
   if (transposed) {
     const uint64_t gxt = grid_for((nrows + kTRows - 1) / kTRows, num_cus, K <= 256 ? 16 : K <= 512 ? 12 : 8);
     const dim3 gridt((unsigned)gxt), blockt(256);
-    if (K <= 64)
-      hipLaunchKernelGGL(k_sweep_nich1_t<1>, (note_kernel(1, "k_sweep_nich1_t<1>"), gridt), blockt, 0, stream, feats_dev, K, kpad, row0, nrows, row_id0, z, crp, rng, zero);
-    else if (K <= 128)
-      hipLaunchKernelGGL(k_sweep_nich1_t<2>, (note_kernel(1, "k_sweep_nich1_t<2>"), gridt), blockt, 0, stream, feats_dev, K, kpad, row0, nrows, row_id0, z, crp, rng, zero);
-    else if (K <= 256)
-      hipLaunchKernelGGL(k_sweep_nich1_t<4>, (note_kernel(1, "k_sweep_nich1_t<4>"), gridt), blockt, 0, stream, feats_dev, K, kpad, row0, nrows, row_id0, z, crp, rng, zero);
-    else if (K <= 512)
-      hipLaunchKernelGGL(k_sweep_nich1_t<8>, (note_kernel(1, "k_sweep_nich1_t<8>"), gridt), blockt, 0, stream, feats_dev, K, kpad, row0, nrows, row_id0, z, crp, rng, zero);
-    else
-      hipLaunchKernelGGL(k_sweep_nich1_t<16>, (note_kernel(1, "k_sweep_nich1_t<16>"), gridt), blockt, 0, stream, feats_dev, K, kpad, row0, nrows, row_id0, z, crp, rng, zero);
-    return launch_status("k_sweep_nich1_t");
+#define MSC_NICH1_T(Gv)                                                                                                       \
+    do {                                                                                                                      \
+      if (acc) {                                                                                                              \
+        static unsigned long long seen = 0;                                                                                   \
+        allow_large_lds(k_sweep_nich1_t_acc<Gv>, seen);                                                                       \
+        hipLaunchKernelGGL(k_sweep_nich1_t_acc<Gv>, (note_kernel(1, "k_sweep_nich1_t_acc<" #Gv ">"), gridt), blockt, hist, stream, \
+                           feats_dev, K, kpad, row0, nrows, row_id0, z, crp, rng, *acc);                                      \
+      } else {                                                                                                                \
+        hipLaunchKernelGGL(k_sweep_nich1_t<Gv>, (note_kernel(1, "k_sweep_nich1_t<" #Gv ">"), gridt), blockt, 0, stream,       \
+                           feats_dev, K, kpad, row0, nrows, row_id0, z, crp, rng, zero);                                      \
+      }                                                                                                                       \
+    } while (0)
+    if (K <= 64) MSC_NICH1_T(1);
+    else if (K <= 128) MSC_NICH1_T(2);
+    else if (K <= 256) MSC_NICH1_T(4);
+    else if (K <= 512) MSC_NICH1_T(8);
+    else MSC_NICH1_T(16);
+#undef MSC_NICH1_T
+    return launch_status(acc ? "k_sweep_nich1_t_acc" : "k_sweep_nich1_t");
   }
   int chunk_rows = 64;
   while (chunk_rows > 4 && (nrows + chunk_rows - 1) / chunk_rows < (uint64_t)num_cus * 32) chunk_rows >>= 1;
   const uint64_t gx = grid_for((nrows + chunk_rows - 1) / chunk_rows, num_cus, 16);
   const dim3 grid((unsigned)gx), block(256);
-  if (K <= 64)
-    hipLaunchKernelGGL(k_sweep_nich1<1>, (note_kernel(1, "k_sweep_nich1<1>"), grid), block, 0, stream, feats_dev, K, kpad, row0, nrows, row_id0, z, own, crp, rng, chunk_rows, zero);
-  else if (K <= 128)
-    hipLaunchKernelGGL(k_sweep_nich1<2>, (note_kernel(1, "k_sweep_nich1<2>"), grid), block, 0, stream, feats_dev, K, kpad, row0, nrows, row_id0, z, own, crp, rng, chunk_rows, zero);
-  else if (K <= 256)
-    hipLaunchKernelGGL(k_sweep_nich1<4>, (note_kernel(1, "k_sweep_nich1<4>"), grid), block, 0, stream, feats_dev, K, kpad, row0, nrows, row_id0, z, own, crp, rng, chunk_rows, zero);
-  else if (K <= 512)
-    hipLaunchKernelGGL(k_sweep_nich1<8>, (note_kernel(1, "k_sweep_nich1<8>"), grid), block, 0, stream, feats_dev, K, kpad, row0, nrows, row_id0, z, own, crp, rng, chunk_rows, zero);
-  else
-    hipLaunchKernelGGL(k_sweep_nich1<16>, (note_kernel(1, "k_sweep_nich1<16>"), grid), block, 0, stream, feats_dev, K, kpad, row0, nrows, row_id0, z, own, crp, rng, chunk_rows, zero);
-  return launch_status("k_sweep_nich1");
+#define MSC_NICH1(Gv)                                                                                                         \
+  do {                                                                                                                        \
+    if (acc)                                                                                                                  \
+      hipLaunchKernelGGL(k_sweep_nich1_acc<Gv>, (note_kernel(1, "k_sweep_nich1_acc<" #Gv ">"), grid), block, hist, stream,    \
+                         feats_dev, K, kpad, row0, nrows, row_id0, z, own, crp, rng, chunk_rows, *acc);                       \
+    else                                                                                                                      \
+      hipLaunchKernelGGL(k_sweep_nich1<Gv>, (note_kernel(1, "k_sweep_nich1<" #Gv ">"), grid), block, 0, stream,               \
+                         feats_dev, K, kpad, row0, nrows, row_id0, z, own, crp, rng, chunk_rows, zero);                       \
+  } while (0)
+  if (K <= 64) MSC_NICH1(1);
+  else if (K <= 128) MSC_NICH1(2);
+  else if (K <= 256) MSC_NICH1(4);
+  else if (K <= 512) MSC_NICH1(8);
+  else MSC_NICH1(16);
+#undef MSC_NICH1
+  return launch_status(acc ? "k_sweep_nich1_acc" : "k_sweep_nich1");
 }
 
 static dim3 rows_grid(uint64_t nrows, uint64_t rows_per_wg, uint64_t cap) {
diff --git a/common_amd/csrc/launchers.hpp b/common_amd/csrc/launchers.hpp
--- a/common_amd/csrc/launchers.hpp
+++ b/common_amd/csrc/launchers.hpp
@@ -84,6 +84,15 @@
   unsigned long long *b = nullptr;
   size_t nb = 0;
 };
+struct AccFuse {
+  unsigned long long *table_i64 = nullptr, *stage_i64 = nullptr;
+  size_t n_i64 = 0;
+  double *table_f64 = nullptr, *stage_f64 = nullptr;
+  size_t n_f64 = 0;
+  unsigned int *ticket = nullptr;
+  bool masked = false;
+};
+inline size_t sweep_nich1_acc_lds_bytes(uint32_t K, bool masked) { return (size_t)K * (masked ? 24u : 20u); }
 int launch_sweep_rows(hipStream_t stream, int num_cus, const TailPlan &tp, const FeatDesc *feats_dev, int nfeat, int nsplit, uint32_t K,
                       uint32_t kpad, uint64_t row0, uint64_t nrows, uint64_t row_id0, int32_t *z, const float *own, const float *crp,
                       const uint64_t *rng, ZeroSpans zero);
@@ -105,7 +114,8 @@
 
 int launch_sweep_nich1(hipStream_t stream, int num_cus, bool transposed, const FeatDesc *feats_dev, uint32_t K,
                        uint32_t kpad, uint64_t row0, uint64_t nrows, uint64_t row_id0, int32_t *z,
-                       const float *own, const float *crp, const uint64_t *rng_dev, ZeroSpans zero);
+                       const float *own, const float *crp, const uint64_t *rng_dev, ZeroSpans zero,
+                       const AccFuse *acc = nullptr );
 #ifndef MSC_NICH_PACK_WAVES
 #define MSC_NICH_PACK_WAVES 8
 #endif
diff --git a/common_amd/csrc/msc_internal.hpp b/common_amd/csrc/msc_internal.hpp
--- a/common_amd/csrc/msc_internal.hpp
+++ b/common_amd/csrc/msc_internal.hpp
@@ -387,6 +387,9 @@
   msc::DevBuf<long long> red_i64;
   msc::DevBuf<double> red_f64;
   size_t n_i64 = 0, n_f64 = 0;
+  msc::DevBuf<long long> stage_i64;
+  msc::DevBuf<double> stage_f64;
+  msc::DevBuf<uint32_t> stage_ticket;
   msc::DevBuf<double> red_pack;
   uint64_t sweep_rows_hint = 0;
   std::vector<std::vector<uint32_t>> col_bounds;
diff --git a/common_amd/csrc/sweep_nich1_body.inc b/common_amd/csrc/sweep_nich1_body.inc
--- /dev/null
+++ b/common_amd/csrc/sweep_nich1_body.inc
@@ -0,0 +1,109 @@
+  const uint64_t seed = rng[0], sweep = rng[1];
+#if !MSC_BODY_ACC
+  zero_spans(zero);
+#endif
+  const FeatDesc fd = feats[0];
+#if MSC_BODY_ACC
+  extern __shared__ __attribute__((aligned(16))) unsigned char acc_lds[];
+  const AccHist hist = acc_hist_zero(acc_lds, K, acc.masked);
+  __syncthreads();
+#endif
+  const int lane = threadIdx.x & 63;
+  const uint32_t kb = (uint32_t)(G * lane);
+  float mh[G], ml[G], c0[G], c1[G], c2[G];
+  bool empty[G];
+#pragma unroll
+  for (int j = 0; j < G; j++) {
+    const uint32_t k = kb + j;
+    const size_t kc = k < kpad ? k : 0;
+    mh[j] = fd.tab[(size_t)NICH_MU_HI * kpad + kc];
+    ml[j] = fd.tab[(size_t)NICH_MU_LO * kpad + kc];
+    c0[j] = fd.tab[(size_t)NICH_C0 * kpad + kc];
+    c1[j] = fd.tab[(size_t)NICH_C1 * kpad + kc];
+    c2[j] = fd.tab[(size_t)NICH_C2 * kpad + kc];
+    const float lcj = crp[kc];
+    empty[j] = __builtin_isinf(lcj);
+    c0[j] += empty[j] ? 0.f : lcj;
+  }
+  const float le0 = crp[2 * (size_t)kpad], le1 = crp[2 * (size_t)kpad + 1];
+  constexpr float kLog2e = 1.44269504088896340736f;
+  const bool any_empty = !__builtin_isinf(le0);
+  const float dle = any_empty ? (le1 - le0) * kLog2e : 0.f;
+  float c0s[G];
+  unsigned emask = 0u;
+  float bound = -INFINITY;
+#pragma unroll
+  for (int j = 0; j < G; j++) {
+    if (empty[j] && kb + j < K) emask |= 1u << j;
+    c0s[j] = (kb + j >= K) ? -INFINITY : (c0[j] + (empty[j] ? le0 : 0.f)) * kLog2e;
+    if (kb + j < K) bound = fmaxf(bound, c0s[j]);
+  }
+  bound = wave_max(bound) + 16.f;
+#pragma unroll
+  for (int j = 0; j < G; j++) c0s[j] -= bound;
+  const float *xcol = reinterpret_cast<const float *>(fd.col) + row0;
+  const uint64_t nchunks = (nrows + chunk_rows - 1) / chunk_rows;
+  const uint64_t wave_id = (uint64_t)blockIdx.x * 4 + (threadIdx.x >> 6);
+  const uint64_t nwaves = (uint64_t)gridDim.x * 4;
+  for (uint64_t chunk = wave_id; chunk < nchunks; chunk += nwaves) {
+    const uint64_t rb = chunk * chunk_rows;
+    const int nr = (int)((nrows - rb) < (uint64_t)chunk_rows ? (nrows - rb) : (uint64_t)chunk_rows);
+    const bool has_row = lane < nr;
+    const float xv = has_row ? xcol[rb + lane] : 0.0f;
+    int gz = has_row ? z[rb + lane] : -1;
+    if ((uint32_t)gz >= K) gz = -1;
+    const float u01 = philox_uniform01(seed, sweep, row_id0 + rb + lane);
+    const unsigned long long mbits =
+        __builtin_amdgcn_ballot_w64(fd.mask != nullptr && has_row && fd.mask[row0 + rb + lane] != 0);
+    float sloo = 0.f;
+    bool single = false;
+    if (gz >= 0) {
+      const float lm1 = crp[kpad + gz];
+      single = __builtin_isinf(lm1);
+      double s = single ? (double)le1 + (double)crp[2 * (size_t)kpad + 3] : (double)lm1 + (double)crp[crp_lo_cntm1(kpad) + gz];
+      if (!((mbits >> lane) & 1ull))
+        s += nich_loo_tab(fd.hp, fd.loo64 + (size_t)gz * kNlooStride, 1, xv);
+      sloo = (float)s * kLog2e - bound;
+    }
+    const unsigned long long singles = any_empty ? __builtin_amdgcn_ballot_w64(single) : 0ull;
+    const unsigned long long odd = mbits | singles;
+    int znew = gz;
+    for (int r = 0; r < nr; r++) {
+      const float x = lane_bcast(xv, r), sl = lane_bcast(sloo, r);
+      const int g = lane_bcast(gz, r);
+      float s[G];
+#pragma unroll
+      for (int j = 0; j < G; j++) s[j] = nich_eval_log2(x, mh[j], ml[j], c0s[j], c1[j], c2[j]);
+      if ((odd >> r) & 1ull) {
+        if ((mbits >> r) & 1ull) {
+          const float e_raw = ((singles >> r) & 1ull) ? le1 : le0;
+#pragma unroll
+          for (int j = 0; j < G; j++) {
+            const float lcj = crp[kb + j < kpad ? kb + j : 0];
+            s[j] = (kb + j >= K) ? -INFINITY : (__builtin_isinf(lcj) ? e_raw : lcj) * kLog2e - bound;
+          }
+        } else {
+#pragma unroll
+          for (int j = 0; j < G; j++) s[j] += ((emask >> j) & 1u) ? dle : 0.f;
+        }
+      }
+      if (g >= 0 && lane == g / G) {
+#pragma unroll
+        for (int j = 0; j < G; j++)
+          if (j == g % G) s[j] = sl;
+      }
+      const int pick = sample_from_scores<G, true, true, true>(s, lane_bcast(u01, r), lane, K);
+      if (lane == r) znew = pick;
+    }
+#if MSC_BODY_ACC
+    if (has_row) {
+      z[rb + lane] = znew;
+      acc_hist_add(hist, K, acc.masked, znew, xv, ((mbits >> lane) & 1ull) != 0);
+    }
+#else
+    if (has_row) z[rb + lane] = znew;
+#endif
+  }
+#if MSC_BODY_ACC
+  acc_flush_and_close(hist, acc, K, kpad);
+#endif
diff --git a/common_amd/csrc/sweep_nich1_t_body.inc b/common_amd/csrc/sweep_nich1_t_body.inc
--- /dev/null
+++ b/common_amd/csrc/sweep_nich1_t_body.inc
@@ -0,0 +1,174 @@
+  constexpr int TR = MSC_BODY_TR;
+  __shared__ float lsum[4][TR * kTPad];
+  __shared__ float cst[64 * G * kTCst];
+  const uint64_t seed = rng[0], sweep = rng[1];
+#if !MSC_BODY_ACC
+  zero_spans(zero);
+#endif
+  const FeatDesc fd = feats[0];
+#if MSC_BODY_ACC
+  extern __shared__ __attribute__((aligned(16))) unsigned char acc_lds[];
+  const AccHist hist = acc_hist_zero(acc_lds, K, acc.masked);
+#endif
+  const int lane = threadIdx.x & 63, wave = __builtin_amdgcn_readfirstlane(threadIdx.x >> 6);
+  float *mysum = lsum[wave];
+  constexpr float kLog2e = 1.44269504088896340736f;
+  const float le0 = crp[2 * (size_t)kpad], le1 = crp[2 * (size_t)kpad + 1];
+  const bool any_empty = !__builtin_isinf(le0);
+  const float dle = any_empty ? (le1 - le0) * kLog2e : 0.f;
+  for (uint32_t k = threadIdx.x; k < 64u * G; k += 256u) {
+    const uint32_t kc = k < kpad ? k : 0u;
+    const float lc = crp[kc];
+    float *c = cst + k * kTCst;
+    c[TC_MH] = fd.tab[NICH_MU_HI * kpad + kc];
+    c[TC_ML] = fd.tab[NICH_MU_LO * kpad + kc];
+    c[TC_C0] = k < K ? (fd.tab[NICH_C0 * kpad + kc] + (__builtin_isinf(lc) ? le0 : lc)) * kLog2e : -INFINITY;
+    c[TC_C1] = fd.tab[NICH_C1 * kpad + kc];
+    c[TC_C2] = fd.tab[NICH_C2 * kpad + kc];
+  }
+  __syncthreads();
+  NichConsts<G> mine;
+  mine.emask = 0u;
+  float bound = -INFINITY;
+#pragma unroll
+  for (int j = 0; j < G; j++) {
+    const uint32_t k = (uint32_t)(G * lane + j);
+    const float *c = cst + k * kTCst;
+    mine.mh[j] = c[TC_MH], mine.ml[j] = c[TC_ML], mine.c0s[j] = c[TC_C0], mine.c1[j] = c[TC_C1], mine.c2[j] = c[TC_C2];
+    if (k < K && __builtin_isinf(crp[k])) mine.emask |= 1u << j;
+    bound = fmaxf(bound, mine.c0s[j]);
+  }
+  bound = wave_max(bound) + 16.f;
+#pragma unroll
+  for (int j = 0; j < G; j++) mine.c0s[j] -= bound;
+  const float *xcol = reinterpret_cast<const float *>(fd.col) + row0;
+  const uint64_t wave_id = (uint64_t)blockIdx.x * 4 + wave, nwaves = (uint64_t)gridDim.x * 4;
+  const uint64_t per = nrows / nwaves, extra = nrows % nwaves;
+  const uint64_t rbeg = wave_id * per + (wave_id < extra ? wave_id : extra), rend = rbeg + per + (wave_id < extra ? 1 : 0);
+  for (uint64_t rb = rbeg; rb < rend; rb += 64) {
+    const int nr = __builtin_amdgcn_readfirstlane((int)((rend - rb) < 64u ? (rend - rb) : 64u));
+    const bool has_row = lane < nr;
+    const float xv = has_row ? xcol[rb + lane] : 0.0f;
+    int gz = has_row ? z[rb + lane] : -1;
+    if ((uint32_t)gz >= K) gz = -1;
+    const float u01 = philox_uniform01(seed, sweep, row_id0 + rb + lane);
+    const bool my_mask = fd.mask != nullptr && has_row && fd.mask[row0 + rb + lane] != 0;
+    const unsigned long long mbits = __builtin_amdgcn_ballot_w64(my_mask);
+    float sloo = 0.f;
+    bool single = false;
+    if (gz >= 0) {
+      const float lm1 = crp[kpad + gz];
+      single = __builtin_isinf(lm1);
+      float s = single ? le1 : lm1;
+      if (!my_mask) s += nich_loo_tab_sweep(fd.hp, fd.loo64 + (size_t)gz * kNlooStride, 1, xv);
+      sloo = s * kLog2e - bound;
+    }
+    const bool my_single = single && any_empty;
+    const unsigned long long singles = __builtin_amdgcn_ballot_w64(my_single);
+    const unsigned long long odd = mbits | singles;
+    const bool plain = !(my_mask || my_single);
+    const NichRowCtx rc = {fd.tab, crp, K, kpad, le0, le1, dle, bound, xv, my_mask, my_single};
+    auto entry = [&](int k) -> float {
+      const float *c = cst + k * kTCst;
+      float s = nich_eval_log2_est(xv, c[TC_MH], c[TC_ML], c[TC_C0] - bound, c[TC_C1], c[TC_C2]);
+      if (!plain) s = nich_entry_log2(rc, (uint32_t)k);
+      return __builtin_amdgcn_exp2f(k == gz ? sloo : s);
+    };
+    const int own_lane = gz >= 0 ? gz / G : -1;
+    float own_sum = 0.f;
+    if (own_lane >= 0) {
+      own_sum = entry(G * own_lane);
+#pragma unroll
+      for (int j = 1; j < G; j++) own_sum += entry(G * own_lane + j);
+    }
+    int pick = gz;
+    bool redo = false;
+    for (int h0 = 0; h0 < nr; h0 += TR) {
+      const int h1 = h0 + TR < nr ? h0 + TR : nr;
+      __builtin_amdgcn_s_waitcnt(0);
+      for (int r = h0; r < h1; r++) {
+        const float x = lane_bcast(xv, r);
+        float s[G];
+        if ((odd >> r) & 1ull) {
+          nich_row_scores<G>(s, mine, x, ((mbits >> r) & 1ull) != 0, ((singles >> r) & 1ull) != 0, dle, -1, 0.f, crp, K, kpad,
+                             (uint32_t)lane, le0, le1, bound);
+        } else {
+#pragma unroll
+          for (int j = 0; j < G; j++) s[j] = nich_eval_log2_est(x, mine.mh[j], mine.ml[j], mine.c0s[j], mine.c1[j], mine.c2[j]);
+        }
+        float sum = __builtin_amdgcn_exp2f(s[0]);
+#pragma unroll
+        for (int j = 1; j < G; j++) sum += __builtin_amdgcn_exp2f(s[j]);
+        mysum[(r - h0) * kTPad + lane] = sum;
+      }
+      __builtin_amdgcn_wave_barrier();
+      if (lane >= h0 && lane < h1) {
+        float *row = mysum + (lane - h0) * kTPad;
+        if (own_lane >= 0) row[own_lane] = own_sum;
+        float blk[8], total = 0.f;
+#pragma unroll
+        for (int b = 0; b < 8; b++) {
+          float t = row[8 * b];
+#pragma unroll
+          for (int i = 1; i < 8; i++) t += row[8 * b + i];
+          blk[b] = t;
+          total = b == 0 ? t : total + t;
+        }
+        if (total > 0x1p-60f && total < 0x1p100f) {
+          const float dart = u01 * total;
+          float c0 = 0.f;
+          int b0 = 0;
+#pragma unroll
+          for (int b = 0; b < 7; b++) {
+            const bool miss = b0 == b && c0 + blk[b] < dart;
+            c0 = miss ? c0 + blk[b] : c0;
+            b0 += miss ? 1 : 0;
+          }
+          int hl = 8 * b0;
+#pragma unroll
+          for (int i = 0; i < 7; i++) {
+            const float v = row[8 * b0 + i];
+            const bool miss = hl == 8 * b0 + i && c0 + v < dart;
+            c0 = miss ? c0 + v : c0;
+            hl += miss ? 1 : 0;
+          }
+          int j0 = 0;
+#pragma unroll
+          for (int j = 0; j < G - 1; j++) {
+            const float v = entry(G * hl + j);
+            const bool miss = j0 == j && c0 + v < dart;
+            c0 = miss ? c0 + v : c0;
+            j0 += miss ? 1 : 0;
+          }
+          const int k = G * hl + j0;
+          pick = k < (int)K ? k : (int)K - 1;
+        } else {
+          redo = true;
+        }
+      }
+      __builtin_amdgcn_wave_barrier();
+    }
+    unsigned long long todo = __builtin_amdgcn_ballot_w64(redo);
+    while (todo != 0ull) {
+      const int r = (int)__builtin_ctzll(todo);
+      todo &= todo - 1ull;
+      const float x = lane_bcast(xv, r);
+      const int g = lane_bcast(gz, r);
+      float s[G];
+      nich_row_scores<G>(s, mine, x, ((mbits >> r) & 1ull) != 0, ((singles >> r) & 1ull) != 0, dle,
+                         (g >= 0 && lane == g / G) ? g % G : -1, lane_bcast(sloo, r), crp, K, kpad, (uint32_t)lane, le0, le1, bound);
+      const int p = sample_from_scores<G, true, false>(s, lane_bcast(u01, r), lane, K);
+      if (lane == r) pick = p;
+    }
+#if MSC_BODY_ACC
+    if (has_row) {
+      z[rb + lane] = pick;
+      acc_hist_add(hist, K, acc.masked, pick, xv, my_mask);
+    }
+#else
+    if (has_row) z[rb + lane] = pick;
+#endif
+  }
+#if MSC_BODY_ACC
+  acc_flush_and_close(hist, acc, K, kpad);
+#endif
```

Result: no change. 1759 billion (median of 2 runs) (+0.8%).
